# proger/haloop

Hardware: AMD Instinct MI355X
Metric: utterances/sec, LSTM-CTC training step (fwd + CTC loss + bwd + clip + AdamW) (higher is better)
Workload: dtype bf16 (dense operands rounded to bf16, 1 MFMA per product, fp32 accumulate; fp32 state, CTC, optimizer and master weights); 1 GPU; LC-2x1024: conv(80->128,k5,s4) + 2-layer LSTM H=1024 + Linear(1024->32) + CTC, 80 frames x 80 mels, vocab 32, targets 5-10 symbols, dropout 0.2; batch_per_gpu=64, global_batch=64, frames=80, mels=80, parallelism=dp1, hip_graph=False, math=bf16

## Files before the change

haloop_amd/_lib.py:

```python
import ctypes as C
import os

_HERE = os.path.dirname(os.path.abspath(__file__))
LIB_PATH = os.path.join(_HERE, 'csrc', 'libhalo.so')

HALO_ABI_VERSION = 21
HALO_GPT_SAMPLE_STREAM = 0x47505453
HALO_MLM_STREAM = 0x4D4C4D31
HALO_GEMM_RELU = 1
HALO_GEMM_GELU = 2
HALO_GEMM_ACCUM = 4
HALO_GEMM_GELU_ERF = 8
HALO_CTC_FULL_LATTICE = 1
HALO_CTC_FINITE_MIN = 2
HALO_CTC_NO_LEAD_BLANK_LOOP = 4
HALO_CTC_WRAP_SKIP = 8
HALO_STREAM_SUBSAMPLE = 1
HALO_STREAM_CLASSIFIER = 2
HALO_STREAM_LSTM_LAYER0 = 16
HALO_SUMSQ_PARTS = 1024
HALO_MATH_F32 = 0
HALO_MATH_BF16X3 = 1
HALO_MATH_BF16 = 2

_vp, _i, _l, _f, _u64, _u32, _sz = C.c_void_p, C.c_int, C.c_long, C.c_float, C.c_uint64, C.c_uint32, C.c_size_t

SIGNATURES = {
    'halo_abi_version': (_i, []),
    'halo_debug_read': (_i, [_vp, _sz, _i, _sz, _vp, _vp]),
    'halo_strerror': (C.c_char_p, [_i]),
    'halo_device_info': (_i, [_i, C.c_char_p, _i, C.POINTER(_i)]),
    'halo_set_math_mode': (_i, [_i]),
    'halo_get_math_mode': (_i, []),
    'halo_set_scratch': (_i, [_vp, _sz]),
    'halo_set_lstm_fusion': (_i, [_i]),
    'halo_dropout_fwd': (_i, [_vp, _vp, _sz, _f, _u64, _u32, _u32, _vp, _vp]),
    'halo_counter_inc': (_i, [_vp, _vp]),
    'halo_gemm_f32': (_i, [_i, _i, _i, _i, _i, _vp, _i, _vp, _i, _vp, _i, _vp, _vp, _i, _f, _u64, _u32, _u32, _vp, _vp]),
    'halo_split_image_bytes': (_sz, [_i, _i]),
    'halo_split_image': (_i, [_vp, _i, _i, _i, _i, _vp, _vp]),
    'halo_layernorm_image': (_i, [_vp, _vp, _vp, _vp, _vp, _i, _i, _f, _vp]),
    'halo_layernorm_bf16': (_i, [_vp, _vp, _vp, _vp, _vp, _vp, _i, _i, _f, _vp]),
    'halo_cast_bf16': (_i, [_vp, _vp, _sz, _vp]),
    'halo_gelu_bf16': (_i, [_vp, _vp, _sz, _i, _vp]),
    'halo_gelu_bwd_bf16': (_i, [_vp, _vp, _vp, _sz, _i, _vp]),
    'halo_gemm_tn_bf16_group': (_i, [_i, _vp, _vp, _vp, _vp, _vp, _vp, _i, _vp, _vp, _i, _vp]),
    'halo_gemm_tn_rows_supported': (_i, [_i, _vp, _vp, _i]),
    'halo_gemm_tn_rows_preferred': (_i, [_i, _vp, _vp, _i]),
    'halo_gemm_tn_rows_group': (_i, [_i, _vp, _vp, _vp, _vp, _vp, _vp, _i, _vp, _vp, _vp]),
    'halo_gelu_b16': (_i, [_vp, _vp, _sz, _i, _vp]),
    'halo_gelu_bwd_b16': (_i, [_vp, _vp, _vp, _sz, _i, _vp]),
    'halo_dx_alloc': (_i, [_sz, _vp, _vp]),
    'halo_dx_open': (_i, [_vp, _vp]),
    'halo_dx_close': (_i, [_vp]),
    'halo_dx_free': (_i, [_vp]),
    'halo_dx_push': (_i, [_vp, _sz, _sz, _i, _vp, _sz, _i, _i, _vp]),
    'halo_dx_signal': (_i, [_vp, _sz, _i, _i, _u32, _vp]),
    'halo_dx_wait': (_i, [_vp, _i, _i, _u32, _vp]),
    'halo_dx_reduce': (_i, [_vp, _vp, _sz, _i, _i, _f, _vp]),
    'halo_attention_fwd_b16': (_i, [_vp, _l, _l, _vp, _vp, _l, _l, _vp, _l, _l, _vp, _l, _l, _vp, _i, _i, _i, _i, _i, _i, _vp]),
    'halo_attention_bwd_b16': (_i, [_vp, _l, _l, _vp, _vp, _l, _l, _vp, _vp, _l, _l, _vp, _vp, _vp, _vp, _vp, _l, _l, _i, _i, _i, _i, _i, _i, _vp]),
    'halo_gemm_rows_supported': (_i, [_i, _i, _i]),
    'halo_gemm_rows': (_i, [_vp, _vp, _l, _vp, _i, _i, _i, _vp, _l, _vp, _l, _vp, _l, _vp]),
    'halo_gemm_rows_gelu': (_i, [_vp, _vp, _l, _vp, _i, _i, _i, _vp, _vp, _l, _i, _vp]),
    'halo_gemm_rows_ce_workspace_bytes': (_sz, [_i, _i]),
    'halo_gemm_rows_ce': (_i, [_vp, _vp, _l, _vp, _i, _i, _i, _vp, _l, _vp, _vp, _vp, _vp, _l, _vp]),
    'halo_cross_entropy_bwd_bf16': (_i, [_vp, _vp, _vp, _vp, _l, _i, _i, _l, _l, _vp]),
    'halo_lora_supported': (_i, [_i, _i, _i, _i]),
    'halo_lora_pack_bytes': (_sz, [_i, _i]),
    'halo_lora_pack': (_i, [_vp, _vp, _i, _i, _i, _vp, _vp]),
    'halo_lora_down': (_i, [_vp, _l, _vp, _i, _i, _f, _vp, _f, _u64, _u32, _u32, _vp, _vp]),
    'halo_lora_up': (_i, [_vp, _vp, _i, _i, _f, _vp, _vp, _l, _f, _u64, _u32, _u32, _vp, _vp]),
    'halo_lora_tn_workspace_bytes': (_sz, [_i, _i]),
    'halo_lora_tn': (_i, [_vp, _vp, _l, _i, _i, _i, _f, _i, _vp, _vp, _f, _u64, _u32, _u32, _vp, _vp]),
    'halo_gemm_split_ce_workspace_bytes': (_sz, [_i, _i]),
    'halo_gemm_split_ce': (_i, [_vp, _vp, _i, _i, _i, _vp, _i, _vp, _vp, _l, _vp, _vp, _vp, _vp]),
    'halo_image_pair': (_i, [_vp, _vp, _i, _i, _l, _l, _i, _vp, _vp, _vp]),
    'halo_cross_entropy_bwd_images': (_i, [_vp, _vp, _vp, _vp, _l, _i, _i, _l, _l, _vp, _vp, _vp]),
    'halo_gemm_split': (_i, [_vp, _vp, _i, _i, _i, _vp, _i, _vp, _vp, _i, _f, _u64, _u32, _u32, _vp, _vp]),
    'halo_gemm_split_residual': (_i, [_vp, _vp, _i, _i, _i, _vp, _i, _vp, _i, _vp, _vp, _i, _f, _u64, _u32, _u32, _vp, _vp]),
    'halo_image_pairs': (_i, [_i, _vp, _vp, _vp, _vp, _vp, _vp, _vp]),
    'halo_gemm_split_io': (_i, [_vp, _vp, _vp, _l, _vp, _i, _i, _i, _vp, _i, _vp, _vp, _l, _vp, _i, _vp, _vp, _i, _vp]),
    'halo_gemm_tn_bf16': (_i, [_vp, _l, _vp, _l, _i, _i, _i, _vp, _i, _i, _vp]),
    'halo_subsample_col_bytes': (_sz, [_i] * 6),
    'halo_subsample_fwd': (_i, [_vp] * 5 + [_i] * 7 + [_f, _u64, _u32, _vp, _vp]),
    'halo_subsample_bwd': (_i, [_vp] * 6 + [_i] * 7 + [_f, _vp]),
    'halo_subsample_bwd_slabs': (_i, [_vp, _i] + [_vp] * 5 + [_i] * 7 + [_f, _vp]),
    'halo_lstm_reserve_bytes': (_sz, [_i] * 5),
    'halo_lstm_bwd_workspace_bytes': (_sz, [_i] * 5),
    'halo_lstm_fwd': (_i, [_vp] * 8 + [_l, _l, _i, _vp, _vp, _vp] + [_i] * 5 + [_f, _u64, _u32, _vp, _vp]),
    'halo_lstm_bwd': (_i, [_vp] * 4 + [_l, _l, _i] + [_vp] * 9 + [_i] * 7 + [_f, _u64, _u32, _vp, _vp]),
    'halo_set_lstm_persistent': (_i, [_i]),
    'halo_set_lstm_persistent_images': (_i, [_i]),
    'halo_lstm_persistent_eligible': (_i, [_i, _i]),
    'halo_set_lstm_persistent2': (_i, [_i]),
    'halo_set_lstm_interleave': (_i, [_i]),
    'halo_set_gemm256': (_i, [_i]),
    'halo_set_lstm_bwd_mid_event': (_i, [_vp]),
    'halo_lstm_bwd_mid_event_recorded': (_i, []),
    'halo_set_lstm_expect_backward': (_i, [_i]),
    'halo_set_lstm_dx_slabs': (_i, [_i]),
    'halo_set_defer_small_jobs': (_i, [_i]),
    'halo_set_grad_sumsq': (_i, [_vp, _i]),
    'halo_grad_sumsq_state': (_i, [_vp, _vp]),
    'halo_flush_small_jobs': (_i, [_vp]),
    'halo_lstm_dx_slabs_left': (_i, []),
    'halo_set_lstm_weights_stamp': (_i, [_u64]),
    'halo_lstm_persistent2_eligible': (_i, [_i, _i, _i, _i]),
    'halo_lstm_status_offset': (_sz, [_i] * 6),
    'halo_ghost_tile': (_i, []),
    'halo_ghost_sqnorm_workspace_bytes': (_sz, [_i, _i, _i]),
    'halo_ghost_sqnorm': (_i, [_vp, _i, _i, _i, _vp, _vp, _vp, _vp]),
    'halo_set_lstm_keep_gate_gradients': (_i, [_i]),
    'halo_get_lstm_keep_gate_gradients': (_i, []),
    'halo_lstm_ghost_terms': (_i, [_vp, _vp, _i, _i, _i, _i, _i, _f, _vp]),
    'halo_relu_dropout_bwd': (_i, [_vp, _vp, _vp, _sz, _f, _vp]),
    'halo_lstm_persist_stamps': (_i, [_vp]),
    'halo_lstm_chain_events': (_i, [_vp, _vp]),
    'halo_lstm_chain_info': (_i, [_i, C.POINTER(_i), C.c_char_p, _i]),
    'halo_log_softmax_fwd': (_i, [_vp, _vp, _i, _i, _vp]),
    'halo_log_softmax_bwd': (_i, [_vp, _vp, _vp, _i, _i, _vp]),
    'halo_colsum': (_i, [_vp, _i, _i, _i, _vp, _vp]),
    'halo_ctc_fwd': (_i, [_vp, _l, _l, _i, _i, _i, _vp, _l, _i, _vp, _vp, _i, _vp, _vp, _vp]),
    'halo_ctc_bwd': (_i, [_vp, _l, _l, _i, _i, _i, _vp, _l, _i, _vp, _vp, _vp, _vp, _vp, _vp, _vp, _l, _l, _vp]),
    'halo_ctc_prepare': (_i, [_vp, _vp, _i, _i, _i, _i, _vp, _vp, _vp]),
    'halo_ctc_mean_loss': (_i, [_vp, _vp, _i, _vp, _vp]),
    'halo_ctc_head_supported': (_i, [_i, _i, _i, _i]),
    'halo_ctc_head_greedy': (_i, [_vp, _vp, _vp, _vp, _vp, _vp, _vp, _vp, _i, _i, _i, _i, _vp]),
    'halo_ctc_head_workspace_bytes': (_sz, [_i, _i, _i]),
    'halo_ctc_head_fwd': (_i, [_vp, _vp, _vp, _f, _u64, _u32, _u32, _vp, _vp, _i, _i, _i, _vp, _l, _i, _vp, _vp, _vp, _vp, _vp, _vp, _vp,
                               _vp, _i, _i, _i, _i, _vp]),
    'halo_ctc_head_bwd': (_i, [_vp, _vp, _f, _u64, _u32, _u32, _vp, _vp, _vp, _l, _i, _vp, _vp, _vp, _vp, _vp, _vp, _vp, _vp, _vp,
                               _i, _i, _i, _i, _vp]),
    'halo_ctc_head_train_workspace_bytes': (_sz, [_i, _i, _i]),
    'halo_ctc_head_train_ticket_words': (_sz, [_i, _i]),
    'halo_ctc_head_train': (_i, [_vp, _vp, _vp, _f, _u64, _u32, _u32, _vp, _vp, _i, _i, _i, _vp, _l, _i, _vp, _vp, _vp, _vp, _vp, _vp, _vp,
                                 _vp, _vp, _vp, _i, _i, _i, _i, _vp]),
    'halo_ctc_greedy': (_i, [_vp, _i, _i, _i, _vp, _vp, _vp, _vp, _vp]),
    'halo_set_beam_vector_chunk': (_i, [_i]),
    'halo_logaddexp_aten': (_i, [_vp, _vp, _vp, _sz, _vp]),
    'halo_ctc_beam_workspace_bytes': (_sz, [_i] * 4),
    'halo_ctc_beam': (_i, [_vp, _i, _i, _i, _i, _i, _vp, _vp, _vp, _vp, _vp]),
    'halo_topk_f32': (_i, [_vp, _i, _i, _i, _vp, _vp, _vp, _vp]),
    'halo_embed_fwd': (_i, [_vp, _vp, _vp, _vp, _i, _i, _i, _i, _i, _vp]),
    'halo_layernorm_fwd': (_i, [_vp, _vp, _vp, _vp, _i, _i, _f, _vp]),
    'halo_attention_causal_fwd': (_i, [_vp, _vp, _i, _i, _i, _i, _vp]),
    'halo_cross_entropy_fwd': (_i, [_vp, _vp, _vp, _i, _i, _l, _l, _vp]),
    'halo_attention_fwd': (_i, [_vp, _l, _l, _vp, _vp, _l, _l, _vp, _l, _l, _vp, _vp, _i, _i, _i, _i, _i, _i, _vp, _vp]),
    'halo_attention_fwd_strided': (_i, [_vp, _l, _l, _l, _vp, _vp, _l, _l, _l, _vp, _l, _l, _vp, _vp, _i, _i, _i, _i, _i, _i, _vp,
                                        _f, _u64, _u32, _u32, _vp, _vp]),
    'halo_kv_cache_store_f32': (_i, [_vp, _l, _l, _vp, _vp, _i, _i, _i, _i, _i, _i, _vp]),
    'halo_rope_table': (_i, [_vp, _vp, _i, _i, _f, _vp]),
    'halo_rope_interleaved': (_i, [_vp, _l, _i, _i, _i, _i, _i, _vp, _vp, _i, _i, _vp]),
    'halo_rope_rows': (_i, [_vp, _i, _l, _l, _i, _i, _i, _i, _vp, _vp, _i, _i, _vp]),
    'halo_kv_cache_store': (_i, [_vp, _l, _l, _vp, _vp, _i, _i, _i, _i, _i, _i, _vp]),
    'halo_attention_decode': (_i, [_vp, _l, _vp, _vp, _vp, _l, _i, _i, _i, _i, _i, _vp, _vp, _vp, _vp]),
    'halo_attention_decode_step': (_i, [_vp, _vp, _vp, _l, _vp, _vp, _vp, _l, _i, _i, _i, _i, _i, _vp, _vp, _vp]),
    'halo_logprob_max': (_i, [_vp, _l, _i, _i, _vp, _vp, _vp, _vp]),
    'halo_greedy_update': (_i, [_vp, _vp, _vp, _vp, _l, _i, _i, _i, _vp, _vp, _vp, _vp, _i, _vp]),
    'halo_fbank_frames': (_i, [_vp, _l, _i, _i, _i, _f, _i, _vp, _vp, _i, _vp]),
    'halo_fbank_power': (_i, [_vp, _i, _i, _vp, _i, _vp]),
    'halo_fbank_log': (_i, [_vp, _l, _f, _vp]),
    'halo_fbank_spectrum_mel': (_i, [_vp, _i, _i, _vp, _vp, _i, _f, _vp, _vp]),
    'halo_star_ctc_workspace_bytes': (_sz, [_i, _i, _i]),
    'halo_star_ctc_fwd': (_i, [_vp, _l, _l, _i, _i, _i, _vp, _i, _vp, _vp, _f, _vp, _vp, _vp]),
    'halo_star_ctc_bwd': (_i, [_vp, _l, _l, _i, _i, _i, _vp, _i, _vp, _vp, _f, _vp, _vp, _vp, _vp, _vp]),
    'halo_transducer_workspace_bytes': (_sz, [_i, _i, _i]),
    'halo_transducer_fwd': (_i, [_vp, _i, _i, _i, _i, _vp, _vp, _vp, _vp, _vp, _vp]),
    'halo_transducer_bwd': (_i, [_vp, _i, _i, _i, _i, _vp, _vp, _vp, _vp, _vp, _vp, _vp, _vp]),
    'halo_decode_image_bytes': (_sz, [_i, _i]),
    'halo_decode_image': (_i, [_vp, _i, _i, _l, _vp, _vp]),
    'halo_decode_linear_supported': (_i, [_i, _i]),
    'halo_decode_linear': (_i, [_vp, _l, _i, _i, _vp, _f, _vp, _i, _vp, _l, _i, _vp]),
    'halo_decode_linear_pair': (_i, [_vp, _vp, _l, _i, _i, _vp, _f, _vp, _i, _vp, _vp, _vp, _l, _i, _vp]),
    'halo_decode_attention_pair': (_i, [_vp, _l, _i, _i, _i, _vp, _vp, _i, _vp, _vp, _vp, _i, _i, _vp, _vp, _vp, _l, _vp]),
    'halo_decode_memory_caches': (_i, [_vp, _l, _i, _vp, _i, _i, _i, _i, _vp]),
    'halo_decode_token': (_i, [_vp, _l, _i, _i, _vp, _l, _i, _i, _i, _vp, _vp, _vp, _vp, _vp, _i, _i, _vp, _vp]),
    'halo_decode_beam_attention': (_i, [_vp, _l, _i, _i, _i, _i, _vp, _vp, _i, _vp, _vp, _vp, _i, _i, _vp, _l, _vp, _vp, _vp, _l, _vp]),
    'halo_decode_beam_select': (_i, [_vp, _l, _i, _i, _i, _i, _i, _i, _f, _vp, _vp, _vp, _vp, _vp, _vp, _vp, _vp, _vp, _vp, _vp, _l, _l, _vp, _i,
                                     _i, _vp, _vp]),
    'halo_rnnt_advance': (_i, [_vp, _l, _l, _i, _i, _i, _vp, _l, _vp, _vp, _vp, _l, _vp, _vp, _vp, _l, _i, _i, _vp, _i, _vp, _l, _vp, _vp]),
    'halo_rnnt_lstm_cell': (_i, [_vp, _l, _i, _i, _vp, _vp, _vp, _vp, _vp, _l, _vp, _l, _vp]),
    'halo_rnnt_beam_step': (_i, [_vp, _l, _l, _i, _i, _i, _vp, _l, _vp, _vp, _i, _i, _i, _vp, _vp, _vp, _vp, _vp, _vp, _l, _vp, _vp, _vp, _vp, _vp, _vp,
                                 _vp, _vp, _i, _i, _vp, _vp, _vp, _vp, _vp, _vp]),
    'halo_rnnt_beam_keep': (_i, [_i, _i, _i, _i, _i, _vp, _vp, _vp, _vp, _vp, _l, _vp, _vp, _vp, _vp]),
    'halo_rnnt_joint_fwd': (_i, [_vp, _l, _l, _vp, _l, _l, _i, _i, _i, _i, _vp, _vp, _vp, _vp, _vp, _vp]),
    'halo_rnnt_joint_bwd': (_i, [_vp, _l, _l, _vp, _l, _l, _i, _i, _i, _i, _vp, _vp, _vp, _vp, _vp, _vp, _l, _l, _vp, _l, _l, _vp]),
    'halo_ctc_viterbi_workspace_bytes': (_sz, [_i, _i, _i]),
    'halo_ctc_viterbi': (_i, [_vp, _l, _l, _i, _i, _i, _vp, _l, _i, _vp, _vp, _vp, _vp, _vp, _vp, _vp, _vp]),
    'halo_transducer_viterbi_workspace_bytes': (_sz, [_i, _i, _i]),
    'halo_transducer_viterbi': (_i, [_vp, _i, _i, _i, _i, _vp, _vp, _vp, _vp, _vp, _vp, _vp]),
    'halo_ctc_prefix_beam_workspace_bytes': (_sz, [_i, _i, _i, _i, _i]),
    'halo_ctc_prefix_beam': (_i, [_vp, _l, _l, _i, _i, _i, _vp, _i, _i, _vp, _vp, _vp, _vp, _vp, _vp]),
    'halo_ctc_lm_beam_step': (_i, [_vp, _l, _l, _i, _i, _i, _vp, _i, _i, _i, _f, _f, _vp, _l, _vp, _vp, _vp, _vp, _vp, _vp, _vp, _l, _vp, _vp, _vp,
                                   _i, _i, _vp, _vp, _vp, _vp, _vp]),
    'halo_edit_distance': (_i, [_vp, _l, _vp, _i, _i, _vp, _l, _vp, _i, _i, _i, _vp, _vp, _vp]),
    'halo_nbest_risk_fwd': (_i, [_vp, _vp, _i, _i, _vp, _vp]),
    'halo_nbest_risk_bwd': (_i, [_vp, _vp, _i, _i, _vp, _vp, _vp]),
    'halo_gpt_decode_linear_supported': (_i, [_i, _i]),
    'halo_gpt_decode_linear': (_i, [_vp, _l, _i, _i, _vp, _f, _vp, _i, _vp, _l, _i, _vp]),
    'halo_gpt_decode_attention': (_i, [_vp, _l, _i, _i, _i, _vp, _vp, _i, _vp, _vp, _l, _vp]),
    'halo_gpt_sample': (_i, [_vp, _l, _i, _i, _vp, _vp, _l, _vp, _l, _i, _vp, _vp, _vp, _i, _i, _vp, _vp]),
    'halo_attention_bwd': (_i, [_vp, _l, _l, _vp, _vp, _l, _l, _vp, _vp, _l, _l, _vp, _vp, _vp, _l, _l, _vp, _vp, _l, _l,
                                _i, _i, _i, _i, _i, _i, _vp, _f, _u64, _u32, _u32, _vp, _vp]),
    'halo_attention_masked': (_i, [_vp, _vp, _vp, _vp, _l, _l, _l, _vp, _vp, _i, _i, _i, _i, _i, _vp]),
    'halo_attention_fwd_bf16': (_i, [_vp, _l, _l, _vp, _vp, _l, _l, _vp, _l, _l, _vp, _l, _l, _vp, _i, _i, _i, _i, _i, _i, _vp, _f, _u64, _u32, _u32,
                                     _vp, _vp]),
    'halo_attention_bwd_bf16': (_i, [_vp, _l, _l, _vp, _vp, _l, _l, _vp, _vp, _l, _l, _vp, _vp, _vp, _vp, _vp, _l, _l, _i, _i, _i, _i, _i, _i, _vp,
                                     _f, _u64, _u32, _u32, _vp, _vp]),
    'halo_layernorm_bwd_workspace_bytes': (_sz, [_i, _i]),
    'halo_layernorm_bwd': (_i, [_vp, _vp, _vp, _vp, _vp, _vp, _vp, _vp, _i, _i, _f, _vp]),
    'halo_layernorm_bwd_bf16': (_i, [_vp, _vp, _vp, _vp, _vp, _vp, _vp, _vp, _vp, _i, _i, _f, _vp]),
    'halo_layernorm_bwd_b16': (_i, [_vp, _vp, _vp, _vp, _vp, _vp, _vp, _vp, _vp, _i, _i, _f, _vp]),
    'halo_gelu_fwd': (_i, [_vp, _vp, _sz, _i, _vp]),
    'halo_gelu_bwd': (_i, [_vp, _vp, _vp, _sz, _i, _vp]),
    'halo_cross_entropy_fwd_lse': (_i, [_vp, _vp, _vp, _vp, _i, _i, _l, _l, _vp]),
    'halo_cross_entropy_bwd': (_i, [_vp, _vp, _vp, _vp, _l, _i, _i, _l, _l, _vp]),
    'halo_embed_bwd': (_i, [_vp, _vp, _vp, _vp, _i, _i, _i, _i, _i, _i, _vp]),
    'halo_embed_bwd_ordered': (_i, [_vp, _vp, _vp, _i, _i, _i, _vp]),
    'halo_add_rows_bcast': (_i, [_vp, _vp, _i, _i, _i, _vp]),
    'halo_im2col_cl': (_i, [_vp, _vp, _i, _i, _i, _i, _i, _i, _vp]),
    'halo_col2im_cl': (_i, [_vp, _vp, _i, _i, _i, _i, _i, _i, _vp]),
    'halo_dwconv1d_cl': (_i, [_vp, _vp, _vp, _vp, _i, _i, _i, _i, _i, _i, _vp]),
    'halo_dwconv1d_cl_bwd_workspace_bytes': (_sz, [_i, _i]),
    'halo_dwconv1d_cl_bwd': (_i, [_vp, _vp, _vp, _vp, _vp, _vp, _vp, _i, _i, _i, _i, _i, _i, _vp]),
    'halo_tape_batch': (_i, [_vp, _i, _l, _i, _i, _l, _i, _l, _vp, _vp]),
    'halo_lm_batch_u16': (_i, [_vp, _l, _vp, _i, _i, _i, _vp, _vp, _vp]),
    'halo_mask_tokens': (_i, [_vp, _vp, _l, _f, _l, _l, _l, _u64, _u32, _vp]),
    'halo_mlm_batch_u16': (_i, [_vp, _l, _vp, _i, _i, _f, _l, _l, _l, _u64, _u32, _vp, _vp, _vp]),
    'halo_target_rows': (_i, [_vp, _i, _l, _i, _i, _vp, _vp, _vp, _vp, _vp]),
    'halo_gather_rows': (_i, [_vp, _vp, _i, _i, _i, _vp, _vp]),
    'halo_scatter_rows': (_i, [_vp, _vp, _vp, _i, _i, _i, _i, _vp, _vp, _vp]),
    'halo_scale_add': (_i, [_vp, _vp, _f, _f, _sz, _vp]),
    'halo_cast_f32_bf16': (_i, [_vp, _vp, _sz, _vp]),
    'halo_cast_bf16_f32': (_i, [_vp, _vp, _f, _sz, _vp]),
    'halo_scale_add_guarded': (_i, [_vp, _vp, _f, _f, _sz, _vp, _vp]),
    'halo_clip_coef_step': (_i, [_vp, _i, _f, _vp, _vp, _vp, _vp]),
    'halo_adamw_ranges_dev': (_i, [_vp, _vp, _vp, _vp, _i, _vp, _vp, _vp, _vp, _f, _vp, _f, _f, _f, _vp, _vp, _vp]),
    'halo_ctx_create': (_vp, []),
    'halo_ctx_destroy': (None, [_vp]),
    'halo_ctx_use': (_i, [_vp]),
    'halo_set_status_word': (_i, [_vp]),
    'halo_debug_mute_workgroup': (_i, [_i]),
    'halo_debug_mfma_clock': (_i, [_vp, _vp, _i, _i, _i, _u32, _vp]),
    'halo_sumsq': (_i, [_vp, _sz, _vp, _vp]),
    'halo_sumsq_ranges': (_i, [_vp, _i, _vp, _vp, _vp, _vp]),
    'halo_pack_ranges_bf16': (_i, [_vp, _i, _vp, _vp, _vp, _vp]),
    'halo_expand_ranges_bf16': (_i, [_vp, _i, _vp, _vp, _i, _i, _vp, _vp]),
    'halo_clip_coef': (_i, [_vp, _i, _f, _vp, _vp, _vp]),
    'halo_adamw_multi_tensor_bytes': (_sz, []),
    'halo_adamw_multi_chunk': (_u32, []),
    'halo_adamw_multi_max_tensors': (_i, []),
    'halo_adamw_multi': (_i, [_vp, _vp, _i, _vp, _i, _f, _f, _f, _f, _i, _vp, _vp]),
    'halo_adamw_ranges': (_i, [_vp, _vp, _vp, _vp, _i, _vp, _vp, _vp, _vp, _f, _f, _f, _f, _i, _vp, _vp]),
    'halo_adamw': (_i, [_vp, _vp, _vp, _vp, _sz, _f, _f, _f, _f, _f, _i, _vp, _vp]),
}



class GhostOperand(C.Structure):
    _fields_ = [('ptr', _vp), ('stride_n', _l), ('stride_t', _l), ('K', _i)]


class GhostTerm(C.Structure):
    _fields_ = [('a', GhostOperand), ('b', GhostOperand * 2), ('n_b', _i), ('n_bias', _i)]


_lib = None


class HaloError(RuntimeError):
    pass


def lib():
    global _lib
    if _lib is None:
        import torch
        if not os.path.exists(LIB_PATH):
            raise HaloError(f'{LIB_PATH} not found: build it with `make -C haloop_amd/csrc` '
                            '(or __graft_entry__.build()); haloop_amd has no CPU fallback')
        handle = C.CDLL(LIB_PATH)
        for name, (res, args) in SIGNATURES.items():
            fn = getattr(handle, name)
            fn.restype = res
            fn.argtypes = args
        if handle.halo_abi_version() != HALO_ABI_VERSION:
            raise HaloError('libhalo.so ABI version mismatch: rebuild it')
        _lib = handle
        mode = os.environ.get('HALO_MATH')
        if mode:
            set_math_mode(mode)
    return _lib


def set_math_mode(mode):
    global _mode
    code = {'f32': HALO_MATH_F32, 'bf16x3': HALO_MATH_BF16X3, 'bf16': HALO_MATH_BF16}[mode]
    check(lib().halo_set_math_mode(code), 'halo_set_math_mode')
    _mode = mode


def set_lstm_fusion(on):
    check(lib().halo_set_lstm_fusion(int(bool(on))), 'halo_set_lstm_fusion')


def set_lstm_persistent(on):
    check(lib().halo_set_lstm_persistent(int(bool(on))), 'halo_set_lstm_persistent')


def set_lstm_bwd_mid_event(event):
    check(lib().halo_set_lstm_bwd_mid_event(None if event is None else C.c_void_p(event.cuda_event)), 'halo_set_lstm_bwd_mid_event')


def set_gemm256(on):
    check(lib().halo_set_gemm256(1 if on else 0), 'halo_set_gemm256')


def set_lstm_interleave(on):
    check(lib().halo_set_lstm_interleave(int(bool(on))), 'halo_set_lstm_interleave')


def set_lstm_keep_gate_gradients(on):
    check(lib().halo_set_lstm_keep_gate_gradients(int(bool(on))), 'halo_set_lstm_keep_gate_gradients')


def get_lstm_keep_gate_gradients():
    return bool(lib().halo_get_lstm_keep_gate_gradients())


def set_lstm_persistent2(on):
    check(lib().halo_set_lstm_persistent2(int(bool(on))), 'halo_set_lstm_persistent2')


_WEIGHTS_EPOCH = [0]


# ... 107 lines not shown
```

haloop_amd/csrc/halo_internal.h:

```cpp
#pragma once
#include <hip/hip_runtime.h>
#include <stddef.h>
#include "halo_common.h"
#include "dyn_lds.h"
#include "small_jobs.h"

int halo_transpose(const float *in, float *out, int rows, int cols, hipStream_t st);
int halo_fill(float *p, size_t n, float v, hipStream_t st);
int halo_colsum2(const float *x, int rows, int cols, int ld, float *out, float *out2, hipStream_t st);

size_t halo_tiled_image_bytes(int R, int K);
int halo_prep_tiles(const float *src, int R, int K, int ld, int src_transposed, void *image, hipStream_t st);
int halo_prep_pair(const float *src, int R, int C, int ld, void *image_rm, void *image_tr, hipStream_t st);
struct HaloPrepJob {
    int kind;
    const float *src;
    int R, K, ld;
    void *image, *image_tr;
};
int halo_prep_jobs(const HaloPrepJob *jobs, int n, hipStream_t st);
int halo_gemm_bf16x3_tiled(const void *Aimg, const void *Bimg, int M, int N, int K, float *C, int ldc,
                           const float *bias1, const float *bias2, int relu, const DropoutCfg *drop, hipStream_t st);
int halo_gemm_bf16x3_tiled_slices(const void *Aimg, const void *Bimg, int M, int N, int K, float *slab, int want, int *slices, hipStream_t st);
bool halo_defer_small_job(const HaloSmallJob &job);
struct HaloCtx {
    int math_mode = 0;
    int lstm_fusion = 0;
    int lstm_persistent = 1, lstm_persistent2 = 1;
    int lstm_interleave = 1;
    int persist_emit = -1;
    int beam_vec_chunk = 32;
    void *scratch = nullptr;
    size_t scratch_bytes = 0;
    int scratch_slot = 0;
    unsigned *status = nullptr;
    hipEvent_t chain_ev0 = nullptr, chain_ev1 = nullptr;
    int bwd_mid_recorded = 0;
    hipEvent_t bwd_mid_event = nullptr;
    unsigned long long *stamps = nullptr;
    float *grad_sumsq = nullptr;
    int grad_sumsq_cap = 0, grad_sumsq_n = 0;
    unsigned grad_sumsq_cover = 0;
    int defer_small_jobs = 0;
    HaloSmallJobs small_jobs = {};
    int lstm_dx_slabs = 1;
    int lstm_dx_slabs_left = 1;
    int lstm_expect_backward = 1;
    const float *packT_reserve = nullptr, *packT_w[3] = {nullptr, nullptr, nullptr};
    const float *bwdflags_reserve = nullptr;
    const float *fwdT_src[2] = {nullptr, nullptr};
    const float *fwdT_reserve = nullptr;
    const float *emitT_reserve = nullptr;
    uint64_t lstm_weights_stamp = 0, packF_stamp = 0;
    const float *packF_reserve = nullptr, *packF_w[3] = {nullptr, nullptr, nullptr};
    int packF_dims[5] = {0, 0, 0, 0, 0};
    int lstm_keep_dg = 0;
    const float *ghost_reserve = nullptr;
    int mute_block = -1;
};
HaloCtx &halo_ctx_cur();
int halo_cu_count();
int halo_gemm_bf16x3_tiled_nsplit(const void *Aimg, const void *Bimg, int M, int N, int K, float *C, int ldc, int n_split, float *C2, int ldc2,
                                  hipStream_t st);
int halo_gemm_bf16x3_tiled_nsplit_carry(const void *Aimg, const void *Bimg, int M, int N, int K, float *C, int ldc, int n_split, float *C2, int ldc2,
                                        const void *rA, const void *rB, int rM, int rN, int rK, float *rslab, int want, int *slices,
                                        float *sumsq_part, int *sumsq_parts, hipStream_t st);
struct HaloG256Problem {
    const void *A, *B;
    int M, N, K;
    float *C; int ldc;
    int n_split; float *C2; int ldc2;
    int kslices; long slab_stride;
    float *sumsq;
    int tiles;
};
int halo_gemm256_enabled();
int halo_gemm256_fits(const HaloG256Problem &q);
int halo_gemm256_launch(HaloG256Problem *probs, int n, hipStream_t st);
int halo_math_mode();
int halo_lstm_fusion();

void halo_get_scratch(void **ptr, size_t *bytes);
void halo_set_scratch_slot(int slot);
int halo_side_stream(hipStream_t *side, hipEvent_t *fork_ev, hipEvent_t *join_ev);
int halo_pick_ksplit(long tiles, int k_steps, long out_elems);
int halo_splitk_reduce(const float *slab, int ksplit, int M, int N, float *C, int ldc, const float *bias1,
                       const float *bias2, int relu, const DropoutCfg &drop, int use_drop, hipStream_t st);
```

haloop_amd/csrc/lstm.hip:

```cpp
#include <stdlib.h>
#include <string.h>
#include "halo_common.h"
#include "halo_internal.h"
#include "tiled_image.h"
#include "lstm_persist.h"

namespace {

enum YMode { Y_NONE = 0, Y_PLAIN = 1, Y_RELU = 2, Y_DROPOUT = 3 };

typedef __bf16 bf16x8 __attribute__((ext_vector_type(8)));

template <bool X3>
struct Packed {
    static constexpr int KB = X3 ? 32 : 16;
    static constexpr int BLOCK_BYTES = X3 ? 2048 : 1024;
    __device__ static __forceinline__ void store(void *img, int tile, int nk, int i, int k, float v) {
        const int blk = k / KB, kk = k % KB;
        char *base = (char *)img + ((long)tile * (nk / KB) + blk) * BLOCK_BYTES;
        if (X3) {
            const int lane = (kk >> 3) * 16 + i, e = kk & 7;
            const __bf16 hi = (__bf16)v;
            const __bf16 lo = (__bf16)(v - (float)hi);
            reinterpret_cast<__bf16 *>(base)[lane * 8 + e] = hi;
// ... 1015 lines not shown
                         const uint32_t *offset_dev, hipStream_t st) {
    const size_t BH = (size_t)B * H, PG = bt16(B) * 4 * H, per = fused_bwd_layer_floats(B, H);
    for (int l = 0; l < L; ++l) {
        float *base = extra + (size_t)l * per;
        HALO_TRY(launch_pack<1>(w_hh[l], base, H, B, 4 * H, H / 16, true, st));
        if (l > 0) HALO_TRY(launch_pack<1>(w_ih[l], base + (size_t)4 * H * H, H, B, 4 * H, H / 16, true, st));
    }
    for (int d = 0; d < T + L - 1; ++d) {
        DiagBwdArgs a;
        a.B = B; a.H = H;
        for (int l = 0; l < MAXL; ++l) {
            DiagBwdLayer &q = a.layer[l];
            const int t = l < L ? T - 1 - (d - (L - 1 - l)) : -1;
            q.active = l < L && t >= 0 && t < T;
            if (!q.active) continue;
            const LayerBufs lb = layer_bufs(reserve, l, T, B, H);
            float *base = extra + (size_t)l * per;
            float *dcarry = base + (size_t)8 * H * H;
            float *dgp = dcarry + BH;
            const bool top = (l == L - 1);
            q.dgp_next = (t == T - 1) ? nullptr : dgp + (size_t)((t + 1) & 1) * PG;
            q.dgp_out = dgp + (size_t)(t & 1) * PG;
            q.wpT_hh = base;
            if (!top) {
                float *above = extra + (size_t)(l + 1) * per;
                q.dgp_above = above + (size_t)8 * H * H + BH + (size_t)(t & 1) * PG;
                q.wpT_ih_above = above + (size_t)4 * H * H;
            } else {
                q.dgp_above = nullptr; q.wpT_ih_above = nullptr;
            }
            q.gates = lb.gates + (size_t)t * B * 4 * H;
            q.c = lb.c + (size_t)(t + 1) * BH;
            q.cprev = lb.c + (size_t)t * BH;
            q.dc = dcarry;
            q.dy = (top && dy) ? dy + (long)t * y_stride_t : nullptr;
            q.dy_stride_b = y_stride_b;
            q.dy_relu = y_relu;
            q.first = (t == T - 1);
            q.dhinit = (t == T - 1 && dhn) ? dhn + (size_t)l * BH : nullptr;
            q.dcinit = (t == T - 1 && dcn) ? dcn + (size_t)l * BH : nullptr;
            q.drop = make_dropout(top ? 0.f : p_drop, seed, HALO_STREAM_LSTM_LAYER0 + (uint32_t)l, offset, offset_dev);
            q.drop_base = (uint64_t)t * BH;
        }
        hipLaunchKernelGGL(lstm_diag_bwd_kernel, dim3(H / 16, (B + 15) / 16, L), dim3(1024), 0, st, a);
        HALO_TRY(halo_launch_status());
    }
    return HALO_OK;
}

inline size_t reserve_flags_offset(int T, int B, int in0, int H, int L) {
    const int kin = in0 > H ? in0 : H;
    const size_t n = ((size_t)4 * H * H + (size_t)L * layer_floats(T, B, H)) * sizeof(float) +
                     halo_tiled_image_bytes(T * B, kin) + halo_tiled_image_bytes(4 * H, kin) +
                     (L >= 2 ? fused_fwd_extra_floats(T, B, H, L) * sizeof(float) : 0);
    return (n + 255) & ~(size_t)255;
}
inline int bwd_dg_images(int T) { return T > 2 ? T : 2; }
inline size_t bwd_flags_offset(int T, int B, int in0, int H, int L) {
    const int kin = in0 > H ? in0 : H;
    const size_t n = ((size_t)H * 4 * H + (size_t)B * H + (size_t)T * B * H + (size_t)bwd_dg_images(T) * bt16(B) * 4 * H) * sizeof(float) +
                     halo_tiled_image_bytes(4 * H, T * B) + halo_tiled_image_bytes(T * B, 4 * H) +
                     2 * halo_tiled_image_bytes(kin, T * B) + halo_tiled_image_bytes(kin, 4 * H) +
                     (L >= 2 ? (size_t)L * fused_bwd_layer_floats(B, H) * sizeof(float) : 0);
    return (n + 255) & ~(size_t)255;
}

inline size_t reserve_p2_images_bytes(int T, int B, int in0, int H) {
    const int kin = in0 > H ? in0 : H;
    return (size_t)3 * 4 * H * H * sizeof(float) + 3 * halo_tiled_image_bytes(H, T * B) + halo_tiled_image_bytes(kin, T * B);
}
inline size_t reserve_p2_bytes(int T, int B, int in0, int H) {
    return reserve_p2_images_bytes(T, B, in0, H) + PERSIST_FLAG_BYTES + halo_tiled_image_bytes(in0 > H ? in0 : H, 4 * H);
}
inline unsigned *reserve_bwd_flags(float *reserve, int T, int B, int in0, int H, int L) {
    return (unsigned *)((char *)reserve + reserve_flags_offset(T, B, in0, H, L) + PERSIST_FLAG_BYTES + reserve_p2_images_bytes(T, B, in0, H));
}
inline char *reserve_p2_wT(float *reserve, int T, int B, int in0, int H, int L) {
    return (char *)reserve_bwd_flags(reserve, T, B, in0, H, L) + PERSIST_FLAG_BYTES;
}
inline char *reserve_p2_images(float *reserve, int T, int B, int in0, int H, int L) {
    return (char *)reserve + reserve_flags_offset(T, B, in0, H, L) + PERSIST_FLAG_BYTES + (size_t)3 * 4 * H * H * sizeof(float);
}

inline bool persist_emit_enabled() {
    int &v = halo_ctx_cur().persist_emit;
    if (v < 0) { const char *e = getenv("HALO_PERSIST_EMIT"); v = e ? (atoi(e) != 0) : 1; }
    return v != 0;
}

inline bool keep_dg_switch() {
    static const bool on = getenv("HALO_LSTM_KEEP_DG") && getenv("HALO_LSTM_KEEP_DG")[0] == '1';
    return on || halo_ctx_cur().lstm_keep_dg != 0;
}

inline bool pair_dw_enabled() {
    static const bool on = !(getenv("HALO_LSTM_PAIR_DW") && atoi(getenv("HALO_LSTM_PAIR_DW")) == 0);
    return on;
}

int lstm_bwd_layer_tail(const float *x, const float *const *w_ih, float *reserve, int l, int in0, int T, int B, int H, int L, float p_drop,
                        uint64_t seed, uint32_t offset, const uint32_t *offset_dev, bool fused, bool emit, char *img_g, char *img_gT,
                        char *img_hT, char *img_inT, char *img_wT, const float *bias_part, float *din, float *dx, float *const *dw_ih,
                        float *const *dw_hh, float *const *db_ih, float *const *db_hh, bool need_din, hipStream_t st) {
    const size_t BH = (size_t)B * H;
    const LayerBufs lb = layer_bufs(reserve, l, T, B, H);
    hipStream_t side = st;
    const float *in;
    int in_dim;
    if (l == 0) { in = x; in_dim = in0; }
    else {
        const LayerBufs pb = layer_bufs(reserve, l - 1, T, B, H);
        in = p_drop > 0.f ? pb.ydrop : pb.h + BH;
        in_dim = H;
    }
    (void)fused;
    float *din_out = l > 0 ? din : dx;
    const DropoutCfg ddrop = make_dropout(l > 0 ? p_drop : 0.f, seed, HALO_STREAM_LSTM_LAYER0 + (uint32_t)(l > 0 ? l - 1 : 0),
                                          offset, offset_dev);
    const bool tiled = halo_math_mode() != HALO_MATH_F32 && in_dim >= 64;
    int rc = HALO_OK;
    if (tiled) {
        HaloPrepJob jobs[5];
        int nj = 0;
        if (need_din) {
            if (!emit) jobs[nj++] = {2, lb.gates, T * B, 4 * H, 4 * H, img_g, img_gT};
            jobs[nj++] = {1, w_ih[l], in_dim, 4 * H, in_dim, img_wT, nullptr};
        } else if (!emit) {
            jobs[nj++] = {1, lb.gates, 4 * H, T * B, 4 * H, img_gT, nullptr};
        }
        if (emit)
            jobs[nj++] = {3, bias_part, (B + 15) / 16, 4 * H, 4 * H, db_ih[l], db_hh[l]};
        jobs[nj++] = {1, lb.h, H, T * B, H, img_hT, nullptr};
        jobs[nj++] = {1, in, in_dim, T * B, in_dim, img_inT, nullptr};
        HALO_TRY(halo_prep_jobs(jobs, nj, st));
    }
    if (need_din) {
        if (tiled) {
            HALO_TRY(halo_gemm_bf16x3_tiled(img_g, img_wT, T * B, in_dim, 4 * H, din_out, in_dim, nullptr, nullptr, 0,
                                            &ddrop, st));
        } else {
            HALO_TRY(halo_gemm_f32(1, 0, T * B, in_dim, 4 * H, lb.gates, 4 * H, w_ih[l], in_dim, din_out, in_dim,
                                   nullptr, nullptr, 0, l > 0 ? p_drop : 0.f, seed,
                                   HALO_STREAM_LSTM_LAYER0 + (uint32_t)(l > 0 ? l - 1 : 0), offset, offset_dev, (halo_stream_t)st));
        }
    }
    if (tiled && H % 128 == 0 && img_inT == img_hT + halo_tiled_image_bytes(H, T * B) && pair_dw_enabled()) {
        HaloG256Problem gp = {};
        gp.A = img_gT; gp.B = img_hT; gp.M = 4 * H; gp.N = H + in_dim; gp.K = T * B;
        gp.C = dw_hh[l]; gp.ldc = H; gp.n_split = H; gp.C2 = dw_ih[l]; gp.ldc2 = in_dim; gp.kslices = 1;
        const long t256 = (long)((4 * H + 255) / 256) * ((H + in_dim + 255) / 256);
        if (halo_gemm256_enabled() && halo_gemm256_fits(gp) && 100 * t256 >= 55 * ((t256 + 255) / 256) * 256) rc = halo_gemm256_launch(&gp, 1, side);
        else
        rc = halo_gemm_bf16x3_tiled_nsplit(img_gT, img_hT, 4 * H, H + in_dim, T * B, dw_hh[l], H, H, dw_ih[l], in_dim, side);
    } else if (tiled) {
        rc = halo_gemm_bf16x3_tiled(img_gT, img_hT, 4 * H, H, T * B, dw_hh[l], H, nullptr, nullptr, 0, nullptr, side);
        if (!rc) rc = halo_gemm_bf16x3_tiled(img_gT, img_inT, 4 * H, in_dim, T * B, dw_ih[l], in_dim, nullptr, nullptr, 0,
                                             nullptr, side);
    } else {
        rc = halo_gemm_f32(0, 0, 4 * H, H, T * B, lb.gates, 4 * H, lb.h, H, dw_hh[l], H, nullptr, nullptr, 0, 0.f, 0, 0,
                           0, nullptr, (halo_stream_t)side);
        if (!rc) rc = halo_gemm_f32(0, 0, 4 * H, in_dim, T * B, lb.gates, 4 * H, in, in_dim, dw_ih[l], in_dim, nullptr,
                                    nullptr, 0, 0.f, 0, 0, 0, nullptr, (halo_stream_t)side);
    }
    if (!rc && !(emit && tiled)) rc = halo_colsum2(lb.gates, T * B, 4 * H, 4 * H, db_ih[l], db_hh[l], side);
    return rc;
}


int lstm_fwd_persist2(const float *in, int in_dim, int lo, const float *const *w_ih, const float *const *w_hh, const float *const *b_ih,
                      const float *const *b_hh, const float *h0, const float *c0, float *y, long y_stride_t, long y_stride_b,
                      int y_relu, float *hn, float *cn, float *reserve, float *extra, char *img_in, char *img_w, int T, int B,
                      int in0, int H, int L, float p_drop, uint64_t seed, uint32_t offset, const uint32_t *offset_dev, hipStream_t st) {
    const int hi = lo + 1;
    const size_t BH = (size_t)B * H;
    const LayerBufs l0 = layer_bufs(reserve, lo, T, B, H), l1 = layer_bufs(reserve, hi, T, B, H);
    w_ih += lo; w_hh += lo; b_ih += lo; b_hh += lo;
    if (h0) h0 += (size_t)lo * BH;
    if (c0) c0 += (size_t)lo * BH;
    HaloCtx &ctx = halo_ctx_cur();
    const bool images_by_pack = in_dim >= 64;
    if (in_dim < 64) {
        HALO_TRY(halo_gemm_f32(1, 1, T * B, 4 * H, in_dim, in, in_dim, w_ih[0], in_dim, l0.gates, 4 * H, b_ih[0], b_hh[0], 0, 0.f, 0, 0, 0,
                               nullptr, (halo_stream_t)st));
    }
    float *wp0 = reserve, *wp1 = fused_wpk(extra, hi, H), *wpi = wp1 + (size_t)4 * H * H;
    unsigned *flags = (unsigned *)((char *)reserve + reserve_flags_offset(T, B, in0, H, L));
    Prologue2Args pa;
    pa.img.n = 0; pa.img.blocks = 0; pa.img.with_lo = halo_math_mode() != HALO_MATH_BF16;
    pa.w[0] = w_hh[0]; pa.wdst[0] = wp0; pa.w[1] = w_hh[1]; pa.wdst[1] = wp1; pa.w[2] = w_ih[1]; pa.wdst[2] = wpi;
    pa.w_units = (long)(H / 16) * 4 * (H / 32) * 64; pa.wK = H;
    for (int l = 0; l < 2; ++l) {
        const LayerBufs lb = l ? l1 : l0;
        pa.h0[l] = h0 ? h0 + (size_t)l * BH : nullptr; pa.hp0[l] = lb.hp; pa.h_rm[l] = lb.h;
        pa.c0[l] = c0 ? c0 + (size_t)l * BH : nullptr; pa.c_rm[l] = lb.c;
    }
    pa.s_units = (long)((B + 15) / 16) * (H / 32) * 64;
    pa.zero = flags; pa.zero_units = (long)(PERSIST_FLAG_BYTES / 16);
    pa.zero2 = nullptr; pa.zero2_units = 0;
    char *xp = p_drop > 0.f ? (char *)fused_yp(extra, lo, T, B, H, L) : nullptr;
    pa.narm = 0; pa.arm_units = 0;
    if (halo_lstm_persist2_fwd_armed(T, B, H)) {
        const size_t image = (size_t)((B + 15) / 16) * (H / 32) * 2048;
        pa.arm[pa.narm++] = (char *)l0.hp + image;
        pa.arm[pa.narm++] = (char *)l1.hp + image;
        if (xp) pa.arm[pa.narm++] = xp;
        pa.arm_units = (long)T * (long)(image / 2048) * 64;
    }
    pa.H = H; pa.B = B;
    ctx.packT_reserve = nullptr;
    ctx.emitT_reserve = nullptr;
    char *emit_hT0 = nullptr, *emit_hT1 = nullptr, *emit_xT1 = nullptr;
    if (ctx.lstm_expect_backward && H % 32 == 0) {
        float *wT = (float *)((char *)reserve + reserve_flags_offset(T, B, in0, H, L) + PERSIST_FLAG_BYTES);
        PackPairArgs pp;
        for (int m = 0; m < 3; ++m) { pp.w[m] = pa.w[m]; pp.fwd[m] = (char *)pa.wdst[m]; pp.tr[m] = (char *)(wT + (size_t)m * 4 * H * H); }
        pp.H = H;
        pp.tile_blocks = 3 * (4 * H / 32) * (H / 32) / 4;
        pp.rest = pa; pp.rest.w_units = 0;
        pp.rest.zero2 = reserve_bwd_flags(reserve, T, B, in0, H, L); pp.rest.zero2_units = (long)(PERSIST_FLAG_BYTES / 16);
        pp.zbase[0] = pp.zbase[1] = nullptr; pp.zstride = 0; pp.zunits = 0; pp.zcount = 0;
        ctx.emitT_reserve = nullptr;
        const bool emitT = persist_emit_enabled() && !h0 && B % 32 == 0 && H % 128 == 0 && T * B >= 32;
        if (emitT) {
            char *imgs = reserve_p2_images(reserve, T, B, in0, H, L);
            const size_t hb = halo_tiled_image_bytes(H, T * B), ib = halo_tiled_image_bytes(in0 > H ? in0 : H, T * B);
            emit_hT0 = imgs; emit_hT1 = imgs + hb + ib; emit_xT1 = emit_hT1 + hb;
            const long KT = (T * B + 31) / 32;
            pp.zbase[0] = emit_hT0; pp.zbase[1] = emit_hT1;
            pp.zstride = KT * 16384; pp.zunits = (long)(B / 32) * 16384 / 16; pp.zcount = H / 128;
            ctx.emitT_reserve = reserve;
        }
        ctx.fwdT_reserve = nullptr;
        if (images_by_pack) {
            ImageJobs &ij = pp.rest.img;
            image_jobs_add(ij, in, T * B, in_dim, in_dim, 0, img_in);
            image_jobs_add(ij, w_ih[0], 4 * H, in_dim, in_dim, 0, img_w);
            if (emitT) {
                image_jobs_add(ij, in, in_dim, T * B, in_dim, 1, emit_hT0 + halo_tiled_image_bytes(H, T * B));
                image_jobs_add(ij, w_ih[0], in_dim, 4 * H, in_dim, 1, reserve_p2_wT(reserve, T, B, in0, H, L));
                ctx.fwdT_reserve = reserve; ctx.fwdT_src[0] = in; ctx.fwdT_src[1] = w_ih[0];
            }
        }
        const unsigned rest_blocks = pack_grid((size_t)(2 * pa.s_units + pa.zero_units + pp.rest.zero2_units + 2L * pp.zcount * pp.zunits +
                                                        (long)pa.narm * pa.arm_units));
        hipLaunchKernelGGL(persist2_pack_pair_kernel, dim3((unsigned)(pp.tile_blocks + pp.rest.img.blocks) + rest_blocks), dim3(256), 0, st, pp);
        HALO_TRY(halo_launch_status());
        if (images_by_pack)
            HALO_TRY(halo_gemm_bf16x3_tiled(img_in, img_w, T * B, 4 * H, in_dim, l0.gates, 4 * H, b_ih[0], b_hh[0], 0, nullptr, st));
        ctx.packT_reserve = reserve;
        ctx.bwdflags_reserve = reserve;
        for (int m = 0; m < 3; ++m) ctx.packT_w[m] = pa.w[m];
    } else {
        const int dims[5] = {T, B, in0, H, L};
        const bool keep = ctx.lstm_weights_stamp != 0 && lo == 0 && ctx.packF_stamp == ctx.lstm_weights_stamp && ctx.packF_reserve == reserve &&
                          ctx.packF_w[0] == pa.w[0] && ctx.packF_w[1] == pa.w[1] && ctx.packF_w[2] == pa.w[2] &&
                          !memcmp(ctx.packF_dims, dims, sizeof(dims));
        if (keep) pa.w_units = 0;
        if (images_by_pack) {
            image_jobs_add(pa.img, in, T * B, in_dim, in_dim, 0, img_in);
            image_jobs_add(pa.img, w_ih[0], 4 * H, in_dim, in_dim, 0, img_w);
        }
        hipLaunchKernelGGL(persist2_prologue_kernel<0>, dim3((unsigned)pa.img.blocks + pack_grid((size_t)(3 * pa.w_units + 2 * pa.s_units + pa.zero_units +
                                                                                                      (long)pa.narm * pa.arm_units))),
                           dim3(256), 0, st, pa);
        HALO_TRY(halo_launch_status());
        if (images_by_pack)
            HALO_TRY(halo_gemm_bf16x3_tiled(img_in, img_w, T * B, 4 * H, in_dim, l0.gates, 4 * H, b_ih[0], b_hh[0], 0, nullptr, st));
        ctx.packF_stamp = lo == 0 ? ctx.lstm_weights_stamp : 0;
        ctx.packF_reserve = reserve;
        for (int m = 0; m < 3; ++m) ctx.packF_w[m] = pa.w[m];
        memcpy(ctx.packF_dims, dims, sizeof(dims));
    }
    Persist2Fwd a;
    a.wp0 = (const char *)wp0; a.wp1 = (const char *)wp1; a.wpi = (const char *)wpi;
    a.hp0 = (char *)l0.hp; a.hp1 = (char *)l1.hp;
    a.xp = xp;
    a.gates0 = l0.gates; a.h0 = l0.h; a.c0 = l0.c;
    a.gates1 = l1.gates; a.h1 = l1.h; a.c1 = l1.c;
    a.b_ih1 = b_ih[1]; a.b_hh1 = b_hh[1];
    a.ydrop = p_drop > 0.f ? l0.ydrop : nullptr;
    a.y = y; a.y_stride_t = y_stride_t; a.y_stride_b = y_stride_b; a.y_mode = y ? (y_relu ? 2 : 1) : 0;
    a.drop = make_dropout(p_drop, seed, HALO_STREAM_LSTM_LAYER0 + (uint32_t)lo, offset, offset_dev);
    a.img_hT0 = emit_hT0; a.img_hT1 = emit_hT1; a.img_xT1 = emit_xT1;
    a.flags = flags;
    a.stamps = halo_lstm_persist_stamp_buffer();
    a.T = T; a.B = B; a.H = H;
    chain_begin(st);
    HALO_TRY(halo_lstm_persist2_fwd(a, st));
    chain_end(st, 0, 1, "lstm_persist2_fwd_kernel");
    for (int l = 0; l < 2; ++l) {
        const LayerBufs lb = l ? l1 : l0;
        if (hn) HALO_TRY(copy_d2d(hn + (size_t)(lo + l) * BH, lb.h + (size_t)T * BH, BH, st));
        if (cn) HALO_TRY(copy_d2d(cn + (size_t)(lo + l) * BH, lb.c + (size_t)T * BH, BH, st));
    }
    return HALO_OK;
}


inline size_t bwd_p2_offset(int T, int B, int in0, int H, int L) {
    const size_t n = bwd_flags_offset(T, B, in0, H, L) + PERSIST_FLAG_BYTES + (size_t)((B + 15) / 16) * 4 * H * sizeof(float);
    return (n + 255) & ~(size_t)255;
}
inline size_t bwd_p2_bytes(int T, int B, int H) {
    return (((size_t)((B + 15) / 16) * 4 * H * sizeof(float) + 255) & ~(size_t)255) + (size_t)T * bt16(B) * 4 * H * sizeof(float) +
           halo_tiled_image_bytes(4 * H, T * B);
}

}

extern "C" {

int halo_lstm_chain_events(void *ev_begin, void *ev_end) {
    halo_ctx_cur().chain_ev0 = (hipEvent_t)ev_begin;
    halo_ctx_cur().chain_ev1 = (hipEvent_t)ev_end;
    return HALO_OK;
}

int halo_lstm_chain_info(int backward, int *launches, char *kernel, int kernel_len) {
    const ChainInfo &ci = g_chain_info[backward ? 1 : 0];
    if (launches) *launches = ci.launches;
    if (kernel && kernel_len > 0) {
        strncpy(kernel, ci.kernel, (size_t)kernel_len - 1);
        kernel[kernel_len - 1] = 0;
    }
    return HALO_OK;
}

size_t halo_lstm_reserve_bytes(int T, int B, int in0, int H, int L) {
    if (T <= 0 || B <= 0 || in0 <= 0 || H <= 0 || L <= 0) return 0;
    return reserve_flags_offset(T, B, in0, H, L) + PERSIST_FLAG_BYTES + (L >= 2 ? reserve_p2_bytes(T, B, in0, H) : 0);
}

int halo_set_lstm_persistent(int on) {
    halo_lstm_persist_enable(on);
    return HALO_OK;
}

int halo_set_lstm_persistent_images(int on) {
    halo_ctx_cur().persist_emit = on ? 1 : 0;
    return HALO_OK;
}


int halo_lstm_persistent_eligible(int B, int H) { return halo_lstm_persist_ok(B, H) && use_x3(H) ? 1 : 0; }

int halo_set_lstm_persistent2(int on) {
    halo_lstm_persist2_enable(on);
    return HALO_OK;
}
int halo_set_lstm_bwd_mid_event(void *event) {
    halo_ctx_cur().bwd_mid_event = (hipEvent_t)event;
    halo_ctx_cur().bwd_mid_recorded = 0;
    return HALO_OK;
}
int halo_lstm_bwd_mid_event_recorded(void) { return halo_ctx_cur().bwd_mid_recorded; }
int halo_set_lstm_interleave(int on) {
    halo_lstm_interleave_enable(on);
    return HALO_OK;
}
int halo_set_lstm_weights_stamp(uint64_t stamp) {
    halo_ctx_cur().lstm_weights_stamp = stamp;
    return HALO_OK;
}

int halo_set_grad_sumsq(float *partials, int capacity) {
    HaloCtx &ctx = halo_ctx_cur();
    if (partials && capacity <= 0) return HALO_EINVAL;
    ctx.grad_sumsq = partials; ctx.grad_sumsq_cap = partials ? capacity : 0; ctx.grad_sumsq_n = 0; ctx.grad_sumsq_cover = 0;
    return HALO_OK;
}
int halo_grad_sumsq_state(int *count, unsigned *covered) {
    const HaloCtx &ctx = halo_ctx_cur();
    if (count) *count = ctx.grad_sumsq_n;
    if (covered) *covered = ctx.grad_sumsq_cover;
    return HALO_OK;
}
int halo_set_lstm_dx_slabs(int n) {
    if (n < 1 || n > 64) return HALO_EINVAL;
    halo_ctx_cur().lstm_dx_slabs = n;
    return HALO_OK;
}
int halo_lstm_dx_slabs_left(void) { return halo_ctx_cur().lstm_dx_slabs_left; }
int halo_set_lstm_expect_backward(int on) {
    halo_ctx_cur().lstm_expect_backward = on ? 1 : 0;
    return HALO_OK;
}
int halo_lstm_persistent2_eligible(int T, int B, int H, int L) {       return !fused_ok(H, L) && use_x3(H) && halo_lstm_persist2_ok(T, B, H, L) ? 1 : 0; }

size_t halo_lstm_status_offset(int backward, int T, int B, int in0, int H, int L) {
    if (T <= 0 || B <= 0 || in0 <= 0 || H <= 0 || L <= 0) return 0;
    return backward ? bwd_flags_offset(T, B, in0, H, L) : reserve_flags_offset(T, B, in0, H, L);
}

size_t halo_lstm_bwd_workspace_bytes(int T, int B, int in0, int H, int L) {
    if (T <= 0 || B <= 0 || H <= 0 || L <= 0) return 0;
    if (L >= 2) return bwd_p2_offset(T, B, in0, H, L) + bwd_p2_bytes(T, B, H);
    return bwd_flags_offset(T, B, in0, H, L) + PERSIST_FLAG_BYTES + (size_t)((B + 15) / 16) * 4 * H * sizeof(float);
}

int halo_lstm_fwd(const float *x, const float *const *w_ih, const float *const *w_hh, const float *const *b_ih,
                  const float *const *b_hh, const float *h0, const float *c0, float *y, long y_stride_t,
                  long y_stride_b, int y_relu, float *hn, float *cn, float *reserve, int T, int B, int in0, int H,
                  int L, float p_drop, uint64_t seed, uint32_t offset, const uint32_t *offset_dev,
                  halo_stream_t stream) {
    HALO_CHECK_ARG(x && w_ih && w_hh && b_ih && b_hh && reserve);
    HALO_CHECK_ARG(T > 0 && B > 0 && in0 > 0 && H > 0 && L > 0);
    if (H % 16 != 0) return HALO_ENOTSUP;
    halo_ctx_cur().ghost_reserve = nullptr;
    hipStream_t st = (hipStream_t)stream;
    const size_t BH = (size_t)B * H, PH = bt16(B) * H;
    halo_ctx_cur().packT_reserve = nullptr;
    halo_ctx_cur().emitT_reserve = nullptr;
    float *wp = reserve;
    const bool x3 = use_x3(H);
    const int kin = in0 > H ? in0 : H;
    char *img_in = (char *)(reserve + (size_t)4 * H * H + (size_t)L * layer_floats(T, B, H));
    char *img_w = img_in + halo_tiled_image_bytes(T * B, kin);
    for (int l = 0; l < L; ++l) HALO_CHECK_ARG(w_ih[l] && w_hh[l] && b_ih[l] && b_hh[l]);
    const bool pair = !fused_ok(H, L) && x3 && halo_lstm_persist2_ok(T, B, H, L);
    const int n_single = pair ? L - 2 : L;
    if (fused_ok(H, L)) {
        float *extra = (float *)(img_w + halo_tiled_image_bytes(4 * H, kin));
        return lstm_fwd_fused(x, w_ih, w_hh, b_ih, b_hh, h0, c0, y, y_stride_t, y_stride_b, y_relu, hn, cn, reserve, extra,
                              img_in, img_w, T, B, in0, H, L, p_drop, seed, offset, offset_dev, st);
    }
    for (int l = 0; l < L; ++l) {
        const LayerBufs lb = layer_bufs(reserve, l, T, B, H);
        const bool last = (l == L - 1);
        const bool drop_out = !last && p_drop > 0.f;
        const float *in;
        int in_dim;
        if (l == 0) { in = x; in_dim = in0; }
        else {
            const LayerBufs pb = layer_bufs(reserve, l - 1, T, B, H);
            in = p_drop > 0.f ? pb.ydrop : pb.h + BH;
            in_dim = H;
        }
        if (pair && l == n_single) {
            float *extra = (float *)(img_w + halo_tiled_image_bytes(4 * H, kin));
            return lstm_fwd_persist2(in, in_dim, l, w_ih, w_hh, b_ih, b_hh, h0, c0, y, y_stride_t, y_stride_b, y_relu, hn, cn, reserve, extra,
                                     img_in, img_w, T, B, in0, H, L, p_drop, seed, offset, offset_dev, st);
        }
        if (halo_math_mode() != HALO_MATH_F32 && in_dim >= 64) {
            const HaloPrepJob jobs[2] = {{0, in, T * B, in_dim, in_dim, img_in, nullptr}, {0, w_ih[l], 4 * H, in_dim, in_dim, img_w, nullptr}};
            HALO_TRY(halo_prep_jobs(jobs, 2, st));
            HALO_TRY(halo_gemm_bf16x3_tiled(img_in, img_w, T * B, 4 * H, in_dim, lb.gates, 4 * H, b_ih[l], b_hh[l], 0,
                                            nullptr, st));
        } else {
            HALO_TRY(halo_gemm_f32(1, 1, T * B, 4 * H, in_dim, in, in_dim, w_ih[l], in_dim, lb.gates, 4 * H, b_ih[l],
                                   b_hh[l], 0, 0.f, 0, 0, 0, nullptr, stream));
        }
        const float *h0l = h0 ? h0 + (size_t)l * BH : nullptr;
        const bool persist = x3 && halo_lstm_persist_ok(B, H) && halo_lstm_persist_fits(T, B, H);
        unsigned *flags = (unsigned *)((char *)reserve + reserve_flags_offset(T, B, in0, H, L));
        if (persist) {
            PrologueArgs pa;
            pa.w = w_hh[l]; pa.wdst = wp; pa.w_units = (long)(H / 16) * 4 * (H / 32) * 64; pa.wK = H;
            pa.h0 = h0l; pa.hp0 = lb.hp; pa.h_rm = lb.h; pa.c0 = c0 ? c0 + (size_t)l * BH : nullptr; pa.c_rm = lb.c;
            pa.s_units = (long)((B + 15) / 16) * (H / 32) * 64;
            pa.zero = flags; pa.zero_units = (long)(PERSIST_FLAG_BYTES / 16);
            pa.zero2 = nullptr; pa.zero2_units = 0;
            pa.H = H; pa.B = B;
            hipLaunchKernelGGL(persist_prologue_kernel<0>, dim3(pack_grid((size_t)(pa.w_units + pa.s_units + pa.zero_units))), dim3(256), 0, st, pa);
            HALO_TRY(halo_launch_status());
        } else {
            HALO_TRY(launch_pack<0>(w_hh[l], wp, H, B, H, (H / 16) * 4, x3, st));
            HALO_TRY(launch_pack<2>(h0l, lb.hp, H, B, H, (B + 15) / 16, x3, st, lb.h, c0 ? c0 + (size_t)l * BH : nullptr, lb.c));
        }
        const DropoutCfg dc = make_dropout(drop_out ? p_drop : 0.f, seed, HALO_STREAM_LSTM_LAYER0 + (uint32_t)l, offset, offset_dev);
        if (persist) {
            PersistFwd a;
            a.wp = (const char *)wp;
            a.hp = (char *)lb.hp;
            a.gates = lb.gates; a.h = lb.h; a.c = lb.c;
            a.T = T; a.B = B; a.H = H;
            a.drop = dc;
            if (last && y) { a.y = y; a.y_stride_t = y_stride_t; a.y_stride_b = y_stride_b; a.y_mode = y_relu ? Y_RELU : Y_PLAIN; }
            else if (drop_out) { a.y = lb.ydrop; a.y_stride_t = (long)BH; a.y_stride_b = H; a.y_mode = Y_DROPOUT; }
            else { a.y = nullptr; a.y_stride_t = 0; a.y_stride_b = 0; a.y_mode = Y_NONE; }
            a.flags = flags;
            a.stamps = halo_lstm_persist_stamp_buffer();
            chain_begin(st);
            HALO_TRY(halo_lstm_persist_fwd(a, st));
            chain_end(st, 0, 1, "lstm_persist_fwd_kernel");
            if (hn) HALO_TRY(copy_d2d(hn + (size_t)l * BH, lb.h + (size_t)T * BH, BH, st));
            if (cn) HALO_TRY(copy_d2d(cn + (size_t)l * BH, lb.c + (size_t)T * BH, BH, st));
            continue;
        }
        chain_begin(st);
        for (int t = 0; t < T; ++t) {
            StepFwdArgs a;
            a.hp_prev = lb.hp + (size_t)t * PH;
            a.cprev = lb.c + (size_t)t * BH;
            a.wp = wp;
            a.gates = lb.gates + (size_t)t * B * 4 * H;
            a.hout = lb.h + (size_t)(t + 1) * BH;
            a.hp_out = lb.hp + (size_t)(t + 1) * PH;
            a.cout = lb.c + (size_t)(t + 1) * BH;
            a.B = B; a.H = H;
            a.drop = dc;
            a.drop_base = (uint64_t)t * BH;
            if (last && y) {
                a.y = y + (long)t * y_stride_t;
                a.y_stride_b = y_stride_b;
                a.y_mode = y_relu ? Y_RELU : Y_PLAIN;
            } else if (drop_out) {
                a.y = lb.ydrop + (size_t)t * BH;
                a.y_stride_b = H;
                a.y_mode = Y_DROPOUT;
            } else {
                a.y = nullptr; a.y_stride_b = 0; a.y_mode = Y_NONE;
            }
            HALO_TRY(launch_step_fwd(a, x3, st));
        }
        chain_end(st, 0, T, "lstm_step_fwd_kernel");
        if (hn) HALO_TRY(copy_d2d(hn + (size_t)l * BH, lb.h + (size_t)T * BH, BH, st));
        if (cn) HALO_TRY(copy_d2d(cn + (size_t)l * BH, lb.c + (size_t)T * BH, BH, st));
    }
    return HALO_OK;
}

int halo_lstm_bwd(const float *x, const float *const *w_ih, const float *const *w_hh, const float *dy,
                  long y_stride_t, long y_stride_b, int y_relu, const float *dhn, const float *dcn, float *reserve,
                  float *workspace, float *dx, float *const *dw_ih, float *const *dw_hh, float *const *db_ih,
// ... 297 lines not shown
```

haloop_amd/csrc/optim.hip:

```cpp
#include <math.h>
#include <stdlib.h>
#include "halo_common.h"
#include "halo_internal.h"

namespace {

__global__ __launch_bounds__(256) void sumsq_kernel(const float *__restrict__ x, size_t n, float *__restrict__ partials) {
    __shared__ float red[4];
    float s = 0.f;
    const size_t n4 = n / 4;
    const f32x4 *x4 = reinterpret_cast<const f32x4 *>(x);
    for (size_t i = blockIdx.x * (size_t)256 + threadIdx.x; i < n4; i += (size_t)gridDim.x * 256) {
        const f32x4 v = x4[i];
        s += v[0] * v[0] + v[1] * v[1] + v[2] * v[2] + v[3] * v[3];
    }
    if (blockIdx.x == 0)
        for (size_t i = n4 * 4 + threadIdx.x; i < n; i += 256) s += x[i] * x[i];
    s = wave_sum(s);
    if ((threadIdx.x & 63) == 0) red[threadIdx.x >> 6] = s;
    __syncthreads();
    if (threadIdx.x == 0) partials[blockIdx.x] = (red[0] + red[1]) + (red[2] + red[3]);
}

struct Ranges8 {
// ... 50 lines not shown
            if ((int)rk == skip) continue;
            const bf16x4 v = reinterpret_cast<const bf16x4 *>(stage)[rk * per_rank + off + j];
            d4[i] = f32x4{(float)v[0], (float)v[1], (float)v[2], (float)v[3]};
        }
        off += c;
    }
}

__global__ __launch_bounds__(256) void clip_coef_kernel(const float *__restrict__ partials, int count, float max_norm,
                                                        float *coef, float *norm_out, uint32_t *applied_steps, const uint32_t *status) {
    __shared__ float red[4];
    float s = 0.f;
    for (int i = threadIdx.x; i < count; i += 256) s += partials[i];
    s = wave_sum(s);
    if ((threadIdx.x & 63) == 0) red[threadIdx.x >> 6] = s;
    __syncthreads();
    if (threadIdx.x == 0) {
        const float norm = sqrtf((red[0] + red[1]) + (red[2] + red[3]));
        const float c = max_norm / (norm + 1e-6f);
        const bool finite = isfinite(norm) && !(status && *status != 0u);
        coef[0] = finite ? (c > 1.0f ? 1.0f : c) : NAN;
        coef[1] = finite ? 1.0f : NAN;
        if (norm_out) *norm_out = norm;
        if (applied_steps && finite) *applied_steps += 1u;
    }
}

__device__ __forceinline__ void adam_update(float &p, float &m, float &v, float g, float decay_mul, float beta1_w, float beta2,
                                            float beta2_w, float step_size, float bc2_sqrt, float eps) {
#pragma clang fp contract(off)
    p = p * decay_mul;
    m = __builtin_fmaf(g - m, beta1_w, m);
    v = __builtin_fmaf(beta2_w * g, g, v * beta2);
    const float denom = sqrtf(v) / bc2_sqrt + eps;
    p = p - step_size * (m / denom);
}

struct AdamArgs {
    float *p;
    const float *g;
    float *m;
    float *v;
    size_t n;
    float decay_mul;
    float beta1_w;
    float beta2;
    float beta2_w;
    float step_size;
    float bc2_sqrt;
    float eps;
    const float *grad_scale;
};

__global__ __launch_bounds__(256) void adamw_kernel(const AdamArgs a) {
    const float gs = a.grad_scale ? *a.grad_scale : 1.0f;
    if (gs != gs) return;
    const size_t n4 = a.n / 4;
    f32x4 *p4 = reinterpret_cast<f32x4 *>(a.p), *m4 = reinterpret_cast<f32x4 *>(a.m), *v4 = reinterpret_cast<f32x4 *>(a.v);
    const f32x4 *g4 = reinterpret_cast<const f32x4 *>(a.g);
    for (size_t i = blockIdx.x * (size_t)256 + threadIdx.x; i < n4; i += (size_t)gridDim.x * 256) {
        f32x4 p = p4[i], m = m4[i], v = v4[i];
        const f32x4 g = g4[i];
#pragma unroll
        for (int e = 0; e < 4; ++e) {
            const float ge = a.grad_scale ? g[e] * gs : g[e];
            float pe = p[e], me = m[e], ve = v[e];
            adam_update(pe, me, ve, ge, a.decay_mul, a.beta1_w, a.beta2, a.beta2_w, a.step_size, a.bc2_sqrt, a.eps);
            p[e] = pe; m[e] = me; v[e] = ve;
        }
        p4[i] = p; m4[i] = m; v4[i] = v;
    }
    if (blockIdx.x == 0) {
        for (size_t i = n4 * 4 + threadIdx.x; i < a.n; i += 256) {
            const float ge = a.grad_scale ? a.g[i] * gs : a.g[i];
            float pe = a.p[i], me = a.m[i], ve = a.v[i];
            adam_update(pe, me, ve, ge, a.decay_mul, a.beta1_w, a.beta2, a.beta2_w, a.step_size, a.bc2_sqrt, a.eps);
            a.p[i] = pe; a.m[i] = me; a.v[i] = ve;
        }
    }
}


constexpr int ADAM_MAX_RANGES = 8;
struct AdamRangesArgs {
    float *p;
    const float *g;
    float *m;
    float *v;
    size_t begin4[ADAM_MAX_RANGES], end4[ADAM_MAX_RANGES];
    float decay_mul[ADAM_MAX_RANGES];
    const float *grad_scale[ADAM_MAX_RANGES];
    int n_ranges;
    float beta1_w, beta2, beta2_w, step_size, bc2_sqrt, eps;
    uint32_t *counter;
    const uint32_t *step_dev;
    const float *lr_dev;
    float weight_decay[ADAM_MAX_RANGES];
    float lr, beta1;
};

template <bool NT>
__global__ __launch_bounds__(256) void adamw_ranges_kernel(const AdamRangesArgs a) {
    f32x4 *p4 = reinterpret_cast<f32x4 *>(a.p), *m4 = reinterpret_cast<f32x4 *>(a.m), *v4 = reinterpret_cast<f32x4 *>(a.v);
    const f32x4 *g4 = reinterpret_cast<const f32x4 *>(a.g);
    float step_size = a.step_size, bc2_sqrt = a.bc2_sqrt;
    const float lr = a.lr_dev ? *a.lr_dev : a.lr;
    if (a.step_dev) {
        const double t = (double)max(*a.step_dev, 1u);
        step_size = (float)((double)lr / (1.0 - pow((double)a.beta1, t)));
        bc2_sqrt = (float)sqrt(1.0 - pow((double)a.beta2, t));
    }
    for (int r = 0; r < a.n_ranges; ++r) {
        const float gs = a.grad_scale[r] ? *a.grad_scale[r] : 1.0f;
        if (gs != gs) continue;
        const float decay_mul = a.lr_dev ? (float)(1.0 - (double)lr * (double)a.weight_decay[r]) : a.decay_mul[r];
        for (size_t i = a.begin4[r] + blockIdx.x * (size_t)256 + threadIdx.x; i < a.end4[r]; i += (size_t)gridDim.x * 256) {
            f32x4 p = p4[i], m = NT ? __builtin_nontemporal_load(m4 + i) : m4[i], v = NT ? __builtin_nontemporal_load(v4 + i) : v4[i];
            const f32x4 g = NT ? __builtin_nontemporal_load(g4 + i) : g4[i];
#pragma unroll
            for (int e = 0; e < 4; ++e) {
                const float ge = a.grad_scale[r] ? g[e] * gs : g[e];
                float pe = p[e], me = m[e], ve = v[e];
                adam_update(pe, me, ve, ge, decay_mul, a.beta1_w, a.beta2, a.beta2_w, step_size, bc2_sqrt, a.eps);
                p[e] = pe; m[e] = me; v[e] = ve;
            }
            p4[i] = p;
            if (NT) { __builtin_nontemporal_store(m, m4 + i); __builtin_nontemporal_store(v, v4 + i); }
            else { m4[i] = m; v4[i] = v; }
        }
    }
    if (a.counter && blockIdx.x == 0 && threadIdx.x == 0) *a.counter += 1u;
}

struct AdamTensor {
    float *p;
    float *m;
    float *v;
    unsigned long long n;
    float weight_decay;
    int pad;
};
constexpr unsigned ADAM_CHUNK = 16384;
constexpr int ADAM_MULTI_MAX = 256;
struct AdamGrads { const float *g[ADAM_MULTI_MAX]; };

__global__ __launch_bounds__(256) void adamw_multi_kernel(const AdamTensor *__restrict__ tensors, const uint2 *__restrict__ chunks,
                                                          const AdamGrads grads, float lr, float beta1_w, float beta2, float beta2_w,
                                                          float step_size, float bc2_sqrt, float eps,
                                                          const float *__restrict__ grad_scale) {
    const float gs = grad_scale ? *grad_scale : 1.0f;
    if (gs != gs) return;
    const uint2 c = chunks[blockIdx.x];
    const AdamTensor t = tensors[c.x];
    const float decay_mul = (float)(1.0 - (double)lr * (double)t.weight_decay);
    const float *tg = grads.g[c.x];
    const size_t begin = (size_t)c.y * ADAM_CHUNK, end = min(begin + (size_t)ADAM_CHUNK, (size_t)t.n);
    auto update = [&](float &pe, float &me, float &ve, float g) {
        adam_update(pe, me, ve, grad_scale ? g * gs : g, decay_mul, beta1_w, beta2, beta2_w, step_size, bc2_sqrt, eps);
    };
    const bool vec = (((uintptr_t)t.p | (uintptr_t)tg | (uintptr_t)t.m | (uintptr_t)t.v) % 16) == 0;
    size_t done = begin;
    if (vec) {
        const size_t e4 = end / 4;
        f32x4 *p4 = reinterpret_cast<f32x4 *>(t.p), *m4 = reinterpret_cast<f32x4 *>(t.m), *v4 = reinterpret_cast<f32x4 *>(t.v);
        const f32x4 *g4 = reinterpret_cast<const f32x4 *>(tg);
        for (size_t i = begin / 4 + threadIdx.x; i < e4; i += 256) {
            f32x4 p = p4[i], m = __builtin_nontemporal_load(m4 + i), v = __builtin_nontemporal_load(v4 + i);
            const f32x4 g = __builtin_nontemporal_load(g4 + i);
#pragma unroll
            for (int e = 0; e < 4; ++e) {
                float pe = p[e], me = m[e], ve = v[e];
                update(pe, me, ve, g[e]);
                p[e] = pe; m[e] = me; v[e] = ve;
            }
            p4[i] = p;
            __builtin_nontemporal_store(m, m4 + i);
            __builtin_nontemporal_store(v, v4 + i);
        }
        done = e4 * 4;
    }
    for (size_t i = done + threadIdx.x; i < end; i += 256) {
        float pe = t.p[i], me = t.m[i], ve = t.v[i];
        update(pe, me, ve, tg[i]);
        t.p[i] = pe; t.m[i] = me; t.v[i] = ve;
    }
}

}

namespace {
__global__ __launch_bounds__(256) void scale_add_kernel(float *__restrict__ y, const float *__restrict__ x, float alpha, float beta, size_t n4,
                                                        size_t n, const float *__restrict__ guard) {
    const size_t i = (size_t)blockIdx.x * 256 + threadIdx.x;
    const bool take_x = !guard || isfinite(*guard);
    const bool take_y = alpha != 0.f;
    if (i < n4) {
        f32x4 a = {0.f, 0.f, 0.f, 0.f}, b = {0.f, 0.f, 0.f, 0.f};
        if (take_y) a = alpha * reinterpret_cast<f32x4 *>(y)[i];
        if (take_x) b = beta * reinterpret_cast<const f32x4 *>(x)[i];
        reinterpret_cast<f32x4 *>(y)[i] = a + b;
    } else if (i == n4) {
        for (size_t e = 4 * n4; e < n; ++e) y[e] = (take_y ? alpha * y[e] : 0.f) + (take_x ? beta * x[e] : 0.f);
    }
}
}

namespace {
typedef __bf16 bf16x4 __attribute__((ext_vector_type(4)));
__global__ __launch_bounds__(256) void cast_f32_bf16_kernel(const float *__restrict__ x, __bf16 *__restrict__ y, size_t n4, size_t n) {
    for (size_t i = (size_t)blockIdx.x * 256 + threadIdx.x; i < n4; i += (size_t)gridDim.x * 256) {
        const f32x4 v = reinterpret_cast<const f32x4 *>(x)[i];
        bf16x4 o;
#pragma unroll
        for (int e = 0; e < 4; ++e) o[e] = (__bf16)v[e];
// ... 77 lines not shown

int halo_pack_ranges_bf16(const float *src, int n, const size_t *begin, const size_t *end, void *dst, halo_stream_t stream) {
    HALO_CHECK_ARG(src && dst && ((uintptr_t)src % 16 == 0) && ((uintptr_t)dst % 8 == 0));
    Ranges8 r; size_t total4;
    { const int rc = make_ranges8(n, begin, end, r, total4); if (rc != HALO_OK) return rc; }
    if (total4 == 0) return HALO_OK;
    const unsigned blocks = (unsigned)((total4 + 255) / 256 < 2048 ? (total4 + 255) / 256 : 2048);
    hipLaunchKernelGGL(pack_ranges_bf16_kernel, dim3(blocks), dim3(256), 0, (hipStream_t)stream, src, r, (__bf16 *)dst);
    return halo_launch_status();
}

int halo_expand_ranges_bf16(const void *stage, int n, const size_t *begin, const size_t *chunk, int world, int skip_rank, float *dst,
                            halo_stream_t stream) {
    HALO_CHECK_ARG(stage && dst && world >= 1 && ((uintptr_t)dst % 16 == 0) && ((uintptr_t)stage % 8 == 0));
    Ranges8 r; size_t total4;
    size_t end[8];
    if (n < 1 || n > 8 || !begin || !chunk) return HALO_EINVAL;
    for (int k = 0; k < n; ++k) end[k] = begin[k] + chunk[k];
    { const int rc = make_ranges8(n, begin, end, r, total4); if (rc != HALO_OK) return rc; }
    if (total4 == 0) return HALO_OK;
    const size_t all4 = total4 * (size_t)world;
    const unsigned blocks = (unsigned)((all4 + 255) / 256 < 4096 ? (all4 + 255) / 256 : 4096);
    hipLaunchKernelGGL(expand_ranges_bf16_kernel, dim3(blocks), dim3(256), 0, (hipStream_t)stream, (const __bf16 *)stage, r, world, skip_rank, dst);
    return halo_launch_status();
}

int halo_clip_coef_step(const float *partials, int count, float max_norm, float *coef, float *norm_out, uint32_t *applied_steps,
                        halo_stream_t stream) {
    HALO_CHECK_ARG(partials && coef && count > 0);
    hipLaunchKernelGGL(clip_coef_kernel, dim3(1), dim3(256), 0, (hipStream_t)stream, partials, count, max_norm, coef,
                       norm_out, applied_steps, (const uint32_t *)halo_ctx_cur().status);
    return halo_launch_status();
}

int halo_clip_coef(const float *partials, int count, float max_norm, float *coef, float *norm_out,
                   halo_stream_t stream) {
    return halo_clip_coef_step(partials, count, max_norm, coef, norm_out, nullptr, stream);
}

int halo_adamw(float *p, const float *g, float *m, float *v, size_t n, float lr, float beta1, float beta2, float eps,
               float weight_decay, int step, const float *grad_scale, halo_stream_t stream) {
    HALO_CHECK_ARG(p && g && m && v && step >= 1);
    HALO_CHECK_ARG(((uintptr_t)p % 16 == 0) && ((uintptr_t)g % 16 == 0) && ((uintptr_t)m % 16 == 0) &&
                   ((uintptr_t)v % 16 == 0));
    if (n == 0) return HALO_OK;
    AdamArgs a;
    a.p = p; a.g = g; a.m = m; a.v = v; a.n = n;
    const double bc1 = 1.0 - pow((double)beta1, (double)step);
    const double bc2 = 1.0 - pow((double)beta2, (double)step);
    a.decay_mul = (float)(1.0 - (double)lr * (double)weight_decay);
    a.beta1_w = (float)(1.0 - (double)beta1);
    a.beta2 = beta2;
    a.beta2_w = (float)(1.0 - (double)beta2);
    a.step_size = (float)((double)lr / bc1);
    a.bc2_sqrt = (float)sqrt(bc2);
    a.eps = eps;
    a.grad_scale = grad_scale;
    size_t blocks = (n / 4 + 255) / 256;
    if (blocks < 1) blocks = 1;
    if (blocks > 2048) blocks = 2048;
    hipLaunchKernelGGL(adamw_kernel, dim3((unsigned)blocks), dim3(256), 0, (hipStream_t)stream, a);
    return halo_launch_status();
}

size_t halo_adamw_multi_tensor_bytes(void) { return sizeof(AdamTensor); }
unsigned halo_adamw_multi_chunk(void) { return ADAM_CHUNK; }

int halo_adamw_multi_max_tensors(void) { return ADAM_MULTI_MAX; }

int halo_adamw_multi(const void *tensor_table, const void *chunk_table, int n_chunks, const float *const *grads, int n_tensors, float lr,
                     float beta1, float beta2, float eps, int step, const float *grad_scale, halo_stream_t stream) {
    HALO_CHECK_ARG(tensor_table && chunk_table && n_chunks > 0 && step >= 1 && grads && n_tensors > 0 && n_tensors <= ADAM_MULTI_MAX);
    AdamGrads gr;
    for (int i = 0; i < ADAM_MULTI_MAX; ++i) gr.g[i] = i < n_tensors ? grads[i] : nullptr;
    for (int i = 0; i < n_tensors; ++i) HALO_CHECK_ARG(grads[i] != nullptr);
    const double bc1 = 1.0 - pow((double)beta1, (double)step);
    const double bc2 = 1.0 - pow((double)beta2, (double)step);
    hipLaunchKernelGGL(adamw_multi_kernel, dim3((unsigned)n_chunks), dim3(256), 0, (hipStream_t)stream, (const AdamTensor *)tensor_table,
                       (const uint2 *)chunk_table, gr, lr, (float)(1.0 - (double)beta1), beta2, (float)(1.0 - (double)beta2),
                       (float)((double)lr / bc1), (float)sqrt(bc2), eps, grad_scale);
    return halo_launch_status();
}

static int adamw_ranges_impl(float *p, const float *g, float *m, float *v, int n_ranges, const size_t *begin, const size_t *end,
                      const float *weight_decay, const float *const *grad_scale, float lr, float beta1, float beta2, float eps, int step,
                      const uint32_t *step_dev, const float *lr_dev, uint32_t *counter, halo_stream_t stream) {
    HALO_CHECK_ARG(p && g && m && v && begin && end && weight_decay && grad_scale && n_ranges > 0 && n_ranges <= ADAM_MAX_RANGES &&
                   (step >= 1 || step_dev) && (!lr_dev || step_dev));
    HALO_CHECK_ARG(((uintptr_t)p % 16 == 0) && ((uintptr_t)g % 16 == 0) && ((uintptr_t)m % 16 == 0) && ((uintptr_t)v % 16 == 0));
    AdamRangesArgs a;
    a.p = p; a.g = g; a.m = m; a.v = v; a.n_ranges = n_ranges; a.counter = counter;
    a.step_dev = step_dev; a.lr_dev = lr_dev; a.lr = lr; a.beta1 = beta1;
    if (step < 1) step = 1;
    size_t biggest = 0;
    for (int r = 0; r < n_ranges; ++r) {
        HALO_CHECK_ARG(begin[r] % 4 == 0 && end[r] % 4 == 0 && begin[r] <= end[r]);
        a.begin4[r] = begin[r] / 4; a.end4[r] = end[r] / 4;
        a.decay_mul[r] = (float)(1.0 - (double)lr * (double)weight_decay[r]);
        a.weight_decay[r] = weight_decay[r];
        a.grad_scale[r] = grad_scale[r];
        if (a.end4[r] - a.begin4[r] > biggest) biggest = a.end4[r] - a.begin4[r];
    }
    const double bc1 = 1.0 - pow((double)beta1, (double)step);
    const double bc2 = 1.0 - pow((double)beta2, (double)step);
    a.beta1_w = (float)(1.0 - (double)beta1);
    a.beta2 = beta2;
    a.beta2_w = (float)(1.0 - (double)beta2);
    a.step_size = (float)((double)lr / bc1);
    a.bc2_sqrt = (float)sqrt(bc2);
    a.eps = eps;
    size_t blocks = (biggest + 255) / 256;
    if (blocks > 4096) blocks = 4096;
    if (blocks < 1) blocks = 1;
    static int nt = -1;
    if (nt < 0) { const char *e = getenv("HALO_ADAMW_NT"); nt = (e && e[0] == '0') ? 0 : 1; }
    if (nt) hipLaunchKernelGGL(adamw_ranges_kernel<true>, dim3((unsigned)blocks), dim3(256), 0, (hipStream_t)stream, a);
    else hipLaunchKernelGGL(adamw_ranges_kernel<false>, dim3((unsigned)blocks), dim3(256), 0, (hipStream_t)stream, a);
    return halo_launch_status();
}

int halo_adamw_ranges(float *p, const float *g, float *m, float *v, int n_ranges, const size_t *begin, const size_t *end,
                      const float *weight_decay, const float *const *grad_scale, float lr, float beta1, float beta2, float eps, int step,
                      uint32_t *counter, halo_stream_t stream) {
    return adamw_ranges_impl(p, g, m, v, n_ranges, begin, end, weight_decay, grad_scale, lr, beta1, beta2, eps, step, nullptr, nullptr,
                             counter, stream);
}

int halo_adamw_ranges_dev(float *p, const float *g, float *m, float *v, int n_ranges, const size_t *begin, const size_t *end,
                          const float *weight_decay, const float *const *grad_scale, float lr, const float *lr_dev, float beta1, float beta2,
                          float eps, const uint32_t *step_dev, uint32_t *counter, halo_stream_t stream) {
    HALO_CHECK_ARG(step_dev);
    return adamw_ranges_impl(p, g, m, v, n_ranges, begin, end, weight_decay, grad_scale, lr, beta1, beta2, eps, 0, step_dev, lr_dev,
                             counter, stream);
}

}
```

haloop_amd/ops.py:

```python
import ctypes as C
from collections import namedtuple

import torch

from . import _lib
from ._lib import check, lib, ptr, ptr_array


def _stream():
    return torch._C._cuda_getCurrentRawStream(torch.cuda.current_device())


def _f32c(t, name):
    if t.dtype != torch.float32 or not t.is_cuda or not t.is_contiguous():
        raise ValueError(f'{name}: expected a contiguous float32 HIP tensor, got {t.dtype} {t.device} '
                         f'contiguous={t.is_contiguous()}')
    return t


class Dropout:
    __slots__ = ('p', 'seed', 'offset', 'counter')

    def __init__(self, p=0.0, seed=0, offset=0, counter=None):
        self.p, self.seed, self.offset, self.counter = float(p), int(seed), int(offset), counter
# ... 318 lines not shown
    R = LORA_RANK_PAD
    buf = torch.empty(lib().halo_lora_pack_bytes(n_in, n_out) // 2, device=A.device, dtype=torch.bfloat16)
    check(lib().halo_lora_pack(ptr(A), ptr(B), r, n_in, n_out, ptr(buf), _stream()), 'halo_lora_pack')
    na, nb = R * n_in, R * n_out
    return (buf[:na].view(R, n_in), buf[na:2 * na].view(n_in, R), buf[2 * na:2 * na + nb].view(n_out, R), buf[2 * na + nb:].view(R, n_out))


def _bf16_rows(t, name, cols=None):
    if t.dtype != torch.bfloat16 or not t.is_cuda or t.dim() != 2 or t.stride(1) != 1 or (cols is not None and t.shape[1] != cols):
        raise ValueError(f'{name}: expected row-major bf16 rows on the HIP device')
    return t


def lora_down(x, p16, scale=1.0, drop=NO_DROPOUT, stream_id=0):
    _bf16_rows(x, 'x'); _bf16_rows(p16, 'p16')
    M, K = x.shape
    if p16.shape != (LORA_RANK_PAD, K) or not p16.is_contiguous():
        raise ValueError('lora_down: p16 [16, K]')
    u = torch.empty(M, LORA_RANK_PAD, device=x.device, dtype=torch.bfloat16)
    check(lib().halo_lora_down(ptr(x), x.stride(0), ptr(p16), M, K, float(scale), ptr(u), drop.p, drop.seed, stream_id, drop.offset,
                               drop.counter_ptr, _stream()), 'halo_lora_down')
    return u


def lora_up_(y, u, p16, scale=1.0, drop=NO_DROPOUT, stream_id=0):
    _bf16_rows(u, 'u', LORA_RANK_PAD); _bf16_rows(p16, 'p16', LORA_RANK_PAD)
    M, N = y.shape
    if y.dtype not in (torch.bfloat16, torch.float32) or y.stride(1) != 1 or u.shape[0] != M or p16.shape[0] != N \
            or not u.is_contiguous() or not p16.is_contiguous():
        raise ValueError('lora_up_: y [M, N] bf16 / fp32 rows, u [M, 16], p16 [N, 16]')
    b16 = y.dtype == torch.bfloat16
    check(lib().halo_lora_up(ptr(u), ptr(p16), M, N, float(scale), ptr(y) if b16 else None, None if b16 else ptr(y), y.stride(0), drop.p,
                             drop.seed, stream_id, drop.offset, drop.counter_ptr, _stream()), 'halo_lora_up')
    return y


def lora_tn(u, x, r, scale=1.0, transpose_out=False, drop=NO_DROPOUT, stream_id=0):
    _bf16_rows(u, 'u', LORA_RANK_PAD); _bf16_rows(x, 'x')
    M, K = x.shape
    if u.shape[0] != M or not u.is_contiguous():
        raise ValueError('lora_tn: u [M, 16] contiguous')
    g = torch.empty((K, r) if transpose_out else (r, K), device=x.device, dtype=torch.float32)
    ws = torch.empty(lib().halo_lora_tn_workspace_bytes(M, K), device=x.device, dtype=torch.uint8)
    check(lib().halo_lora_tn(ptr(u), ptr(x), x.stride(0), M, K, r, float(scale), int(transpose_out), ptr(g), ptr(ws), drop.p, drop.seed,
                             stream_id, drop.offset, drop.counter_ptr, _stream()), 'halo_lora_tn')
    return g


def dropout_fwd(x, drop, stream_id):
    _f32c(x, 'x')
    y = torch.empty_like(x)
    check(lib().halo_dropout_fwd(ptr(x), ptr(y), x.numel(), drop.p, drop.seed, stream_id, drop.offset,
                                 drop.counter_ptr, _stream()), 'halo_dropout_fwd')
    return y


def subsample_fwd(x, w, bias, drop, ks=5, stride=4, pad=3):
    _f32c(x, 'inputs'); _f32c(w, 'subsample.weight'); _f32c(bias, 'subsample.bias')
    B, T, F = x.shape
    Cc = w.shape[0]
    Tp = subsampled_length(T, ks, stride, pad)
    y = torch.empty(Tp, B, Cc, device=x.device, dtype=torch.float32)
    col = torch.empty(Tp * B, F * ks, device=x.device, dtype=torch.float32)
    check(lib().halo_subsample_fwd(ptr(x), ptr(w), ptr(bias), ptr(y), ptr(col), B, T, F, Cc, ks, stride, pad,
                                   drop.p, drop.seed, drop.offset, drop.counter_ptr, _stream()), 'halo_subsample_fwd')
    return y, col


def subsample_bwd(dy, y, col, B, T, F, Cc, p_drop, dw=None, dbias=None, ks=5, stride=4, pad=3, slabs=1):
    _f32c(dy, 'dy')
    if slabs > 1 and dy.numel() < slabs * y.numel():
        raise ValueError('haloop_amd.ops.subsample_bwd: dy holds fewer than `slabs` matrices')
    dpre = torch.empty_like(y)
    if dw is None:
        dw = torch.empty(Cc, F, ks, device=y.device, dtype=torch.float32)
    if dbias is None:
        dbias = torch.empty(Cc, device=y.device, dtype=torch.float32)
    check(lib().halo_subsample_bwd_slabs(ptr(dy), int(slabs), ptr(y), ptr(col), ptr(dpre), ptr(dw), ptr(dbias), B, T, F, Cc, ks, stride,
                                         pad, p_drop, _stream()), 'halo_subsample_bwd_slabs')
    return dw, dbias


def lstm_fwd(x_tm, w_ih, w_hh, b_ih, b_hh, h0=None, c0=None, y=None, y_strides=None, y_relu=False,
             want_state=False, drop=NO_DROPOUT, expect_backward=True, reserve=None, weights_stamp=0):
    _f32c(x_tm, 'x')
    T, B, in0 = x_tm.shape
    L = len(w_hh)
    H = w_hh[0].shape[1]
    for t in list(w_ih) + list(w_hh) + list(b_ih) + list(b_hh):
        _f32c(t, 'lstm parameter')
    dev = x_tm.device
    if y is None:
        y = torch.empty(T, B, H, device=dev, dtype=torch.float32)
        y_strides = (B * H, H)
    need = (lib().halo_lstm_reserve_bytes(T, B, in0, H, L) + 3) // 4
    if reserve is None:
        reserve = torch.empty(need, device=dev, dtype=torch.float32)
    elif reserve.dtype != torch.float32 or reserve.numel() < need or not reserve.is_contiguous():
        raise ValueError('lstm_fwd: the reserve is too small for this shape (ops.lstm_reserve)')
    hn = torch.empty(L, B, H, device=dev, dtype=torch.float32) if want_state else None
    cn = torch.empty(L, B, H, device=dev, dtype=torch.float32) if want_state else None
    if h0 is not None:
        _f32c(h0, 'h0'); _f32c(c0, 'c0')
    a_ih, a_hh, a_bi, a_bh = ptr_array(w_ih), ptr_array(w_hh), ptr_array(b_ih), ptr_array(b_hh)
    if not expect_backward:
        lib().halo_set_lstm_expect_backward(0)
        lib().halo_set_lstm_weights_stamp(int(weights_stamp))
    try:
        check(lib().halo_lstm_fwd(ptr(x_tm), a_ih, a_hh, a_bi, a_bh, ptr(h0), ptr(c0), ptr(y), y_strides[0], y_strides[1],
                                  int(y_relu), ptr(hn), ptr(cn), ptr(reserve), T, B, in0, H, L, drop.p, drop.seed,
                                  drop.offset, drop.counter_ptr, _stream()), 'halo_lstm_fwd')
    finally:
        if not expect_backward:
            lib().halo_set_lstm_expect_backward(1)
            lib().halo_set_lstm_weights_stamp(0)
    return y, hn, cn, reserve


def lstm_reserve(T, B, in0, H, L, device):
    return torch.empty((lib().halo_lstm_reserve_bytes(T, B, in0, H, L) + 3) // 4, device=device, dtype=torch.float32)


def lstm_bwd_workspace(x_tm, w_hh):
    T, B, in0 = x_tm.shape
    return torch.empty((lib().halo_lstm_bwd_workspace_bytes(T, B, in0, w_hh[0].shape[1], len(w_hh)) + 3) // 4,
                       device=x_tm.device, dtype=torch.float32)


def lstm_bwd(x_tm, w_ih, w_hh, dy, y_strides, y_relu, reserve, dhn=None, dcn=None, want_dx=False,
             grads=None, drop=NO_DROPOUT, layers=None, workspace=None, dx=None, dx_slabs=1):
    T, B, in0 = x_tm.shape
    L = len(w_hh)
    H = w_hh[0].shape[1]
    dev = x_tm.device
    if grads is None:
        grads = {
            'dw_ih': [torch.empty_like(w) for w in w_ih],
            'dw_hh': [torch.empty_like(w) for w in w_hh],
            'db_ih': [torch.empty(4 * H, device=dev, dtype=torch.float32) for _ in range(L)],
            'db_hh': [torch.empty(4 * H, device=dev, dtype=torch.float32) for _ in range(L)],
        }
    ws = workspace if workspace is not None else lstm_bwd_workspace(x_tm, w_hh)
    lo, hi = layers if layers is not None else (0, L)
    if dx is None and want_dx and lo == 0:
        dx = torch.empty(T, B, in0, device=dev, dtype=torch.float32)
    a_ih, a_hh = ptr_array(w_ih), ptr_array(w_hh)
    g_ih, g_hh = ptr_array(grads['dw_ih']), ptr_array(grads['dw_hh'])
    g_bi, g_bh = ptr_array(grads['db_ih']), ptr_array(grads['db_hh'])
    if dx_slabs > 1:
        if dx is None or dx.numel() < dx_slabs * T * B * in0:
            raise ValueError('haloop_amd.ops.lstm_bwd: dx_slabs needs a dx buffer of that many [T, B, in] matrices')
        check(lib().halo_set_lstm_dx_slabs(int(dx_slabs)), 'halo_set_lstm_dx_slabs')
    try:
        check(lib().halo_lstm_bwd(ptr(x_tm), a_ih, a_hh, ptr(dy), y_strides[0], y_strides[1], int(y_relu), ptr(dhn),
                                  ptr(dcn), ptr(reserve), ptr(ws), ptr(dx), g_ih, g_hh, g_bi, g_bh, T, B, in0, H, L, lo, hi,
                                  drop.p, drop.seed, drop.offset, drop.counter_ptr, _stream()), 'halo_lstm_bwd')
    finally:
        if dx_slabs > 1:
            lib().halo_set_lstm_dx_slabs(1)
    return dx, grads


def relu_dropout_bwd(dy, y, p_drop):
    _f32c(dy, 'dy'); _f32c(y, 'y')
    if dy.numel() != y.numel():
        raise ValueError('haloop_amd.ops.relu_dropout_bwd: dy and y differ in size')
    dpre = torch.empty_like(y)
    check(lib().halo_relu_dropout_bwd(ptr(dy), ptr(y), ptr(dpre), y.numel(), float(p_drop), _stream()), 'halo_relu_dropout_bwd')
    return dpre


def _ghost_operand(t, time_major, N, T, name):
    if t.dtype != torch.float32 or not t.is_cuda or t.dim() != 3 or (t.shape[2] > 1 and t.stride(2) != 1):
        raise ValueError(f'{name}: expected a 3-d float32 HIP tensor with unit stride along K')
    n_dim, t_dim = (1, 0) if time_major else (0, 1)
    if t.shape[n_dim] != N or t.shape[t_dim] != T:
        raise ValueError(f'{name}: shape {tuple(t.shape)} does not hold N = {N} utterances of T = {T} frames')
    return _lib.GhostOperand(t.data_ptr(), t.stride(n_dim), t.stride(t_dim), t.shape[2])


def ghost_term(a, bs=(), n_bias=0, time_major=False):
    bs = tuple(bs)
    if len(bs) > 2 or not 0 <= int(n_bias) <= 2:
        raise ValueError('haloop_amd.ops.ghost_term: at most two b operands and two bias vectors')
    N, T = (a.shape[1], a.shape[0]) if time_major else (a.shape[0], a.shape[1])
    tm = _lib.GhostTerm()
    tm.a = _ghost_operand(a, time_major, N, T, 'a')
    for j, b in enumerate(bs):
        tm.b[j] = _ghost_operand(b, time_major, N, T, f'b{j}')
    tm.n_b, tm.n_bias = len(bs), int(n_bias)
    tm.tensors = (a,) + bs
    return tm


def lstm_ghost_terms(x_tm, reserve, H, L, p_drop=0.0):
    _f32c(x_tm, 'x')
    T, B, in0 = x_tm.shape
    arr = (_lib.GhostTerm * L)()
    check(lib().halo_lstm_ghost_terms(ptr(x_tm), ptr(reserve), T, B, in0, H, L, float(p_drop), arr), 'halo_lstm_ghost_terms')
    terms = []
    for l in range(L):
        tm = _lib.GhostTerm.from_buffer_copy(arr[l])
        tm.tensors = (x_tm, reserve)
# ... 248 lines not shown
    lens = torch.empty(N, beam, device=dev, dtype=torch.int32)
    scores = torch.empty(N, beam, device=dev, dtype=torch.float32)
    ws = torch.empty(lib().halo_ctc_beam_workspace_bytes(N, T, V, beam), device=dev, dtype=torch.uint8)
    check(lib().halo_ctc_beam(ptr(em), N, T, V, beam, int(log_domain), ptr(seqs), ptr(lens), ptr(scores), ptr(ws),
                              _stream()), 'halo_ctc_beam')
    return seqs, lens, scores


def logaddexp_aten(a, b):
    _f32c(a, 'a'); _f32c(b, 'b')
    out = torch.empty_like(a)
    check(lib().halo_logaddexp_aten(ptr(a), ptr(b), ptr(out), a.numel(), _stream()), 'halo_logaddexp_aten')
    return out


def topk(values2d, k):
    _f32c(values2d, 'values')
    rows, n = values2d.shape
    dev = values2d.device
    vals = torch.empty(rows, k, device=dev, dtype=torch.float32)
    idx = torch.empty(rows, k, device=dev, dtype=torch.int64)
    ws = torch.empty(rows * n * 8, device=dev, dtype=torch.uint8)
    check(lib().halo_topk_f32(ptr(values2d), rows, n, k, ptr(vals), ptr(idx), ptr(ws), _stream()), 'halo_topk_f32')
    return vals, idx


def sumsq_partials(flat, partials=None):
    if partials is None:
        partials = torch.empty(_lib.HALO_SUMSQ_PARTS, device=flat.device, dtype=torch.float32)
    check(lib().halo_sumsq(ptr(flat), flat.numel(), ptr(partials), _stream()), 'halo_sumsq')
    return partials


def _range_arrays(ranges):
    n = len(ranges)
    return n, (C.c_size_t * n)(*[int(r[0]) for r in ranges]), (C.c_size_t * n)(*[int(r[1]) for r in ranges])


def sumsq_ranges(flat, ranges, partials):
    n, b, e = _range_arrays(ranges)
    check(lib().halo_sumsq_ranges(ptr(flat), n, b, e, ptr(partials), _stream()), 'halo_sumsq_ranges')
    return partials


def pack_ranges_bf16(flat, ranges, dst):
    n, b, e = _range_arrays(ranges)
    check(lib().halo_pack_ranges_bf16(ptr(flat), n, b, e, ptr(dst), _stream()), 'halo_pack_ranges_bf16')
    return dst


def expand_ranges_bf16(stage, spans, chunks, world, skip_rank, flat):
    n = len(spans)
    b = (C.c_size_t * n)(*[int(s) for s in spans])
    c = (C.c_size_t * n)(*[int(x) for x in chunks])
    check(lib().halo_expand_ranges_bf16(ptr(stage), n, b, c, int(world), int(skip_rank), ptr(flat), _stream()), 'halo_expand_ranges_bf16')
    return flat


GRAD_SUMSQ_ALL = 31


def collect_grad_sumsq(partials):
    check(lib().halo_set_grad_sumsq(ptr(partials), 0 if partials is None else partials.numel()), 'halo_set_grad_sumsq')


def grad_sumsq_state():
    n, bits = C.c_int(0), C.c_uint(0)
    check(lib().halo_grad_sumsq_state(C.byref(n), C.byref(bits)), 'halo_grad_sumsq_state')
    return int(n.value), int(bits.value)


def clip_coef(partials, count, max_norm, coef, norm, applied_steps=None):
    check(lib().halo_clip_coef_step(ptr(partials), count, float(max_norm), ptr(coef), ptr(norm), ptr(applied_steps), _stream()),
          'halo_clip_coef_step')


def adamw(p, g, m, v, lr, beta1, beta2, eps, weight_decay, step, grad_scale=None):
    _lib.bump_weights_epoch()
    check(lib().halo_adamw(ptr(p), ptr(g), ptr(m), ptr(v), p.numel(), lr, beta1, beta2, eps, weight_decay, step,
                           ptr(grad_scale), _stream()), 'halo_adamw')
    torch.autograd.graph.increment_version(p)


def adamw_ranges(p, g, m, v, ranges, lr, beta1, beta2, eps, step, counter=None):
    _lib.bump_weights_epoch()
    n = len(ranges)
    begin = (C.c_size_t * n)(*[r[0] for r in ranges])
    end = (C.c_size_t * n)(*[r[1] for r in ranges])
    wd = (C.c_float * n)(*[float(r[2]) for r in ranges])
    gs = (C.c_void_p * n)(*[ptr(r[3]) for r in ranges])
    if torch.is_tensor(step):
        lr_dev = lr if torch.is_tensor(lr) else None
        check(lib().halo_adamw_ranges_dev(ptr(p), ptr(g), ptr(m), ptr(v), n, begin, end, wd, gs, 0.0 if lr_dev is not None else lr,
                                          ptr(lr_dev), beta1, beta2, eps, ptr(step), ptr(counter), _stream()), 'halo_adamw_ranges_dev')
    else:
        check(lib().halo_adamw_ranges(ptr(p), ptr(g), ptr(m), ptr(v), n, begin, end, wd, gs, lr, beta1, beta2, eps, step, ptr(counter),
                                      _stream()), 'halo_adamw_ranges')
    torch.autograd.graph.increment_version(p)


class AdamWMulti:

    def __init__(self, params, weight_decays, lr, betas=(0.9, 0.999), eps=1e-8):
        import numpy as np
        self.params = list(params)
        self.wds = [float(w) for w in weight_decays]
        self.param_groups = [{'lr': float(lr), 'params': self.params}]
        self.betas, self.eps = betas, float(eps)
        for p in self.params:
            if p.dtype != torch.float32 or not p.is_contiguous() or not p.is_cuda:
                raise ValueError('AdamWMulti: parameters must be contiguous float32 tensors on the HIP device')
        self.m = [torch.zeros_like(p) for p in self.params]
        self.v = [torch.zeros_like(p) for p in self.params]
        self.t = 0
        dev = self.params[0].device
        chunk, group = lib().halo_adamw_multi_chunk(), lib().halo_adamw_multi_max_tensors()
        assert lib().halo_adamw_multi_tensor_bytes() == 40
        rec = np.dtype([('p', '<u8'), ('m', '<u8'), ('v', '<u8'), ('n', '<u8'), ('decay', '<f4'), ('pad', '<i4')])
        self.groups = []
        for first in range(0, len(self.params), group):
            idx = range(first, min(first + group, len(self.params)))
            table = np.zeros(len(idx), dtype=rec)
            for k, i in enumerate(idx):
                p = self.params[i]
                table[k] = (p.data_ptr(), self.m[i].data_ptr(), self.v[i].data_ptr(), p.numel(), self.wds[i], 0)
            pairs = [(k, c) for k, i in enumerate(idx) for c in range((self.params[i].numel() + chunk - 1) // chunk)]
            self.groups.append((first, len(idx), torch.from_numpy(table.view(np.uint8)).to(dev),
                                torch.tensor(pairs, dtype=torch.int32).view(-1).to(dev), len(pairs)))

    @property
    def lr(self):
        return self.param_groups[0]['lr']

    @lr.setter
    def lr(self, value):
        self.param_groups[0]['lr'] = float(value)

    def step(self, grad_scale=None):
        _lib.bump_weights_epoch()
        self.t += 1
        for first, count, table, chunks, n_chunks in self.groups:
            ptrs = (C.c_void_p * count)()
            for k in range(count):
                p = self.params[first + k]
                g = p.grad
                if g is None or g.dtype != torch.float32 or not g.is_contiguous() or g.device != p.device or g.shape != p.shape:
                    raise ValueError('AdamWMulti.step: every parameter needs a contiguous float32 .grad of its shape on its device')
                ptrs[k] = g.data_ptr()
            check(lib().halo_adamw_multi(ptr(table), ptr(chunks), n_chunks, ptrs, count, self.lr, self.betas[0], self.betas[1], self.eps,
                                         self.t, ptr(grad_scale), _stream()), 'halo_adamw_multi')
        for p in self.params:
            torch.autograd.graph.increment_version(p)


def scale_add_(y, x, alpha, beta, guard=None):
    check(lib().halo_scale_add_guarded(ptr(y), ptr(x), float(alpha), float(beta), y.numel(), ptr(guard), _stream()),
          'halo_scale_add_guarded')
    return y


def cast_f32_to_bf16_(dst_bf16, src_f32):
    check(lib().halo_cast_f32_bf16(ptr(src_f32), ptr(dst_bf16), src_f32.numel(), _stream()), 'halo_cast_f32_bf16')
    return dst_bf16


def cast_bf16_to_f32_(dst_f32, src_bf16, scale=1.0):
    check(lib().halo_cast_bf16_f32(ptr(src_bf16), ptr(dst_f32), float(scale), dst_f32.numel(), _stream()), 'halo_cast_bf16_f32')
    return dst_f32


def counter_inc(counter):
    check(lib().halo_counter_inc(ptr(counter), _stream()), 'halo_counter_inc')


# ... 810 lines not shown
```

haloop_amd/train.py:

```python
import os
import re
import time

import torch

from . import _lib, _linear, dp, ops
from .ops import Dropout, NO_DROPOUT
from .rnn import lstm_param_list


def decay_groups(encoder, recognizer):
    decay, no_decay = [], []
    for prefix, mod in (('encoder.', encoder), ('recognizer.', recognizer)):
        for name, p in mod.named_parameters():
            is_lstm = name.startswith('lstm.') or name.startswith('rnn.')
            if is_lstm or not name.endswith('bias'):
                decay.append((prefix + name, p))
            else:
                no_decay.append((prefix + name, p))
    return decay, no_decay


def _merge_adjacent(ranges):
    out = []
# ... 61 lines not shown
    def attach_grads(self):
        for n, p, _ in self.slots:
            p.grad = self.grad_views[n]


class LstmCtcTrainer:
    DX_SLABS = int(os.environ.get('HALO_DX_SLABS', '8'))

    def __init__(self, encoder, recognizer, lr=3e-4, betas=(0.9, 0.99), eps=1e-8, weight_decay=0.01,
                 clip_grad_norm=0.1, seed=None, use_graph=True, process_group=None, accumulate=1, grad_dtype='f32',
                 alias_loss=False, fused_head=True, head_one_launch=True, dp_algo='rs_ag', rehearse_dp=False, gather_dtype='f32'):
        self.alias_loss = bool(alias_loss)
        self.fused_head = fused_head
        self.head_one_launch = head_one_launch
        self.encoder, self.recognizer = encoder, recognizer
        self.accumulate = int(accumulate)
        self._micro = 0
        self.betas, self.eps, self.weight_decay, self.clip = betas, eps, weight_decay, clip_grad_norm
        if dp_algo not in ('rs_ag', 'rs_ag_flat', 'allreduce', 'direct'):
            raise ValueError(f"dp_algo must be 'rs_ag', 'direct', 'rs_ag_flat' or 'allreduce', got {dp_algo!r}")
        if gather_dtype not in ('auto', 'f32', 'bf16'):
            raise ValueError(f"gather_dtype must be 'auto', 'f32' or 'bf16', got {gather_dtype!r}")
        self.world = dp.world_size(process_group)
        self.dp_algo = dp_algo if ((self.world > 1 or rehearse_dp) and self.accumulate == 1) else 'allreduce'
        if self.dp_algo in ('rs_ag', 'direct') and grad_dtype == 'bf16':
            self.dp_algo = 'rs_ag_flat'
        self._rehearse_dp = bool(rehearse_dp)
        self.flat = FlatParams(encoder, recognizer, pad_to=4 * self.world if self.dp_algo != 'allreduce' else 4)
        dev = self.flat.params.device
        self._lr_dev = torch.zeros(1, device=dev, dtype=torch.float32)
        self.lr = lr
        self.status = torch.zeros(1, device=dev, dtype=torch.int32)
        _lib.set_status_word(self.status)
        _lib.lend_scratch(device=dev)
        self.device = dev
        self.seed = int(torch.initial_seed() if seed is None else seed) & 0xFFFFFFFFFFFFFFFF
        self.counter = torch.zeros(1, device=dev, dtype=torch.int32)
        self.partials = torch.zeros(_lib.HALO_SUMSQ_PARTS, device=dev, dtype=torch.float32)
        self.partials_p = torch.zeros(4 * _lib.HALO_SUMSQ_PARTS, device=dev, dtype=torch.float32)
        self.coef = torch.ones(2, device=dev, dtype=torch.float32)
        self.grad_norm = torch.zeros(1, device=dev, dtype=torch.float32)
        self.loss = torch.zeros((), device=dev, dtype=torch.float32)
        self.step_count = 0
        self.adam_step = torch.zeros(1, device=dev, dtype=torch.int32)
        self._ticket = torch.zeros(1, device=dev, dtype=torch.int32)
        auto = use_graph == 'auto'
        if auto:
            use_graph = True
        self.use_graph = use_graph
        self._auto = {'n': 0} if (auto and self.world == 1 and not rehearse_dp and self.accumulate == 1) else None
        self.auto_choice = None
        self.eager_forward_backward = os.environ.get('HALO_DP_EAGER_FB', '1') != '0'
        self.pg = process_group
        dp.broadcast_parameters(self.flat.params, process_group)
        self.sharded = None
        self.masters_stale = False
        self._gather_mode = None
        if self.dp_algo in ('rs_ag', 'direct'):
            f = self.flat
            bf16_gather = gather_dtype == 'bf16' or (gather_dtype == 'auto' and _lib.get_math_mode() == 'bf16')
            self._gather_mode = _lib.get_math_mode()
            try:
                if self.dp_algo == 'direct':
                    self.sharded = dp.DirectExchange(f.params, f.grads, f.big_early, f.big_late, f.small_range, process_group,
                                                     gather_bf16=bf16_gather, norm_parts=self.partials.numel())
                else:
                    self.sharded = dp.SpanSharded(f.params, f.grads, f.big_early, f.big_late, f.small_range, process_group,
                                                  always=self._rehearse_dp, gather_bf16=bf16_gather)
            except ValueError as e:
                import logging
                logging.getLogger(__name__).warning('haloop_amd.train: %s; using dp_algo rs_ag_flat', e)
                self.dp_algo = 'rs_ag_flat'
            else:
                self._mid_event = torch.cuda.Event() if dev.type == 'cuda' else None
                if self._mid_event is not None:
                    self._mid_event.record()
        if self.dp_algo == 'rs_ag_flat':
            self.sharded = dp.ShardedUpdate(self.flat.params, self.flat.grads, process_group, always=self._rehearse_dp, wire_dtype=grad_dtype)
        self.avg_early = dp.GradientAverager(self.flat.grads, process_group, span=self.flat.early_range, wire_dtype=grad_dtype)
        self.avg_late = dp.GradientAverager(self.flat.grads, process_group, span=self.flat.late_range, wire_dtype=grad_dtype)
        self._graphs = None
        self._static = None
        self._accum = torch.zeros_like(self.flat.grads) if self.accumulate > 1 else None

    @property
    def lr(self):
        return self._lr

    @lr.setter
    def lr(self, value):
        self._lr = float(value)
        self._lr_dev.fill_(self._lr)

    def check_status(self):
        if int(self.status.item()) != 0:
            raise _lib.HaloError('a persistent LSTM recurrence timed out waiting for its peer workgroups (they were not all resident); '
                                 'no optimizer update has been applied since.  Free the GPU of other work, or select the step-launch '
                                 'chain with haloop_amd._lib.set_lstm_persistent(False), then zero trainer.status and continue.')

    def _dropout(self):
        p = self.encoder.dropout.p if self.encoder.training else 0.0
        return Dropout(p, self.seed, 0, self.counter) if p > 0 else NO_DROPOUT

    def _forward_backward(self, x, il, tg, tl):
        self._backward_rest(self._forward_backward_top(x, il, tg, tl))

    def _forward_backward_top(self, x, il, tg, tl):
        self._defer = not (self.world > 1 and self.dp_algo == 'allreduce')
        if self._defer:
            ops.defer_small_jobs.begin()
        self._norm_count = 0
        self._collect = self._defer and self.world == 1 and self.sharded is None and self.accumulate == 1 and self.encoder.lstm.num_layers == 2
        if self._collect:
            ops.collect_grad_sumsq(self.partials_p)
        try:
            return self._forward_backward_top_body(x, il, tg, tl)
        except BaseException:
            if self._defer:
                self._defer = False
                _lib.lib().halo_set_defer_small_jobs(0)
            if self._collect:
                self._collect = False
                _lib.lib().halo_set_grad_sumsq(None, 0)
            raise

    def _forward_backward_top_body(self, x, il, tg, tl):
        enc, rec, gv = self.encoder, self.recognizer, self.flat.grad_views
        drop = self._dropout()
        B, T, F = x.shape
        L = enc.lstm.num_layers
        lp_list = lstm_param_list(enc.lstm)
        w_ih, w_hh, b_ih, b_hh = lp_list[0::4], lp_list[1::4], lp_list[2::4], lp_list[3::4]
        H, Cc = w_hh[0].shape[1], enc.subsample.weight.shape[0]
        V = rec.classifier.weight.shape[0]
        y_sub, col = ops.subsample_fwd(x, enc.subsample.weight, enc.subsample.bias, drop)
        Tp = y_sub.shape[0]
        feats = torch.empty(B, Tp, H, device=x.device, dtype=torch.float32)
        _, _, _, reserve = ops.lstm_fwd(y_sub, w_ih, w_hh, b_ih, b_hh, y=feats, y_strides=(H, Tp * H), y_relu=True, drop=drop)
        p_cls = rec.dropout.p if rec.training else 0.0
        cdrop = Dropout(p_cls, self.seed, 0, self.counter) if p_cls > 0 else NO_DROPOUT
        grads = {'dw_ih': [gv[f'encoder.lstm.weight_ih_l{k}'] for k in range(L)],
                 'dw_hh': [gv[f'encoder.lstm.weight_hh_l{k}'] for k in range(L)],
                 'db_ih': [gv[f'encoder.lstm.bias_ih_l{k}'] for k in range(L)],
                 'db_hh': [gv[f'encoder.lstm.bias_hh_l{k}'] for k in range(L)]}
        if self.fused_head and ops.ctc_head_supported(Tp, H, V, tg.shape[1]):
            sid = _lib.HALO_STREAM_CLASSIFIER
            if self.head_one_launch and _lib.get_math_mode() != 'f32':
                if getattr(self, '_head_tws', None) is None or self._head_tws_dims != (B, H, V):
                    self._head_tws, self._head_tws_dims = ops.ctc_head_train_workspace(B, H, V, x.device), (B, H, V)
                    self._head_ticket = ops.ctc_head_train_ticket(B, H, x.device)
                dfeats, _, _, _ = ops.ctc_head_train(feats, rec.classifier.weight, rec.classifier.bias, cdrop, sid, il, tg, tl, self.loss,
                                                     self._head_ticket, gv['recognizer.classifier.weight'], gv['recognizer.classifier.bias'],
                                                     workspace=self._head_tws)
                return self._lstm_backward_top(x, y_sub, col, w_ih, w_hh, reserve, grads, drop, dfeats.view(B * Tp, H),
                                               (B, T, F, Cc, H, Tp, L))
            lp, alpha, nll, flen, grad_out, (tg64, tl64) = ops.ctc_head_fwd(feats, rec.classifier.weight, rec.classifier.bias, cdrop, sid,
                                                                           il, tg, tl, self.loss, self._ticket)
            if getattr(self, '_head_ws', None) is None or self._head_ws_dims != (B, H, V):
                self._head_ws, self._head_ws_dims = ops.ctc_head_workspace(B, H, V, x.device), (B, H, V)
            dfeats = ops.ctc_head_bwd(feats, rec.classifier.weight, cdrop, sid, flen, tg64, tl64, lp, alpha, nll, grad_out,
                                      gv['recognizer.classifier.weight'], gv['recognizer.classifier.bias'],
                                      workspace=self._head_ws).view(B * Tp, H)
            return self._lstm_backward_top(x, y_sub, col, w_ih, w_hh, reserve, grads, drop, dfeats, (B, T, F, Cc, H, Tp, L))
        fdrop = ops.dropout_fwd(feats, cdrop, _lib.HALO_STREAM_CLASSIFIER) if p_cls > 0 else feats
        f2d = fdrop.view(B * Tp, H)
        logits = ops.gemm(f2d, rec.classifier.weight, True, True, B * Tp, V, H, bias1=rec.classifier.bias)
        lp = ops.log_softmax_fwd(logits)
        flen, grad_out = ops.ctc_prepare(il, tl)
        nll, alpha, saved = ops.ctc_fwd(lp.view(B, Tp, V), False, tg, flen, tl)
        ops.ctc_mean_loss(nll, tl, self.loss)
        dlp = ops.ctc_bwd(lp.view(B, Tp, V), False, saved, alpha, nll, grad_out)
        dlogits = ops.log_softmax_bwd(dlp.view(B * Tp, V), lp)
        ops.gemm(dlogits, f2d, False, False, V, H, B * Tp, out=gv['recognizer.classifier.weight'])
        ops.colsum(dlogits, out=gv['recognizer.classifier.bias'])
        dfeats = ops.gemm(dlogits, rec.classifier.weight, True, False, B * Tp, H, V, drop=cdrop,
                          stream_id=_lib.HALO_STREAM_CLASSIFIER)
        return self._lstm_backward_top(x, y_sub, col, w_ih, w_hh, reserve, grads, drop, dfeats, (B, T, F, Cc, H, Tp, L))

    def _lstm_backward_top(self, x, y_sub, col, w_ih, w_hh, reserve, grads, drop, dfeats, dims):
        B, T, F, Cc, H, Tp, L = dims
        ws = ops.lstm_bwd_workspace(y_sub, w_hh)
        dy_sub = torch.empty((self.DX_SLABS,) + tuple(y_sub.shape), device=y_sub.device, dtype=torch.float32)
        top = (L - 1 if L > 1 else 0) if (self.world > 1 and self.dp_algo == 'allreduce') else 0
        ops.lstm_bwd(y_sub, w_ih, w_hh, dfeats, (H, Tp * H), True, reserve, grads=grads, drop=drop, layers=(top, L),
                     workspace=ws, dx=dy_sub, dx_slabs=self.DX_SLABS)
        self._dx_slabs = ops.lstm_dx_slabs_left() if top == 0 else 1
        return (y_sub, col, w_ih, w_hh, reserve, grads, drop, ws, dy_sub, top, (B, T, F, Cc, H, Tp, L))

    def _backward_rest(self, st):
        y_sub, col, w_ih, w_hh, reserve, grads, drop, ws, dy_sub, top, (B, T, F, Cc, H, Tp, L) = st
        gv = self.flat.grad_views
        if top > 0:
            if self.world > 1:
                if getattr(self, '_ctx_steps', None) is None:
                    self._ctx_steps = _lib.Context()
                    with self._ctx_steps:
                        _lib.set_lstm_persistent(False)
                with self._ctx_steps:
                    ops.lstm_bwd(y_sub, w_ih, w_hh, None, (H, Tp * H), True, reserve, grads=grads, drop=drop, layers=(0, top),
                                 workspace=ws, dx=dy_sub)
            else:
                ops.lstm_bwd(y_sub, w_ih, w_hh, None, (H, Tp * H), True, reserve, grads=grads, drop=drop, layers=(0, top),
                             workspace=ws, dx=dy_sub)
        try:
            ops.subsample_bwd(dy_sub, y_sub, col, B, T, F, Cc, drop.p, dw=gv['encoder.subsample.weight'],
                              dbias=gv['encoder.subsample.bias'], slabs=self._dx_slabs)
        finally:
            if self._defer:
                self._defer = False
                ops.defer_small_jobs.end()
            if self._collect:
                self._collect = False
                n, bits = ops.grad_sumsq_state()
                ops.collect_grad_sumsq(None)
                self._norm_count = n if bits == ops.GRAD_SUMSQ_ALL else 0

    def _all_reduce(self):
        self.avg_early.average()
        self.avg_late.average()

    def _warm_optimizer_kernels(self):
        dev = self.device
        d = [torch.zeros(8, device=dev, dtype=torch.float32) for _ in range(4)]
        parts = torch.zeros(_lib.HALO_SUMSQ_PARTS, device=dev, dtype=torch.float32)
        coef, norm = torch.ones(2, device=dev, dtype=torch.float32), torch.zeros(1, device=dev, dtype=torch.float32)
        cnt = torch.ones(1, device=dev, dtype=torch.int32)
        ops.sumsq_partials(d[1], parts)
        ops.clip_coef(parts, _lib.HALO_SUMSQ_PARTS, self.clip, coef, norm, applied_steps=cnt)
        ops.adamw_ranges(d[0], d[1], d[2], d[3], [(0, 8, 0.0, coef[0:1])], self.lr, self.betas[0], self.betas[1], self.eps, cnt)

    def _optimizer(self):
        if getattr(self, '_norm_count', 0) > 0 and self.sharded is None:
            self._apply_update(count=self._norm_count)
            return
        self._norm_partials()
        self._apply_update()

    def _own_ranges(self):
        if isinstance(self.sharded, dp.SpanSharded):
            return self.sharded.own_ranges()
        if self.sharded is not None:
            return [self.sharded.span]
        return [(0, self.flat.padded)]

    def _norm_partials(self):
        f = self.flat
        src = self.sharded.norm_ranges() if isinstance(self.sharded, dp.SpanSharded) else self._own_ranges()
        cut = [(max(f.encoder_range[0], lo), min(f.encoder_range[1], hi)) for lo, hi in src]
        cut = _merge_adjacent([(a, b) for a, b in cut if b > a])
        if not cut:
            self.partials.zero_()
        elif len(cut) == 1:
            ops.sumsq_partials(f.grads[cut[0][0]:cut[0][1]], self.partials)
        else:
            ops.sumsq_ranges(f.grads, cut, self.partials)

    def _apply_update(self, count=None):
        f = self.flat
        ops.clip_coef(self.partials_p if count else self.partials, count or _lib.HALO_SUMSQ_PARTS, self.clip, self.coef, self.grad_norm,
                      applied_steps=self.adam_step)
        ranges = [(max(a, lo), min(b, hi), self.weight_decay if decays else 0.0, self.coef[0:1] if clipped else self.coef[1:2])
                  for a, b, decays, clipped in f.ranges for lo, hi in _merge_adjacent(self._own_ranges()) if min(b, hi) > max(a, lo)]
        if ranges:
            ops.adamw_ranges(f.params, f.grads, f.exp_avg, f.exp_avg_sq, ranges, self._lr_dev, self.betas[0], self.betas[1], self.eps,
                             self.adam_step, counter=self.counter)
        else:
            ops.counter_inc(self.counter)

    def _sharded_tail(self):
        sh = self.sharded
        mark = self._dp_mark
        if isinstance(sh, dp.SpanSharded):
            if not self._early_started:
                sh.reduce_scatter('early')
            mark('reduce_scatter_early_tail')
            sh.reduce_scatter('late')
            mark('reduce_scatter_late')
            sh.all_reduce_small()
            mark('all_reduce_small')
        else:
            sh.reduce_scatter()
            mark('reduce_scatter')
        self._norm_partials()
        sh.all_reduce_sum(self.partials)
        mark('norm_partials_and_their_all_reduce')
        self._apply_update()
        mark('clip_and_adamw_on_owned_ranges')
        sh.all_gather()
        mark('all_gather')

    _dp_marks = None

    def _dp_mark(self, name):
        if self._dp_marks is not None:
            ev = torch.cuda.Event(enable_timing=True)
            ev.record()
            self._dp_marks.append((name, ev))

    def profile_dp_components(self, x, il, tg, tl, steps=5):
        if self.sharded is None:
            return None
        was_graph, self.use_graph = self.use_graph, False
        acc = {}
        try:
            for it in range(steps + 1):
                self._dp_marks = []
                start = torch.cuda.Event(enable_timing=True)
                start.record()
                self._early_started = False
                self.masters_stale = bool(getattr(self.sharded, 'gather_bf16', False))
                handle = self._forward_backward_overlapped(x, il, tg, tl)
                self._dp_mark('forward_backward')
                if handle is not None:
                    self.sharded.wait(handle)
                    self._early_started = True
                self._dp_mark('wait_early_reduce_scatter')
                self._sharded_tail()
                torch.cuda.synchronize()
                if it > 0:
                    prev = start
                    for name, ev in self._dp_marks:
                        acc[name] = acc.get(name, 0.0) + 1e3 * prev.elapsed_time(ev) / steps
                        prev = ev
                    acc['step_total'] = acc.get('step_total', 0.0) + 1e3 * start.elapsed_time(prev) / steps
        finally:
            self._dp_marks = None
            self.use_graph = was_graph
        return {k: round(v, 1) for k, v in acc.items()}

    def gather_master_weights(self):
        if isinstance(self.sharded, dp.SpanSharded) and self.sharded.gather_bf16:
            self.sharded.gather_masters()
            _lib.bump_weights_epoch()
        self.masters_stale = False

    def state_dict(self):
        if self.masters_stale:
            self.gather_master_weights()
        return {'encoder': self.encoder.state_dict(), 'recognizer': self.recognizer.state_dict()}

    def step(self, x, input_lengths, targets, target_lengths):
        if self._auto is not None:
            loss = self._auto_step(x, input_lengths, targets, target_lengths)
        else:
            loss = self._step(x, input_lengths, targets, target_lengths)
        return loss if self.alias_loss else loss.clone()

    _AUTO = (8, 28, 33, 53)

    def _auto_step(self, x, il, tg, tl):
        a, (w0, g1, w1, e1) = self._auto, self._AUTO
        a['n'] += 1
        n = a['n']
        if n == w0 + 1 or n == w1 + 1:
            torch.cuda.synchronize()
            a['t0'] = time.perf_counter()
        self.use_graph = n <= g1
        loss = self._step(x, il, tg, tl)
        if n == g1 or n == e1:
            torch.cuda.synchronize()
            a['graph' if n == g1 else 'eager'] = time.perf_counter() - a['t0']
        if n == e1:
            self.use_graph = not (a['eager'] / (e1 - w1) < 0.99 * a['graph'] / (g1 - w0))
            self.auto_choice = {'graph_replay_ms': 1e3 * a['graph'] / (g1 - w0), 'eager_launches_ms': 1e3 * a['eager'] / (e1 - w1),
                                'use_graph': self.use_graph}
            self._auto = None
        return loss

    def _step(self, x, input_lengths, targets, target_lengths):
        if _lib._status_tensor is not self.status:
            _lib.set_status_word(self.status)
        if self.accumulate > 1:
            return self._accumulating_step(x, input_lengths, targets, target_lengths)
        self.step_count += 1
        if self.sharded is not None:
            if self._gather_mode is not None and getattr(self.sharded, 'gather_bf16', False) and _lib.get_math_mode() != self._gather_mode:
                self.gather_master_weights()
                self.sharded.gather_bf16 = False
                self._tail_graph, self._tail_calls = None, 0
            return self._sharded_step(x, input_lengths, targets, target_lengths)
        if not self.use_graph:
            st = self._forward_backward_top(x, input_lengths, targets, target_lengths)
            w1 = self.avg_early.start()
            self._backward_rest(st)
            w2 = self.avg_late.start()
            self.avg_early.finish(w1)
            self.avg_late.finish(w2)
            self._optimizer()
            return self.loss
        return self._graph_step(x, input_lengths, targets, target_lengths)

    def _forward_backward_overlapped(self, x, il, tg, tl):
        sh = self.sharded
        ev = self._mid_event if (isinstance(sh, dp.SpanSharded) and (sh._native or getattr(sh, 'side_ok', False)) and 'early' in sh.spans) else None
        if ev is None:
            self._forward_backward(x, il, tg, tl)
            return None
        _lib.set_lstm_bwd_mid_event(ev)
        try:
            st = self._forward_backward_top(x, il, tg, tl)
            recorded = _lib.lib().halo_lstm_bwd_mid_event_recorded() == 1
        finally:
            _lib.set_lstm_bwd_mid_event(None)
        handle = sh.reduce_scatter('early', after=ev) if recorded else None
        self._backward_rest(st)
        return handle

    def _sharded_step(self, x, il, tg, tl):
        handle = None
        self._early_started = False
        self.masters_stale = bool(getattr(self.sharded, 'gather_bf16', False))
        if not self.use_graph or self.eager_forward_backward:
            handle = self._forward_backward_overlapped(x, il, tg, tl)
        else:
            self._replay_forward_backward(x, il, tg, tl)
        if handle is not None:
            self.sharded.wait(handle)
            self._early_started = True
        if not self.use_graph:
            self._sharded_tail()
            return self.loss
        self._tail_calls = getattr(self, '_tail_calls', 0) + 1
        want_capture = os.environ.get('HALO_DP_CAPTURE', '1' if self.world == 1 else '0') != '0'
        if self._tail_calls == 2 and self.sharded._native and want_capture:
            try:
                torch.cuda.synchronize()
                g = torch.cuda.CUDAGraph()
                with torch.cuda.graph(g, capture_error_mode='thread_local'):
                    self._sharded_tail()
                self._tail_graph, self._tail_graph_early = g, self._early_started
            except Exception as e:
                import logging
                logging.getLogger(__name__).warning('haloop_amd.train: capturing the collectives failed (%s: %s); they run eagerly',
                                                    type(e).__name__, e)
                torch.cuda.synchronize()
                self._tail_graph = None
        if getattr(self, '_tail_graph', None) is not None and self._tail_graph_early == self._early_started:
            _lib.bump_weights_epoch()
            self._tail_graph.replay()
        else:
            self._sharded_tail()
        return self.loss

    def _accumulating_step(self, x, il, tg, tl):
        if self.use_graph:
            self._replay_forward_backward(x, il, tg, tl)
        else:
            self._forward_backward(x, il, tg, tl)
        self._micro += 1
        first, last = self._micro == 1, self._micro == self.accumulate
        ops.scale_add_(self._accum, self.flat.grads, 0.0 if first else 1.0, 1.0 / self.accumulate, guard=self.loss)
        if not last:
            ops.counter_inc(self.counter)
            return self.loss
        self._micro = 0
        self.flat.grads.copy_(self._accum)
        self._all_reduce()
        self.step_count += 1
        self._optimizer()
        return self.loss

    def _replay_forward_backward(self, x, il, tg, tl):
        if self._graphs is None or len(self._graphs) != 1 or self._static[0].shape != x.shape or self._static[2].shape != tg.shape:
            self._static = tuple(t.contiguous().clone() for t in (x, il.to(torch.int64), tg.to(torch.int64), tl.to(torch.int64)))
            sx, sil, stg, stl = self._static
            side = torch.cuda.Stream()
            side.wait_stream(torch.cuda.current_stream())
            with torch.cuda.stream(side):
                self._forward_backward(sx, sil, stg, stl)
            torch.cuda.current_stream().wait_stream(side)
            g = torch.cuda.CUDAGraph()
            with torch.cuda.graph(g):
                self._forward_backward(sx, sil, stg, stl)
# ... 107 lines not shown
```

include/halo.h:

```cpp
#ifndef HALO_H
#define HALO_H

#include <stddef.h>
#include <stdint.h>

#ifdef __cplusplus
extern "C" {
#endif

#define HALO_ABI_VERSION 21

#define HALO_OK 0
#define HALO_EINVAL (-22)
#define HALO_ENOTSUP (-95)
#define HALO_ELAUNCH (-5)

typedef void *halo_stream_t;

int halo_abi_version(void);
int halo_debug_read(const void *src, size_t bytes, int pattern, size_t row_bytes, float *sink, void *stream);
const char *halo_strerror(int code);
int halo_device_info(int device, char *arch, int arch_len, int *cu_count);

#define HALO_MATH_F32 0
// ... 66 lines not shown
                            float *const *C, const long *ldc, halo_stream_t stream);

int halo_gemm_split_io(const void *a_image, const void *a_hi, const void *a_lo, long lda, const void *b_image, int M, int N, int K, float *C,
                       int ldc, void *out_hi, void *out_lo, long ldo, const float *residual, int ldr, const float *bias1,
                       const float *bias2, int flags, halo_stream_t stream);

int halo_attention_fwd_b16(const void *q, long q_row_stride, long q_batch_stride, const void *k, const void *v, long kv_row_stride,
                           long kv_batch_stride, float *y, long y_row_stride, long y_batch_stride, void *y_bf16, long yb_row_stride,
                           long yb_batch_stride, float *lse, int N, int heads, int head_dim, int Tq, int Tk, int causal, halo_stream_t stream);
int halo_attention_bwd_b16(const void *q, long q_row_stride, long q_batch_stride, const void *k, const void *v, long kv_row_stride,
                           long kv_batch_stride, const void *y_bf16, const void *dy_bf16, long y_row_stride, long y_batch_stride, const float *lse,
                           float *delta, void *dq_bf16, void *dk_bf16, void *dv_bf16, long d_row_stride, long d_batch_stride, int N, int heads,
                           int head_dim, int Tq, int Tk, int causal, halo_stream_t stream);

int halo_gemm_rows_supported(int M, int N, int K);
int halo_gemm_rows(const void *a_image, const void *a_bf16, long lda, const void *b_image, int M, int N, int K, float *C, long ldc,
                   const float *residual, long ldr, void *out_bf16, long ldo, halo_stream_t stream);
int halo_gemm_rows_gelu(const void *a_image, const void *a_bf16, long lda, const void *b_image, int M, int N, int K, void *out_bf16,
                        void *pre_bf16, long ldo, int exact, halo_stream_t stream);
size_t halo_gemm_rows_ce_workspace_bytes(int M, int N);
int halo_gemm_rows_ce(const void *a_image, const void *a_bf16, long lda, const void *b_image, int M, int N, int K, const int64_t *targets,
                      long ignore_index, void *workspace, float *loss, float *lse, void *logits_bf16, long ldo, halo_stream_t stream);
int halo_cross_entropy_bwd_bf16(void *logits_bf16, const int64_t *targets, const float *lse, const float *grad, long grad_stride, int rows,
                                int V, long ld, long ignore_index, halo_stream_t stream);

int halo_lora_supported(int M, int n_in, int n_out, int r);
size_t halo_lora_pack_bytes(int n_in, int n_out);
int halo_lora_pack(const float *A, const float *B, int r, int n_in, int n_out, void *packed, halo_stream_t stream);
int halo_lora_down(const void *x_bf16, long ldx, const void *p16, int M, int K, float scale, void *u_bf16, float p_drop, uint64_t seed,
                   uint32_t stream_id, uint32_t offset, const uint32_t *offset_dev, halo_stream_t stream);
int halo_lora_up(const void *u_bf16, const void *p16, int M, int N, float scale, void *y_bf16, float *y_f32, long ldy, float p_drop,
                 uint64_t seed, uint32_t stream_id, uint32_t offset, const uint32_t *offset_dev, halo_stream_t stream);
size_t halo_lora_tn_workspace_bytes(int M, int K);
int halo_lora_tn(const void *u_bf16, const void *x_bf16, long ldx, int M, int K, int r, float scale, int transpose_out, float *g,
                 void *workspace, float p_drop, uint64_t seed, uint32_t stream_id, uint32_t offset, const uint32_t *offset_dev,
                 halo_stream_t stream);

size_t halo_gemm_split_ce_workspace_bytes(int M, int N);
int halo_gemm_split_ce(const void *a_image, const void *b_image, int M, int N, int K, float *logits, int ldc, const float *bias,
                       const int64_t *targets, long ignore_index, void *workspace, float *loss, float *lse, halo_stream_t stream);

size_t halo_subsample_col_bytes(int B, int T, int F, int ks, int stride, int pad);
int halo_subsample_fwd(const float *x, const float *w, const float *bias, float *y, float *col, int B,
                       int T, int F, int C, int ks, int stride, int pad, float p_drop, uint64_t seed,
                       uint32_t offset, const uint32_t *offset_dev, halo_stream_t stream);
int halo_subsample_bwd(const float *dy, const float *y, const float *col, float *dpre, float *dw,
                       float *dbias, int B, int T, int F, int C, int ks, int stride, int pad, float p_drop,
                       halo_stream_t stream);
int halo_subsample_bwd_slabs(float *dy, int slabs, const float *y, const float *col, float *dpre, float *dw,
                             float *dbias, int B, int T, int F, int C, int ks, int stride, int pad, float p_drop,
                             halo_stream_t stream);

size_t halo_lstm_reserve_bytes(int T, int B, int in0, int H, int L);
size_t halo_lstm_bwd_workspace_bytes(int T, int B, int in0, int H, int L);
int halo_lstm_fwd(const float *x, const float *const *w_ih, const float *const *w_hh,
                  const float *const *b_ih, const float *const *b_hh, const float *h0, const float *c0,
                  float *y, long y_stride_t, long y_stride_b, int y_relu, float *hn, float *cn,
                  float *reserve, int T, int B, int in0, int H, int L, float p_drop, uint64_t seed,
                  uint32_t offset, const uint32_t *offset_dev, halo_stream_t stream);
int halo_lstm_bwd(const float *x, const float *const *w_ih, const float *const *w_hh, const float *dy,
                  long y_stride_t, long y_stride_b, int y_relu, const float *dhn, const float *dcn,
                  float *reserve, float *workspace, float *dx, float *const *dw_ih, float *const *dw_hh,
                  float *const *db_ih, float *const *db_hh, int T, int B, int in0, int H, int L,
                  int layer_begin, int layer_end, float p_drop, uint64_t seed, uint32_t offset,
                  const uint32_t *offset_dev, halo_stream_t stream);

typedef struct halo_ctx halo_ctx;
halo_ctx *halo_ctx_create(void);
void halo_ctx_destroy(halo_ctx *ctx);
int halo_ctx_use(halo_ctx *ctx);
int halo_set_status_word(uint32_t *device_word);
int halo_debug_mute_workgroup(int block);
int halo_debug_mfma_clock(unsigned long long *ticks, float *sink, int blocks, int iters, int shape, unsigned seed, halo_stream_t stream);

int halo_set_lstm_persistent(int on);
int halo_set_lstm_persistent_images(int on);
int halo_lstm_persistent_eligible(int B, int H);
int halo_set_lstm_persistent2(int on);
int halo_set_lstm_interleave(int on);
int halo_set_gemm256(int on);
int halo_set_lstm_bwd_mid_event(void *event);
int halo_lstm_bwd_mid_event_recorded(void);
int halo_set_lstm_weights_stamp(uint64_t stamp);
int halo_set_lstm_expect_backward(int on);
int halo_set_lstm_dx_slabs(int n);
int halo_lstm_dx_slabs_left(void);
int halo_set_defer_small_jobs(int on);
int halo_flush_small_jobs(halo_stream_t stream);
int halo_set_grad_sumsq(float *partials, int capacity);
int halo_grad_sumsq_state(int *count, unsigned *covered);
int halo_lstm_persistent2_eligible(int T, int B, int H, int L);
size_t halo_lstm_status_offset(int backward, int T, int B, int in0, int H, int L);

typedef struct halo_ghost_operand {
    const float *ptr;
    long stride_n, stride_t;
    int K;
} halo_ghost_operand;
typedef struct halo_ghost_term {
    halo_ghost_operand a;
    halo_ghost_operand b[2];
    int n_b, n_bias;
} halo_ghost_term;
int halo_ghost_tile(void);
size_t halo_ghost_sqnorm_workspace_bytes(int n_terms, int N, int T);
int halo_ghost_sqnorm(const halo_ghost_term *terms, int n_terms, int N, int T, float *workspace, float *sq, float *norm,
                      halo_stream_t stream);
int halo_set_lstm_keep_gate_gradients(int on);
int halo_get_lstm_keep_gate_gradients(void);
int halo_lstm_ghost_terms(const float *x, float *reserve, int T, int B, int in0, int H, int L, float p_drop, halo_ghost_term *terms_out);
int halo_relu_dropout_bwd(const float *dy, const float *y, float *dpre, size_t n, float p_drop, halo_stream_t stream);

int halo_lstm_persist_stamps(void *device_buffer);

int halo_lstm_chain_events(void *ev_begin, void *ev_end);
int halo_lstm_chain_info(int backward, int *launches, char *kernel, int kernel_len);

int halo_log_softmax_fwd(const float *x, float *y, int rows, int cols, halo_stream_t stream);
int halo_log_softmax_bwd(const float *dy, const float *y, float *dx, int rows, int cols,
                         halo_stream_t stream);
int halo_colsum(const float *x, int rows, int cols, int ld, float *out, halo_stream_t stream);

#define HALO_CTC_FULL_LATTICE 1
#define HALO_CTC_FINITE_MIN 2
#define HALO_CTC_NO_LEAD_BLANK_LOOP 4
#define HALO_CTC_WRAP_SKIP 8
int halo_ctc_fwd(const float *lp, long stride_t, long stride_n, int T, int N, int C,
                 const int64_t *targets, long tg_stride, int S, const int64_t *input_lengths,
                 const int64_t *target_lengths, int flags, float *alpha, float *nll,
                 halo_stream_t stream);
int halo_ctc_bwd(const float *lp, long stride_t, long stride_n, int T, int N, int C,
                 const int64_t *targets, long tg_stride, int S, const int64_t *input_lengths,
                 const int64_t *target_lengths, const float *alpha, const float *nll,
                 const float *grad_out, float *beta, float *grad, long gstride_t, long gstride_n,
                 halo_stream_t stream);

int halo_ctc_prepare(const int64_t *input_lengths, const int64_t *target_lengths, int n, int ks, int stride,
                     int pad, int64_t *feature_lengths, float *grad_out, halo_stream_t stream);
int halo_ctc_mean_loss(const float *nll, const int64_t *target_lengths, int n, float *loss,
                       halo_stream_t stream);

int halo_ctc_head_greedy(const float *features, const float *weight, const float *bias, float *lp, int64_t *alignments, float *scores,
                         int64_t *hyp, int64_t *hyp_len, int B, int T, int H, int V, halo_stream_t stream);
int halo_ctc_head_supported(int T, int H, int V, int S);
size_t halo_ctc_head_workspace_bytes(int B, int H, int V);
int halo_ctc_head_fwd(const float *features, const float *weight, const float *bias, float p_drop, uint64_t seed,
                      uint32_t stream_id, uint32_t offset, const uint32_t *offset_dev, const int64_t *input_lengths, int ks,
                      int stride, int pad, const int64_t *targets, long tg_stride, int S, const int64_t *target_lengths,
                      float *lp, float *alpha, float *nll, int64_t *feature_lengths, float *grad_out, float *loss,
                      uint32_t *ticket, int B, int T, int H, int V, halo_stream_t stream);
int halo_ctc_head_bwd(const float *features, const float *weight, float p_drop, uint64_t seed, uint32_t stream_id,
                      uint32_t offset, const uint32_t *offset_dev, const int64_t *feature_lengths, const int64_t *targets,
                      long tg_stride, int S, const int64_t *target_lengths, const float *lp, const float *alpha,
                      const float *nll, const float *grad_out, float *dfeatures, float *dweight, float *dbias,
                      void *workspace, int B, int T, int H, int V, halo_stream_t stream);

size_t halo_ctc_head_train_workspace_bytes(int B, int H, int V);
size_t halo_ctc_head_train_ticket_words(int B, int H);
int halo_ctc_head_train(const float *features, const float *weight, const float *bias, float p_drop, uint64_t seed,
                        uint32_t stream_id, uint32_t offset, const uint32_t *offset_dev, const int64_t *input_lengths, int ks,
                        int stride, int pad, const int64_t *targets, long tg_stride, int S, const int64_t *target_lengths,
                        float *lp, float *nll, int64_t *feature_lengths, float *loss, uint32_t *ticket, float *dfeatures,
                        float *dweight, float *dbias, void *workspace, int B, int T, int H, int V, halo_stream_t stream);

int halo_ctc_greedy(const float *lp, int N, int T, int C, int64_t *alignments, float *scores,
                    int64_t *hyp, int64_t *hyp_len, halo_stream_t stream);
// ... 177 lines not shown
                            int heads, int head_dim, int Tq, int Tk, int causal, const int *key_lengths, float p_drop, uint64_t seed,
                            uint32_t stream_id, uint32_t offset, const uint32_t *offset_dev, halo_stream_t stream);
size_t halo_layernorm_bwd_workspace_bytes(int rows, int C);
int halo_layernorm_bwd(const float *dy, const float *x, const float *weight, const float *dres, float *dx,
                       float *dweight, float *dbias, void *workspace, int rows, int C, float eps,
                       halo_stream_t stream);
int halo_layernorm_bwd_bf16(const float *dy, const float *x, const float *weight, const float *dres, float *dx, void *dx_bf16,
                            float *dweight, float *dbias, void *workspace, int rows, int C, float eps, halo_stream_t stream);
int halo_layernorm_bwd_b16(const void *dy_bf16, const float *x, const float *weight, const float *dres, float *dx, void *dx_bf16, float *dweight,
                           float *dbias, void *workspace, int rows, int C, float eps, halo_stream_t stream);
int halo_gelu_fwd(const float *a, float *y, size_t n, int exact, halo_stream_t stream);
int halo_gelu_bwd(const float *dy, const float *a, float *da, size_t n, int exact, halo_stream_t stream);
int halo_cross_entropy_fwd_lse(const float *logits, const int64_t *targets, float *loss, float *lse, int rows, int V,
                               long ld, long ignore_index, halo_stream_t stream);
int halo_cross_entropy_bwd(float *logits, const int64_t *targets, const float *lse, const float *grad,
                           long grad_stride, int rows, int V, long ld, long ignore_index, halo_stream_t stream);
int halo_embed_bwd(const int64_t *ids, const float *dx, float *dwte, float *dwpe, int B, int T, int C, int pos0,
                   int vocab, int accumulate_wpe, halo_stream_t stream);
int halo_embed_bwd_ordered(const int64_t *ids, const float *dx, float *dwte, int n, int C, int vocab, halo_stream_t stream);
int halo_add_rows_bcast(float *x, const float *p, int rows, int T, int C, halo_stream_t stream);

int halo_im2col_cl(const float *x, float *col, int N, int T, int Cin, int ks, int stride, int pad,
                   halo_stream_t stream);
int halo_col2im_cl(const float *dcol, float *dx, int N, int T, int Cin, int ks, int stride, int pad,
                   halo_stream_t stream);
int halo_dwconv1d_cl(const float *x, const float *weight, const float *bias, float *y, int N, int T, int C, int ks,
                     int stride, int pad, halo_stream_t stream);
size_t halo_dwconv1d_cl_bwd_workspace_bytes(int C, int ks);
int halo_dwconv1d_cl_bwd(const float *dy, const float *x, const float *weight, float *dx, float *dweight,
                         float *dbias, void *workspace, int N, int T, int C, int ks, int stride, int pad,
                         halo_stream_t stream);

int halo_tape_batch(const void *data, int elem_bytes, long n_tokens, int batch_size, int bptt_len, long part_index,
                    int rows, long pad_value, void *out, halo_stream_t stream);
int halo_lm_batch_u16(const uint16_t *data, long n_tokens, const int64_t *offsets, int B, int T, int objective_cond,
                      int64_t *x, int64_t *y, halo_stream_t stream);

int halo_mask_tokens(int64_t *inputs, int64_t *labels, long n, float mlm_probability, long mask_token, long endoftext_token,
                     long max_token, uint64_t seed, uint32_t step, halo_stream_t stream);
int halo_mlm_batch_u16(const uint16_t *data, long n_tokens, const int64_t *offsets, int B, int T, float mlm_probability,
                       long mask_token, long endoftext_token, long max_token, uint64_t seed, uint32_t step, int64_t *x, int64_t *y,
                       halo_stream_t stream);
int halo_target_rows(const int64_t *targets, int M, long ignore_index, int capacity, int limit, int *rows, int64_t *targets_c,
                     int *slot, int *count, halo_stream_t stream);
int halo_gather_rows(const float *src, const int *rows, int M, int K, int C, float *dst, halo_stream_t stream);
int halo_scatter_rows(const float *src, const int *slot, const int *count, int capacity, int limit, int M, int C, float *dst,
                      void *dst_bf16, halo_stream_t stream);

#define HALO_SUMSQ_PARTS 1024
int halo_scale_add(float *y, const float *x, float alpha, float beta, size_t n, halo_stream_t stream);
int halo_scale_add_guarded(float *y, const float *x, float alpha, float beta, size_t n, const float *guard,
                           halo_stream_t stream);
int halo_cast_f32_bf16(const float *x, void *y_bf16, size_t n, halo_stream_t stream);
int halo_cast_bf16_f32(const void *x_bf16, float *y, float scale, size_t n, halo_stream_t stream);
int halo_sumsq(const float *x, size_t n, float *partials, halo_stream_t stream);
int halo_dx_alloc(size_t bytes, void **ptr, void *handle64);
int halo_dx_open(const void *handle64, void **ptr);
int halo_dx_close(void *ptr);
int halo_dx_free(void *ptr);
int halo_dx_push(const void *src, size_t piece_bytes, size_t piece_stride_bytes, int same, void *const *peer_bases, size_t dst_offset, int world,
                 int rank, halo_stream_t stream);
int halo_dx_signal(void *const *peer_bases, size_t flag_offset, int world, int rank, uint32_t epoch, halo_stream_t stream);
int halo_dx_wait(const void *own_flags, int world, int rank, uint32_t epoch, halo_stream_t stream);
int halo_dx_reduce(float *own, const float *inbox, size_t elems, int world, int rank, float scale, halo_stream_t stream);

int halo_sumsq_ranges(const float *x, int n, const size_t *begin, const size_t *end, float *partials, halo_stream_t stream);
int halo_pack_ranges_bf16(const float *src, int n, const size_t *begin, const size_t *end, void *dst, halo_stream_t stream);
int halo_expand_ranges_bf16(const void *stage, int n, const size_t *begin, const size_t *chunk, int world, int skip_rank, float *dst,
                            halo_stream_t stream);
int halo_clip_coef(const float *partials, int count, float max_norm, float *coef, float *norm_out,
                   halo_stream_t stream);
int halo_clip_coef_step(const float *partials, int count, float max_norm, float *coef, float *norm_out,
                        uint32_t *applied_steps, halo_stream_t stream);
int halo_adamw(float *p, const float *g, float *m, float *v, size_t n, float lr, float beta1, float beta2,
               float eps, float weight_decay, int step, const float *grad_scale, halo_stream_t stream);
int halo_adamw_ranges(float *p, const float *g, float *m, float *v, int n_ranges, const size_t *begin, const size_t *end,
                      const float *weight_decay, const float *const *grad_scale, float lr, float beta1, float beta2,
                      float eps, int step, uint32_t *counter, halo_stream_t stream);

int halo_adamw_ranges_dev(float *p, const float *g, float *m, float *v, int n_ranges, const size_t *begin, const size_t *end,
                          const float *weight_decay, const float *const *grad_scale, float lr, const float *lr_dev, float beta1,
                          float beta2, float eps, const uint32_t *step_dev, uint32_t *counter, halo_stream_t stream);

size_t halo_adamw_multi_tensor_bytes(void);
unsigned halo_adamw_multi_chunk(void);
int halo_adamw_multi_max_tensors(void);
int halo_adamw_multi(const void *tensor_table, const void *chunk_table, int n_chunks, const float *const *grads, int n_tensors,
                     float lr, float beta1, float beta2, float eps, int step, const float *grad_scale, halo_stream_t stream);

#ifdef __cplusplus
}
#endif
#endif
```

Before: 158,700 utterances/s.

## Fuse bf16 LSTM pair-image packing into the AdamW update

The AdamW kernel gains an images variant: for the three recurrent LSTM weight matrices it writes the updated weights straight into the bf16 forward and transposed tiled images held in a persistent reserve. The next forward pass can then skip the pack-pair tile work, because a 'current' flag marks the images as already fresh. This removes a separate read of the fp32 weights plus a repack each step. In exchange it adds reserve-lifetime bookkeeping, a version key that triggers a refill when needed, LDS transposes inside the optimizer, and extra paths that need the bf16 mode and H divisible by 256.

```diff
diff --git a/haloop_amd/_lib.py b/haloop_amd/_lib.py
--- a/haloop_amd/_lib.py
+++ b/haloop_amd/_lib.py
@@ -106,6 +106,9 @@
     'halo_flush_small_jobs': (_i, [_vp]),
     'halo_lstm_dx_slabs_left': (_i, []),
     'halo_set_lstm_weights_stamp': (_i, [_u64]),
+    'halo_set_lstm_pair_images_current': (_i, [_vp]),
+    'halo_lstm_pair_image_offsets': (_i, [_i] * 5 + [_vp, _vp]),
+    'halo_lstm_pack_pair_images': (_i, [_vp, _vp, _vp, _vp] + [_i] * 5 + [_vp]),
     'halo_lstm_persistent2_eligible': (_i, [_i, _i, _i, _i]),
     'halo_lstm_status_offset': (_sz, [_i] * 6),
     'halo_ghost_tile': (_i, []),
@@ -253,6 +256,7 @@
     'halo_adamw_multi_max_tensors': (_i, []),
     'halo_adamw_multi': (_i, [_vp, _vp, _i, _vp, _i, _f, _f, _f, _f, _i, _vp, _vp]),
     'halo_adamw_ranges': (_i, [_vp, _vp, _vp, _vp, _i, _vp, _vp, _vp, _vp, _f, _f, _f, _f, _i, _vp, _vp]),
+    'halo_adamw_ranges_images': (_i, [_vp, _vp, _vp, _vp, _i, _vp, _vp, _vp, _vp, _f, _vp, _f, _f, _f, _i, _vp, _vp, _i, _vp, _i, _vp, _vp, _vp]),
     'halo_adamw': (_i, [_vp, _vp, _vp, _vp, _sz, _f, _f, _f, _f, _f, _i, _vp, _vp]),
 }
 
diff --git a/haloop_amd/csrc/halo_internal.h b/haloop_amd/csrc/halo_internal.h
--- a/haloop_amd/csrc/halo_internal.h
+++ b/haloop_amd/csrc/halo_internal.h
@@ -54,6 +54,7 @@
     uint64_t lstm_weights_stamp = 0, packF_stamp = 0;
     const float *packF_reserve = nullptr, *packF_w[3] = {nullptr, nullptr, nullptr};
     int packF_dims[5] = {0, 0, 0, 0, 0};
+    const float *pair_images_current = nullptr;
     int lstm_keep_dg = 0;
     const float *ghost_reserve = nullptr;
     int mute_block = -1;
diff --git a/haloop_amd/csrc/lstm.hip b/haloop_amd/csrc/lstm.hip
--- a/haloop_amd/csrc/lstm.hip
+++ b/haloop_amd/csrc/lstm.hip
@@ -1121,6 +1121,16 @@
     return (char *)reserve + reserve_flags_offset(T, B, in0, H, L) + PERSIST_FLAG_BYTES + (size_t)3 * 4 * H * H * sizeof(float);
 }
 
+inline void pair_image_offsets(int T, int B, int in0, int H, int L, size_t fwd[3], size_t tr[3]) {
+    const int kin = in0 > H ? in0 : H;
+    const size_t extra = ((size_t)4 * H * H + (size_t)L * layer_floats(T, B, H)) * sizeof(float) + halo_tiled_image_bytes(T * B, kin) +
+                         halo_tiled_image_bytes(4 * H, kin);
+    fwd[0] = 0;
+    fwd[1] = extra + ((size_t)4 * H * H + (size_t)(L - 2) * 8 * H * H) * sizeof(float);
+    fwd[2] = fwd[1] + (size_t)4 * H * H * sizeof(float);
+    for (int m = 0; m < 3; ++m) tr[m] = reserve_flags_offset(T, B, in0, H, L) + PERSIST_FLAG_BYTES + (size_t)m * 4 * H * H * sizeof(float);
+}
+
 inline bool persist_emit_enabled() {
     int &v = halo_ctx_cur().persist_emit;
     if (v < 0) { const char *e = getenv("HALO_PERSIST_EMIT"); v = e ? (atoi(e) != 0) : 1; }
@@ -1209,7 +1219,8 @@
 int lstm_fwd_persist2(const float *in, int in_dim, int lo, const float *const *w_ih, const float *const *w_hh, const float *const *b_ih,
                       const float *const *b_hh, const float *h0, const float *c0, float *y, long y_stride_t, long y_stride_b,
                       int y_relu, float *hn, float *cn, float *reserve, float *extra, char *img_in, char *img_w, int T, int B,
-                      int in0, int H, int L, float p_drop, uint64_t seed, uint32_t offset, const uint32_t *offset_dev, hipStream_t st) {
+                      int in0, int H, int L, float p_drop, uint64_t seed, uint32_t offset, const uint32_t *offset_dev, bool images_current,
+                      hipStream_t st) {
     const int hi = lo + 1;
     const size_t BH = (size_t)B * H;
     const LayerBufs l0 = layer_bufs(reserve, lo, T, B, H), l1 = layer_bufs(reserve, hi, T, B, H);
@@ -1254,7 +1265,7 @@
         PackPairArgs pp;
         for (int m = 0; m < 3; ++m) { pp.w[m] = pa.w[m]; pp.fwd[m] = (char *)pa.wdst[m]; pp.tr[m] = (char *)(wT + (size_t)m * 4 * H * H); }
         pp.H = H;
-        pp.tile_blocks = 3 * (4 * H / 32) * (H / 32) / 4;
+        pp.tile_blocks = images_current ? 0 : 3 * (4 * H / 32) * (H / 32) / 4;
         pp.rest = pa; pp.rest.w_units = 0;
         pp.rest.zero2 = reserve_bwd_flags(reserve, T, B, in0, H, L); pp.rest.zero2_units = (long)(PERSIST_FLAG_BYTES / 16);
         pp.zbase[0] = pp.zbase[1] = nullptr; pp.zstride = 0; pp.zunits = 0; pp.zcount = 0;
@@ -1402,6 +1413,30 @@
     return HALO_OK;
 }
 
+int halo_set_lstm_pair_images_current(const float *reserve) {
+    halo_ctx_cur().pair_images_current = reserve;
+    return HALO_OK;
+}
+int halo_lstm_pair_image_offsets(int T, int B, int in0, int H, int L, size_t *fwd, size_t *tr) {
+    HALO_CHECK_ARG(T > 0 && B > 0 && in0 > 0 && H > 0 && L >= 2 && fwd && tr);
+    pair_image_offsets(T, B, in0, H, L, fwd, tr);
+    return HALO_OK;
+}
+int halo_lstm_pack_pair_images(const float *w_hh_lo, const float *w_hh_hi, const float *w_ih_hi, float *reserve, int T, int B, int in0,
+                               int H, int L, halo_stream_t stream) {
+    HALO_CHECK_ARG(w_hh_lo && w_hh_hi && w_ih_hi && reserve && T > 0 && B > 0 && in0 > 0 && H > 0 && L >= 2);
+    if (H % 32 != 0) return HALO_ENOTSUP;
+    size_t fwd[3], tr[3];
+    pair_image_offsets(T, B, in0, H, L, fwd, tr);
+    PackPairArgs pp = {};
+    pp.w[0] = w_hh_lo; pp.w[1] = w_hh_hi; pp.w[2] = w_ih_hi;
+    for (int m = 0; m < 3; ++m) { pp.fwd[m] = (char *)reserve + fwd[m]; pp.tr[m] = (char *)reserve + tr[m]; }
+    pp.H = H;
+    pp.tile_blocks = 3 * (4 * H / 32) * (H / 32) / 4;
+    hipLaunchKernelGGL(persist2_pack_pair_kernel, dim3((unsigned)pp.tile_blocks), dim3(256), 0, (hipStream_t)stream, pp);
+    return halo_launch_status();
+}
+
 int halo_set_grad_sumsq(float *partials, int capacity) {
     HaloCtx &ctx = halo_ctx_cur();
     if (partials && capacity <= 0) return HALO_EINVAL;
@@ -1450,6 +1485,8 @@
     const size_t BH = (size_t)B * H, PH = bt16(B) * H;
     halo_ctx_cur().packT_reserve = nullptr;
     halo_ctx_cur().emitT_reserve = nullptr;
+    const bool images_current = halo_ctx_cur().pair_images_current == reserve;
+    halo_ctx_cur().pair_images_current = nullptr;
     float *wp = reserve;
     const bool x3 = use_x3(H);
     const int kin = in0 > H ? in0 : H;
@@ -1478,7 +1515,7 @@
         if (pair && l == n_single) {
             float *extra = (float *)(img_w + halo_tiled_image_bytes(4 * H, kin));
             return lstm_fwd_persist2(in, in_dim, l, w_ih, w_hh, b_ih, b_hh, h0, c0, y, y_stride_t, y_stride_b, y_relu, hn, cn, reserve, extra,
-                                     img_in, img_w, T, B, in0, H, L, p_drop, seed, offset, offset_dev, st);
+                                     img_in, img_w, T, B, in0, H, L, p_drop, seed, offset, offset_dev, images_current, st);
         }
         if (halo_math_mode() != HALO_MATH_F32 && in_dim >= 64) {
             const HaloPrepJob jobs[2] = {{0, in, T * B, in_dim, in_dim, img_in, nullptr}, {0, w_ih[l], 4 * H, in_dim, in_dim, img_w, nullptr}};
diff --git a/haloop_amd/csrc/optim.hip b/haloop_amd/csrc/optim.hip
--- a/haloop_amd/csrc/optim.hip
+++ b/haloop_amd/csrc/optim.hip
@@ -156,39 +156,45 @@
 
 
 constexpr int ADAM_MAX_RANGES = 8;
+constexpr int ADAM_RANGE_SLOTS = ADAM_MAX_RANGES + 3;
 struct AdamRangesArgs {
     float *p;
     const float *g;
     float *m;
     float *v;
-    size_t begin4[ADAM_MAX_RANGES], end4[ADAM_MAX_RANGES];
-    float decay_mul[ADAM_MAX_RANGES];
-    const float *grad_scale[ADAM_MAX_RANGES];
+    size_t begin4[ADAM_RANGE_SLOTS], end4[ADAM_RANGE_SLOTS];
+    float decay_mul[ADAM_RANGE_SLOTS];
+    const float *grad_scale[ADAM_RANGE_SLOTS];
     int n_ranges;
     float beta1_w, beta2, beta2_w, step_size, bc2_sqrt, eps;
     uint32_t *counter;
     const uint32_t *step_dev;
     const float *lr_dev;
-    float weight_decay[ADAM_MAX_RANGES];
+    float weight_decay[ADAM_RANGE_SLOTS];
     float lr, beta1;
 };
 
-template <bool NT>
-__global__ __launch_bounds__(256) void adamw_ranges_kernel(const AdamRangesArgs a) {
-    f32x4 *p4 = reinterpret_cast<f32x4 *>(a.p), *m4 = reinterpret_cast<f32x4 *>(a.m), *v4 = reinterpret_cast<f32x4 *>(a.v);
-    const f32x4 *g4 = reinterpret_cast<const f32x4 *>(a.g);
-    float step_size = a.step_size, bc2_sqrt = a.bc2_sqrt;
-    const float lr = a.lr_dev ? *a.lr_dev : a.lr;
+__device__ __forceinline__ void adam_ranges_scalars(const AdamRangesArgs &a, float &lr, float &step_size, float &bc2_sqrt) {
+    step_size = a.step_size; bc2_sqrt = a.bc2_sqrt;
+    lr = a.lr_dev ? *a.lr_dev : a.lr;
     if (a.step_dev) {
         const double t = (double)max(*a.step_dev, 1u);
         step_size = (float)((double)lr / (1.0 - pow((double)a.beta1, t)));
         bc2_sqrt = (float)sqrt(1.0 - pow((double)a.beta2, t));
     }
+}
+
+template <bool NT>
+__device__ __forceinline__ void adam_ranges_body(const AdamRangesArgs &a, unsigned block, unsigned nblocks) {
+    f32x4 *p4 = reinterpret_cast<f32x4 *>(a.p), *m4 = reinterpret_cast<f32x4 *>(a.m), *v4 = reinterpret_cast<f32x4 *>(a.v);
+    const f32x4 *g4 = reinterpret_cast<const f32x4 *>(a.g);
+    float lr, step_size, bc2_sqrt;
+    adam_ranges_scalars(a, lr, step_size, bc2_sqrt);
     for (int r = 0; r < a.n_ranges; ++r) {
         const float gs = a.grad_scale[r] ? *a.grad_scale[r] : 1.0f;
         if (gs != gs) continue;
         const float decay_mul = a.lr_dev ? (float)(1.0 - (double)lr * (double)a.weight_decay[r]) : a.decay_mul[r];
-        for (size_t i = a.begin4[r] + blockIdx.x * (size_t)256 + threadIdx.x; i < a.end4[r]; i += (size_t)gridDim.x * 256) {
+        for (size_t i = a.begin4[r] + block * (size_t)256 + threadIdx.x; i < a.end4[r]; i += (size_t)nblocks * 256) {
             f32x4 p = p4[i], m = NT ? __builtin_nontemporal_load(m4 + i) : m4[i], v = NT ? __builtin_nontemporal_load(v4 + i) : v4[i];
             const f32x4 g = NT ? __builtin_nontemporal_load(g4 + i) : g4[i];
 #pragma unroll
@@ -203,7 +209,79 @@
             else { m4[i] = m; v4[i] = v; }
         }
     }
+}
+
+template <bool NT>
+__global__ __launch_bounds__(256) void adamw_ranges_kernel(const AdamRangesArgs a) {
+    adam_ranges_body<NT>(a, blockIdx.x, gridDim.x);
     if (a.counter && blockIdx.x == 0 && threadIdx.x == 0) *a.counter += 1u;
+}
+
+constexpr int ADAM_IMG_SPAN = 256;
+struct AdamImagesArgs {
+    size_t mat_begin[3];
+    char *fwd[3], *tr[3];
+    float decay_mul[3], weight_decay[3];
+    const float *grad_scale[3];
+    int H, chunk_blocks;
+};
+
+template <bool NT>
+__global__ __launch_bounds__(256) void adamw_images_kernel(const AdamRangesArgs a, const AdamImagesArgs im) {
+    typedef __bf16 bf16x4 __attribute__((ext_vector_type(4)));
+    typedef __bf16 bf16x8 __attribute__((ext_vector_type(8)));
+    if ((int)blockIdx.x >= im.chunk_blocks) {
+        adam_ranges_body<NT>(a, blockIdx.x - im.chunk_blocks, gridDim.x - im.chunk_blocks);
+        if (a.counter && (int)blockIdx.x == im.chunk_blocks && threadIdx.x == 0) *a.counter += 1u;
+        return;
+    }
+    __shared__ __attribute__((aligned(16))) __bf16 tile[32][ADAM_IMG_SPAN + 8];
+    const int H = im.H, spans = H / ADAM_IMG_SPAN, per_mat = (4 * H / 32) * spans;
+    const int mi = (int)blockIdx.x / per_mat, rem = (int)blockIdx.x % per_mat;
+    const int R0 = (rem / spans) * 32, C0 = (rem % spans) * ADAM_IMG_SPAN;
+    const float gs = im.grad_scale[mi] ? *im.grad_scale[mi] : 1.0f;
+    if (gs != gs) return;
+    float lr, step_size, bc2_sqrt;
+    adam_ranges_scalars(a, lr, step_size, bc2_sqrt);
+    const float decay_mul = a.lr_dev ? (float)(1.0 - (double)lr * (double)im.weight_decay[mi]) : im.decay_mul[mi];
+    const int wave = threadIdx.x >> 6, lane = threadIdx.x & 63;
+    const size_t base4 = (im.mat_begin[mi] + (size_t)R0 * H + C0) / 4 + lane;
+    f32x4 *p4 = reinterpret_cast<f32x4 *>(a.p), *m4 = reinterpret_cast<f32x4 *>(a.m), *v4 = reinterpret_cast<f32x4 *>(a.v);
+    const f32x4 *g4 = reinterpret_cast<const f32x4 *>(a.g);
+#pragma unroll 2
+    for (int row = wave; row < 32; row += 4) {
+        const size_t i = base4 + (size_t)row * (H / 4);
+        f32x4 p = p4[i], m = NT ? __builtin_nontemporal_load(m4 + i) : m4[i], v = NT ? __builtin_nontemporal_load(v4 + i) : v4[i];
+        const f32x4 g = NT ? __builtin_nontemporal_load(g4 + i) : g4[i];
+        bf16x4 b;
+#pragma unroll
+        for (int e = 0; e < 4; ++e) {
+            const float ge = im.grad_scale[mi] ? g[e] * gs : g[e];
+            float pe = p[e], me = m[e], ve = v[e];
+            adam_update(pe, me, ve, ge, decay_mul, a.beta1_w, a.beta2, a.beta2_w, step_size, bc2_sqrt, a.eps);
+            p[e] = pe; m[e] = me; v[e] = ve;
+            b[e] = (__bf16)pe;
+        }
+        p4[i] = p;
+        if (NT) { __builtin_nontemporal_store(m, m4 + i); __builtin_nontemporal_store(v, v4 + i); }
+        else { m4[i] = m; v4[i] = v; }
+        *reinterpret_cast<bf16x4 *>(&tile[row][lane * 4]) = b;
+    }
+    __syncthreads();
+    const int i16 = lane & 15, kg = lane >> 4;
+    const int nkb = H / 32, nkb4 = 4 * H / 32;
+    const int g = R0 / H, jt = (R0 % H) / 16;
+    for (int q = wave; q < 2 * (ADAM_IMG_SPAN / 32); q += 4) {
+        const int half = q / (ADAM_IMG_SPAN / 32), kbl = q % (ADAM_IMG_SPAN / 32);
+        const bf16x8 hi = *reinterpret_cast<const bf16x8 *>(&tile[half * 16 + i16][kbl * 32 + kg * 8]);
+        *reinterpret_cast<bf16x8 *>(im.fwd[mi] + (((long)(jt + half) * 4 + g) * nkb + C0 / 32 + kbl) * 2048 + lane * 16) = hi;
+    }
+    for (int c = wave; c < ADAM_IMG_SPAN / 16; c += 4) {
+        bf16x8 hi;
+#pragma unroll
+        for (int e = 0; e < 8; ++e) hi[e] = tile[kg * 8 + e][c * 16 + i16];
+        *reinterpret_cast<bf16x8 *>(im.tr[mi] + ((long)(C0 / 16 + c) * nkb4 + R0 / 32) * 2048 + lane * 16) = hi;
+    }
 }
 
 struct AdamTensor {
@@ -447,25 +525,69 @@
     return halo_launch_status();
 }
 
+namespace {
+struct AdamImages {
+    int n = 0, H = 0;
+    const size_t *begin = nullptr;
+    void *const *fwd = nullptr, *const *tr = nullptr;
+};
+}
+
 static int adamw_ranges_impl(float *p, const float *g, float *m, float *v, int n_ranges, const size_t *begin, const size_t *end,
                       const float *weight_decay, const float *const *grad_scale, float lr, float beta1, float beta2, float eps, int step,
-                      const uint32_t *step_dev, const float *lr_dev, uint32_t *counter, halo_stream_t stream) {
+                      const uint32_t *step_dev, const float *lr_dev, uint32_t *counter, const AdamImages &img, halo_stream_t stream) {
     HALO_CHECK_ARG(p && g && m && v && begin && end && weight_decay && grad_scale && n_ranges > 0 && n_ranges <= ADAM_MAX_RANGES &&
                    (step >= 1 || step_dev) && (!lr_dev || step_dev));
     HALO_CHECK_ARG(((uintptr_t)p % 16 == 0) && ((uintptr_t)g % 16 == 0) && ((uintptr_t)m % 16 == 0) && ((uintptr_t)v % 16 == 0));
     AdamRangesArgs a;
-    a.p = p; a.g = g; a.m = m; a.v = v; a.n_ranges = n_ranges; a.counter = counter;
+    AdamImagesArgs im = {};
+    a.p = p; a.g = g; a.m = m; a.v = v; a.counter = counter;
     a.step_dev = step_dev; a.lr_dev = lr_dev; a.lr = lr; a.beta1 = beta1;
     if (step < 1) step = 1;
+    const size_t mat_len = (size_t)4 * img.H * img.H;
+    int order[3] = {0, 1, 2};
+    if (img.n) {
+        HALO_CHECK_ARG(img.n >= 1 && img.n <= 3 && img.H > 0 && img.H % ADAM_IMG_SPAN == 0 && img.begin && img.fwd && img.tr);
+        for (int k = 0; k < img.n; ++k)
+            HALO_CHECK_ARG(img.begin[k] % 4 == 0 && img.fwd[k] && img.tr[k] && (uintptr_t)img.fwd[k] % 16 == 0 && (uintptr_t)img.tr[k] % 16 == 0);
+        for (int i = 0; i < img.n; ++i)
+            for (int j = i + 1; j < img.n; ++j)
+                if (img.begin[order[j]] < img.begin[order[i]]) { const int t = order[i]; order[i] = order[j]; order[j] = t; }
+        for (int i = 0; i + 1 < img.n; ++i) HALO_CHECK_ARG(img.begin[order[i]] + mat_len <= img.begin[order[i + 1]]);
+        im.H = img.H;
+        im.chunk_blocks = img.n * (4 * img.H / 32) * (img.H / ADAM_IMG_SPAN);
+    }
     size_t biggest = 0;
+    int n_out = 0, placed = 0;
     for (int r = 0; r < n_ranges; ++r) {
         HALO_CHECK_ARG(begin[r] % 4 == 0 && end[r] % 4 == 0 && begin[r] <= end[r]);
-        a.begin4[r] = begin[r] / 4; a.end4[r] = end[r] / 4;
-        a.decay_mul[r] = (float)(1.0 - (double)lr * (double)weight_decay[r]);
-        a.weight_decay[r] = weight_decay[r];
-        a.grad_scale[r] = grad_scale[r];
-        if (a.end4[r] - a.begin4[r] > biggest) biggest = a.end4[r] - a.begin4[r];
-    }
+        size_t at = begin[r];
+        auto piece = [&](size_t lo, size_t hi) {
+            if (img.n && lo == hi) return;
+            a.begin4[n_out] = lo / 4; a.end4[n_out] = hi / 4;
+            a.decay_mul[n_out] = (float)(1.0 - (double)lr * (double)weight_decay[r]);
+            a.weight_decay[n_out] = weight_decay[r];
+            a.grad_scale[n_out] = grad_scale[r];
+            if (hi / 4 - lo / 4 > biggest) biggest = hi / 4 - lo / 4;
+            ++n_out;
+        };
+        for (int i = 0; i < img.n; ++i) {
+            const int k = order[i];
+            const size_t mb = img.begin[k], me = mb + mat_len;
+            if (me <= begin[r] || mb >= end[r]) continue;
+            HALO_CHECK_ARG(mb >= at && me <= end[r]);
+            piece(at, mb);
+            at = me;
+            im.mat_begin[k] = mb; im.fwd[k] = (char *)img.fwd[k]; im.tr[k] = (char *)img.tr[k];
+            im.decay_mul[k] = (float)(1.0 - (double)lr * (double)weight_decay[r]);
+            im.weight_decay[k] = weight_decay[r];
+            im.grad_scale[k] = grad_scale[r];
+            ++placed;
+        }
+        piece(at, end[r]);
+    }
+    HALO_CHECK_ARG(placed == img.n);
+    a.n_ranges = n_out;
     const double bc1 = 1.0 - pow((double)beta1, (double)step);
     const double bc2 = 1.0 - pow((double)beta2, (double)step);
     a.beta1_w = (float)(1.0 - (double)beta1);
@@ -479,6 +601,12 @@
     if (blocks < 1) blocks = 1;
     static int nt = -1;
     if (nt < 0) { const char *e = getenv("HALO_ADAMW_NT"); nt = (e && e[0] == '0') ? 0 : 1; }
+    if (img.n) {
+        const dim3 grid((unsigned)(im.chunk_blocks + blocks));
+        if (nt) hipLaunchKernelGGL(adamw_images_kernel<true>, grid, dim3(256), 0, (hipStream_t)stream, a, im);
+        else hipLaunchKernelGGL(adamw_images_kernel<false>, grid, dim3(256), 0, (hipStream_t)stream, a, im);
+        return halo_launch_status();
+    }
     if (nt) hipLaunchKernelGGL(adamw_ranges_kernel<true>, dim3((unsigned)blocks), dim3(256), 0, (hipStream_t)stream, a);
     else hipLaunchKernelGGL(adamw_ranges_kernel<false>, dim3((unsigned)blocks), dim3(256), 0, (hipStream_t)stream, a);
     return halo_launch_status();
@@ -488,7 +616,7 @@
                       const float *weight_decay, const float *const *grad_scale, float lr, float beta1, float beta2, float eps, int step,
                       uint32_t *counter, halo_stream_t stream) {
     return adamw_ranges_impl(p, g, m, v, n_ranges, begin, end, weight_decay, grad_scale, lr, beta1, beta2, eps, step, nullptr, nullptr,
-                             counter, stream);
+                             counter, AdamImages(), stream);
 }
 
 int halo_adamw_ranges_dev(float *p, const float *g, float *m, float *v, int n_ranges, const size_t *begin, const size_t *end,
@@ -496,7 +624,18 @@
                           float eps, const uint32_t *step_dev, uint32_t *counter, halo_stream_t stream) {
     HALO_CHECK_ARG(step_dev);
     return adamw_ranges_impl(p, g, m, v, n_ranges, begin, end, weight_decay, grad_scale, lr, beta1, beta2, eps, 0, step_dev, lr_dev,
-                             counter, stream);
-}
-
-}
+                             counter, AdamImages(), stream);
+}
+
+int halo_adamw_ranges_images(float *p, const float *g, float *m, float *v, int n_ranges, const size_t *begin, const size_t *end,
+                             const float *weight_decay, const float *const *grad_scale, float lr, const float *lr_dev, float beta1,
+                             float beta2, float eps, int step, const uint32_t *step_dev, uint32_t *counter, int n_mats,
+                             const size_t *mat_begin, int H, void *const *img_fwd, void *const *img_tr, halo_stream_t stream) {
+    HALO_CHECK_ARG(n_mats >= 1 && n_mats <= 3 && mat_begin && img_fwd && img_tr);
+    AdamImages img;
+    img.n = n_mats; img.H = H; img.begin = mat_begin; img.fwd = img_fwd; img.tr = img_tr;
+    return adamw_ranges_impl(p, g, m, v, n_ranges, begin, end, weight_decay, grad_scale, lr, beta1, beta2, eps, step_dev ? 0 : step, step_dev,
+                             lr_dev, counter, img, stream);
+}
+
+}
diff --git a/haloop_amd/ops.py b/haloop_amd/ops.py
--- a/haloop_amd/ops.py
+++ b/haloop_amd/ops.py
@@ -424,7 +424,7 @@
 
 
 def lstm_fwd(x_tm, w_ih, w_hh, b_ih, b_hh, h0=None, c0=None, y=None, y_strides=None, y_relu=False,
-             want_state=False, drop=NO_DROPOUT, expect_backward=True, reserve=None, weights_stamp=0):
+             want_state=False, drop=NO_DROPOUT, expect_backward=True, reserve=None, weights_stamp=0, images_current=False):
     _f32c(x_tm, 'x')
     T, B, in0 = x_tm.shape
     L = len(w_hh)
@@ -448,6 +448,8 @@
     if not expect_backward:
         lib().halo_set_lstm_expect_backward(0)
         lib().halo_set_lstm_weights_stamp(int(weights_stamp))
+    if images_current:
+        lib().halo_set_lstm_pair_images_current(ptr(reserve))
     try:
         check(lib().halo_lstm_fwd(ptr(x_tm), a_ih, a_hh, a_bi, a_bh, ptr(h0), ptr(c0), ptr(y), y_strides[0], y_strides[1],
                                   int(y_relu), ptr(hn), ptr(cn), ptr(reserve), T, B, in0, H, L, drop.p, drop.seed,
@@ -461,6 +463,22 @@
 
 def lstm_reserve(T, B, in0, H, L, device):
     return torch.empty((lib().halo_lstm_reserve_bytes(T, B, in0, H, L) + 3) // 4, device=device, dtype=torch.float32)
+
+
+def lstm_pair_images(reserve, T, B, in0, H, L):
+    fwd, tr = (C.c_size_t * 3)(), (C.c_size_t * 3)()
+    check(lib().halo_lstm_pair_image_offsets(T, B, in0, H, L, fwd, tr), 'halo_lstm_pair_image_offsets')
+    base = reserve.data_ptr()
+    if max(tr) + 4 * H * H * 4 > reserve.numel() * 4:
+        raise ValueError('lstm_pair_images: the reserve is too small for this shape (ops.lstm_reserve)')
+    return [base + o for o in fwd], [base + o for o in tr]
+
+
+def lstm_pack_pair_images(w_hh_lo, w_hh_hi, w_ih_hi, reserve, T, B, in0, L):
+    for t in (w_hh_lo, w_hh_hi, w_ih_hi):
+        _f32c(t, 'lstm parameter')
+    check(lib().halo_lstm_pack_pair_images(ptr(w_hh_lo), ptr(w_hh_hi), ptr(w_ih_hi), ptr(reserve), T, B, in0, w_hh_lo.shape[1], L,
+                                           _stream()), 'halo_lstm_pack_pair_images')
 
 
 def lstm_bwd_workspace(x_tm, w_hh):
@@ -875,14 +893,23 @@
     torch.autograd.graph.increment_version(p)
 
 
-def adamw_ranges(p, g, m, v, ranges, lr, beta1, beta2, eps, step, counter=None):
+def adamw_ranges(p, g, m, v, ranges, lr, beta1, beta2, eps, step, counter=None, images=None):
     _lib.bump_weights_epoch()
     n = len(ranges)
     begin = (C.c_size_t * n)(*[r[0] for r in ranges])
     end = (C.c_size_t * n)(*[r[1] for r in ranges])
     wd = (C.c_float * n)(*[float(r[2]) for r in ranges])
     gs = (C.c_void_p * n)(*[ptr(r[3]) for r in ranges])
-    if torch.is_tensor(step):
+    if images is not None:
+        offs, H, fwd, tr = images
+        k = len(offs)
+        dev_step = torch.is_tensor(step)
+        lr_dev = lr if (dev_step and torch.is_tensor(lr)) else None
+        check(lib().halo_adamw_ranges_images(ptr(p), ptr(g), ptr(m), ptr(v), n, begin, end, wd, gs, 0.0 if lr_dev is not None else lr,
+                                             ptr(lr_dev), beta1, beta2, eps, 0 if dev_step else step, ptr(step) if dev_step else None,
+                                             ptr(counter), k, (C.c_size_t * k)(*offs), H, (C.c_void_p * k)(*fwd), (C.c_void_p * k)(*tr),
+                                             _stream()), 'halo_adamw_ranges_images')
+    elif torch.is_tensor(step):
         lr_dev = lr if torch.is_tensor(lr) else None
         check(lib().halo_adamw_ranges_dev(ptr(p), ptr(g), ptr(m), ptr(v), n, begin, end, wd, gs, 0.0 if lr_dev is not None else lr,
                                           ptr(lr_dev), beta1, beta2, eps, ptr(step), ptr(counter), _stream()), 'halo_adamw_ranges_dev')
diff --git a/haloop_amd/train.py b/haloop_amd/train.py
--- a/haloop_amd/train.py
+++ b/haloop_amd/train.py
@@ -167,6 +167,11 @@
         self._graphs = None
         self._static = None
         self._accum = torch.zeros_like(self.flat.grads) if self.accumulate > 1 else None
+        self.adamw_images = os.environ.get('HALO_ADAMW_IMAGES', '1') != '0'
+        self._img = None
+        self._img_on = False
+        self._graph_img = None
+        self.image_refills = 0
 
     @property
     def lr(self):
@@ -182,6 +187,51 @@
             raise _lib.HaloError('a persistent LSTM recurrence timed out waiting for its peer workgroups (they were not all resident); '
                                  'no optimizer update has been applied since.  Free the GPU of other work, or select the step-launch '
                                  'chain with haloop_amd._lib.set_lstm_persistent(False), then zero trainer.status and continue.')
+
+    @property
+    def adamw_images_active(self):
+        return self._img_on
+
+    def _images_mats(self):
+        lstm = self.encoder.lstm
+        return (lstm.weight_hh_l0, lstm.weight_hh_l1, lstm.weight_ih_l1)
+
+    def _images_key(self):
+        return (_lib.weights_epoch(), _lib.get_math_mode()) + tuple((p.data_ptr(), p._version) for p in self._images_mats())
+
+    def _images_dims(self, x):
+        lstm = getattr(self.encoder, 'lstm', None)
+        if not self.adamw_images or self.sharded is not None or self.world > 1 or lstm is None or lstm.num_layers != 2:
+            return None
+        B, T, _ = x.shape
+        H, Tp, in0 = lstm.weight_hh_l0.shape[1], ops.subsampled_length(T), self.encoder.subsample.weight.shape[0]
+        if H % 256 != 0 or _lib.get_math_mode() != 'bf16' or _lib.lib().halo_lstm_persistent2_eligible(Tp, B, H, 2) != 1:
+            return None
+        return (Tp, B, in0, H, 2)
+
+    def _images_begin(self, x, dims):
+        self._img_on = dims is not None
+        if dims is None:
+            if self._img is not None:
+                self._img['key'] = None
+            return
+        if self._img is None or self._img['dims'] != dims:
+            Tp, B, in0, H, L = dims
+            reserve = ops.lstm_reserve(Tp, B, in0, H, L, x.device)
+            fwd, tr = ops.lstm_pair_images(reserve, Tp, B, in0, H, L)
+            where = {n: o for n, _, o in self.flat.slots}
+            offs = [where[f'encoder.lstm.{n}'] for n in ('weight_hh_l0', 'weight_hh_l1', 'weight_ih_l1')]
+            self._img = {'dims': dims, 'reserve': reserve, 'fwd': fwd, 'tr': tr, 'offs': offs, 'key': None}
+            if self._graph_img is not None and self._graph_img != dims:
+                self._graphs, self._graph_img = None, None
+        if self._img['key'] != self._images_key():
+            Tp, B, in0, H, L = dims
+            ops.lstm_pack_pair_images(*self._images_mats(), self._img['reserve'], Tp, B, in0, L)
+            self.image_refills += 1
+
+    def _images_end(self):
+        if self._img_on:
+            self._img['key'] = self._images_key()
 
     def _dropout(self):
         p = self.encoder.dropout.p if self.encoder.training else 0.0
@@ -221,7 +271,9 @@
         y_sub, col = ops.subsample_fwd(x, enc.subsample.weight, enc.subsample.bias, drop)
         Tp = y_sub.shape[0]
         feats = torch.empty(B, Tp, H, device=x.device, dtype=torch.float32)
-        _, _, _, reserve = ops.lstm_fwd(y_sub, w_ih, w_hh, b_ih, b_hh, y=feats, y_strides=(H, Tp * H), y_relu=True, drop=drop)
+        home = self._img['reserve'] if self._img_on else None
+        _, _, _, reserve = ops.lstm_fwd(y_sub, w_ih, w_hh, b_ih, b_hh, y=feats, y_strides=(H, Tp * H), y_relu=True, drop=drop,
+                                        reserve=home, images_current=self._img_on)
         p_cls = rec.dropout.p if rec.training else 0.0
         cdrop = Dropout(p_cls, self.seed, 0, self.counter) if p_cls > 0 else NO_DROPOUT
         grads = {'dw_ih': [gv[f'encoder.lstm.weight_ih_l{k}'] for k in range(L)],
@@ -313,6 +365,12 @@
         ops.sumsq_partials(d[1], parts)
         ops.clip_coef(parts, _lib.HALO_SUMSQ_PARTS, self.clip, coef, norm, applied_steps=cnt)
         ops.adamw_ranges(d[0], d[1], d[2], d[3], [(0, 8, 0.0, coef[0:1])], self.lr, self.betas[0], self.betas[1], self.eps, cnt)
+        if self._img_on:
+            f, im = self.flat, self._img
+            nan = torch.full((1,), float('nan'), device=dev, dtype=torch.float32)
+            lo, hi = min(im['offs']), max(im['offs']) + 4 * im['dims'][3] ** 2
+            ops.adamw_ranges(f.params, f.grads, f.exp_avg, f.exp_avg_sq, [(lo, hi, 0.0, nan)], self.lr, self.betas[0], self.betas[1],
+                             self.eps, cnt, images=(im['offs'], im['dims'][3], im['fwd'], im['tr']))
 
     def _optimizer(self):
         if getattr(self, '_norm_count', 0) > 0 and self.sharded is None:
@@ -347,8 +405,10 @@
         ranges = [(max(a, lo), min(b, hi), self.weight_decay if decays else 0.0, self.coef[0:1] if clipped else self.coef[1:2])
                   for a, b, decays, clipped in f.ranges for lo, hi in _merge_adjacent(self._own_ranges()) if min(b, hi) > max(a, lo)]
         if ranges:
+            im = self._img
+            images = (im['offs'], im['dims'][3], im['fwd'], im['tr']) if self._img_on else None
             ops.adamw_ranges(f.params, f.grads, f.exp_avg, f.exp_avg_sq, ranges, self._lr_dev, self.betas[0], self.betas[1], self.eps,
-                             self.adam_step, counter=self.counter)
+                             self.adam_step, counter=self.counter, images=images)
         else:
             ops.counter_inc(self.counter)
 
@@ -456,7 +516,10 @@
         if _lib._status_tensor is not self.status:
             _lib.set_status_word(self.status)
         if self.accumulate > 1:
-            return self._accumulating_step(x, input_lengths, targets, target_lengths)
+            self._images_begin(x, self._images_dims(x) if not self.use_graph else self._graph_images_dims(x))
+            loss = self._accumulating_step(x, input_lengths, targets, target_lengths)
+            self._images_end()
+            return loss
         self.step_count += 1
         if self.sharded is not None:
             if self._gather_mode is not None and getattr(self.sharded, 'gather_bf16', False) and _lib.get_math_mode() != self._gather_mode:
@@ -465,6 +528,7 @@
                 self._tail_graph, self._tail_calls = None, 0
             return self._sharded_step(x, input_lengths, targets, target_lengths)
         if not self.use_graph:
+            self._images_begin(x, self._images_dims(x))
             st = self._forward_backward_top(x, input_lengths, targets, target_lengths)
             w1 = self.avg_early.start()
             self._backward_rest(st)
@@ -472,8 +536,17 @@
             self.avg_early.finish(w1)
             self.avg_late.finish(w2)
             self._optimizer()
+            self._images_end()
             return self.loss
-        return self._graph_step(x, input_lengths, targets, target_lengths)
+        self._images_begin(x, self._graph_images_dims(x))
+        loss = self._graph_step(x, input_lengths, targets, target_lengths)
+        self._images_end()
+        return loss
+
+    def _graph_images_dims(self, x):
+        if self._graphs is None or self._static[0].shape != x.shape:
+            self._graph_img = self._images_dims(x)
+        return self._graph_img
 
     def _forward_backward_overlapped(self, x, il, tg, tl):
         sh = self.sharded
diff --git a/include/halo.h b/include/halo.h
--- a/include/halo.h
+++ b/include/halo.h
@@ -172,6 +172,10 @@
 int halo_set_lstm_bwd_mid_event(void *event);
 int halo_lstm_bwd_mid_event_recorded(void);
 int halo_set_lstm_weights_stamp(uint64_t stamp);
+int halo_set_lstm_pair_images_current(const float *reserve);
+int halo_lstm_pair_image_offsets(int T, int B, int in0, int H, int L, size_t *fwd, size_t *tr);
+int halo_lstm_pack_pair_images(const float *w_hh_lo, const float *w_hh_hi, const float *w_ih_hi, float *reserve, int T, int B, int in0,
+                               int H, int L, halo_stream_t stream);
 int halo_set_lstm_expect_backward(int on);
 int halo_set_lstm_dx_slabs(int n);
 int halo_lstm_dx_slabs_left(void);
@@ -515,6 +519,11 @@
                           const float *weight_decay, const float *const *grad_scale, float lr, const float *lr_dev, float beta1,
                           float beta2, float eps, const uint32_t *step_dev, uint32_t *counter, halo_stream_t stream);
 
+int halo_adamw_ranges_images(float *p, const float *g, float *m, float *v, int n_ranges, const size_t *begin, const size_t *end,
+                             const float *weight_decay, const float *const *grad_scale, float lr, const float *lr_dev, float beta1,
+                             float beta2, float eps, int step, const uint32_t *step_dev, uint32_t *counter, int n_mats,
+                             const size_t *mat_begin, int H, void *const *img_fwd, void *const *img_tr, halo_stream_t stream);
+
 size_t halo_adamw_multi_tensor_bytes(void);
 unsigned halo_adamw_multi_chunk(void);
 int halo_adamw_multi_max_tensors(void);
```

After: 160,600 utterances/s (median of 4 runs). 1.2% higher.
